# AmnonDrory/PointDSC

Measured on AMD Instinct MI355X. Metric: correspondence-pairs/sec through NSM (N=1k/5k) at 1/2/4/8 GPUs; 3DMatch recall parity, higher is better.
Workload: dtype f32 (3xf16-split contractions); 1 GPU; synthetic random correspondences N=1000 (3dmatch-like, 30% inliers), 128 scan pairs per GPU per step, full PointDSC testing forward (12 layers x 128 ch, trained synthetic weights, classifier rescaled by synthetic.BENCH_CLS for tie-free seed ranking); num_corr=1000, global_batch=128, parallelism=dp1 (independent pairs)

## Files before the change

### include/pdsc.h

```cpp
#ifndef PDSC_H_
#define PDSC_H_

#include <stddef.h>
#include <stdint.h>

#ifdef __cplusplus
extern "C" {
#endif

typedef void *pdsc_stream_t;

enum pdsc_status {
    PDSC_OK = 0,
    PDSC_ERR_ARG = 1,
    PDSC_ERR_HIP = 2,
    PDSC_ERR_UNSUPPORTED = 3,
    PDSC_ERR_RANGE = 4,
};

enum pdsc_precision {
    PDSC_PRECISION_H3 = 0,
    PDSC_PRECISION_F32 = 1,
};

int32_t pdsc_range_status(const void *forward_workspace, int32_t B, int32_t *flags, pdsc_stream_t stream);

int32_t pdsc_range_poll(const void *forward_workspace, int32_t B, pdsc_stream_t stream);

typedef struct pdsc_config {
    int32_t in_dim;
    int32_t num_layers;
    int32_t num_channels;
    int32_t num_iterations;
    int32_t k;
    double ratio;
    float inlier_threshold;
    float nms_radius;
    float refine_threshold;
    int32_t precision;
} pdsc_config;

const char *pdsc_version(void);
const char *pdsc_last_error(void);

int32_t pdsc_param_count(const pdsc_config *cfg);
const char *pdsc_param_name(const pdsc_config *cfg, int32_t i);
size_t pdsc_packed_weights_floats(const pdsc_config *cfg);
int32_t pdsc_pack_weights(const pdsc_config *cfg, const float *const *params_host_array,
                          float *packed, pdsc_stream_t stream);

int32_t pdsc_compat_f32(const float *src, const float *tgt, int32_t B, int32_t N,
                        const float *sigma_d_dev, float *M, pdsc_stream_t stream);
size_t pdsc_compat_packed_floats(int32_t N);
int32_t pdsc_compat_packed_f32(const float *src, const float *tgt, int32_t B, int32_t N,
                               const float *sigma_d_dev, float *Mp, pdsc_stream_t stream);

size_t pdsc_encoder_workspace_bytes(const pdsc_config *cfg, int32_t B, int32_t N);
int32_t pdsc_encoder_f32(const pdsc_config *cfg, const float *packed, const float *corr_pos,
                         const float *M, int32_t B, int32_t N, float *feat, float *normed,
                         float *conf, void *workspace, size_t workspace_bytes,
                         pdsc_stream_t stream);

size_t pdsc_attention_workspace_bytes(int32_t B, int32_t N, int32_t C, int32_t precision);
int32_t pdsc_attention_f32(const float *q, const float *k, const float *v, const float *M,
                           int32_t B, int32_t N, int32_t C, int32_t precision, float *msg, void *workspace,
                           size_t workspace_bytes, pdsc_stream_t stream);

int32_t pdsc_attention_layout(int32_t B, int32_t N, int32_t precision, int32_t *Npad, int32_t *nsplit);

int32_t pdsc_encoder_plan(int32_t B, int32_t N, int32_t precision, int32_t *fused);

int32_t pdsc_attention_timing(void *const *start_events, void *const *stop_events, int32_t capacity,
                              int32_t *count);
#define PDSC_FORWARD_STAGES 7
int32_t pdsc_forward_timing(void *const *events, int32_t capacity, int32_t *count);
int32_t pdsc_diag_qkv_delay(int32_t loops);

int32_t pdsc_pick_seeds(const float *src, const float *conf, int32_t B, int32_t N, float radius,
                        int32_t S, int32_t *seeds, float *is_local_max, pdsc_stream_t stream);

size_t pdsc_seed_knn_workspace_bytes(int32_t B, int32_t N, int32_t S);
int32_t pdsc_seed_knn(const float *normed, const int32_t *seeds, int32_t B, int32_t N, int32_t C,
                      int32_t S, int32_t k, int32_t precision, int32_t *knn, void *workspace,
                      size_t workspace_bytes, pdsc_stream_t stream);

size_t pdsc_nsm_workspace_bytes(int32_t B, int32_t N, int32_t S, int32_t k, int32_t num_iterations);
int32_t pdsc_nsm_weights(const float *normed, const float *src, const float *tgt,
                         const int32_t *knn, int32_t B, int32_t N, int32_t C, int32_t S, int32_t k,
                         int32_t num_iterations, int32_t precision, const float *sigma_dev,
                         const float *sigma_d_dev, float *weights, int32_t *iters_used, void *workspace,
                         size_t workspace_bytes, pdsc_stream_t stream);

int32_t pdsc_rigid_transform_3d(const float *A, const float *Bp, const float *w, int32_t nb,
                                int32_t n, float *trans, pdsc_stream_t stream);

size_t pdsc_seed_hypotheses_workspace_bytes(int32_t B, int32_t S);
int32_t pdsc_seed_hypotheses(const float *src, const float *tgt, const int32_t *knn,
                             const float *weights, int32_t B, int32_t N, int32_t S, int32_t k,
                             float tau, float *seed_trans, float *fitness, int32_t *best,
                             float *trans, float *labels, void *workspace, size_t workspace_bytes,
                             pdsc_stream_t stream);

int32_t pdsc_post_refine(float *trans, const float *src, const float *tgt, int32_t B, int32_t N,
                         float thr, pdsc_stream_t stream);

size_t pdsc_spectral_matching_workspace_bytes(int32_t N);
int32_t pdsc_spectral_matching(const float *corr_pos, const float *src, const float *tgt, int32_t N,
                               double inlier_threshold, double top_ratio, int32_t num_iterations, float *trans,
                               float *labels, float *leading_eig, void *workspace, size_t workspace_bytes,
                               pdsc_stream_t stream);
int32_t pdsc_sm_matvec(const float *M, const float *v, int32_t N, float *y, pdsc_stream_t stream);

size_t pdsc_forward_training_workspace_bytes(const pdsc_config *cfg, int32_t B, int32_t N);
int32_t pdsc_forward_training(const pdsc_config *cfg, const float *packed, const float *corr_pos,
                              const float *src, const float *tgt, int32_t B, int32_t N, float *final_trans,
                              float *confidence, float *M_out, int32_t *seeds_out, void *workspace,
                              size_t workspace_bytes, pdsc_stream_t stream);
size_t pdsc_spectral_matching_loss_workspace_bytes(int32_t B, int32_t N);
int32_t pdsc_spectral_matching_loss(const float *M, const float *gt_labels, int32_t B, int32_t N, int32_t balanced,
                                    float *loss, void *workspace, size_t workspace_bytes, pdsc_stream_t stream);

size_t pdsc_mutual_nn_workspace_bytes(int32_t Ns, int32_t Nt);
int32_t pdsc_mutual_nn(const float *src_desc, const float *tgt_desc, int32_t Ns, int32_t Nt, int32_t D,
                       int32_t *nn_src, int32_t *nn_tgt, void *workspace, size_t workspace_bytes,
                       pdsc_stream_t stream);
int32_t pdsc_build_correspondences(const float *src_desc, const float *tgt_desc, const float *src_xyz,
                                   const float *tgt_xyz, int32_t Ns, int32_t Nt, int32_t D, int32_t mutual,
                                   const double *gt_trans, double inlier_threshold, int32_t *corr,
                                   int32_t *count, float *corr_pos, float *src_keypts, float *tgt_keypts,
                                   float *labels, void *workspace, size_t workspace_bytes, pdsc_stream_t stream);

int32_t pdsc_ply_read_xyz(const char *path, float *xyz, int64_t capacity, int64_t *n_points);
size_t pdsc_radius_knn_workspace_bytes(int32_t n);
int32_t pdsc_radius_knn(const float *pts, int32_t n, float radius, int32_t max_nn, int32_t *nbr, double *dist2,
                        int32_t *count, void *workspace, size_t workspace_bytes, pdsc_stream_t stream);
enum pdsc_normal_orientation {
    PDSC_NORMALS_OPEN3D = 0,
    PDSC_NORMALS_VIEWPOINT = 1,
    PDSC_NORMALS_CENTROID = 2,
};
size_t pdsc_estimate_normals_workspace_bytes(int32_t n, int32_t max_nn);
int32_t pdsc_estimate_normals(const float *pts, int32_t n, float radius, int32_t max_nn, int32_t orient,
                              const float *viewpoint, float *normals, void *workspace, size_t workspace_bytes,
                              pdsc_stream_t stream);
size_t pdsc_voxel_down_sample_workspace_bytes(int32_t n);
int32_t pdsc_voxel_down_sample(const float *pts, const float *normals, int32_t n, float voxel_size, float *out_pts,
                               float *out_normals, int32_t *out_count, void *workspace, size_t workspace_bytes,
                               pdsc_stream_t stream);
size_t pdsc_compute_fpfh_workspace_bytes(int32_t n, int32_t max_nn);
int32_t pdsc_compute_fpfh(const float *pts, const float *normals, int32_t n, float radius, int32_t max_nn,
                          double *fpfh, float *fpfh_normalized, void *workspace, size_t workspace_bytes,
                          pdsc_stream_t stream);

size_t pdsc_forward_workspace_bytes(const pdsc_config *cfg, int32_t B, int32_t N);
int32_t pdsc_forward_testing(const pdsc_config *cfg, const float *packed, const float *corr_pos,
                             const float *src, const float *tgt, int32_t B, int32_t N,
                             float *final_trans, float *final_labels, float *conf_out,
                             int32_t *seeds_out, void *workspace, size_t workspace_bytes,
                             pdsc_stream_t stream);
typedef struct pdsc_forward_debug {
    float *conf;
    int32_t *seeds;
    int32_t *knn;
    float *weights;
    float *trans_pre_refine;
} pdsc_forward_debug;
int32_t pdsc_forward_testing_debug(const pdsc_config *cfg, const float *packed, const float *corr_pos,
                                   const float *src, const float *tgt, int32_t B, int32_t N,
                                   float *final_trans, float *final_labels, const pdsc_forward_debug *debug,
                                   void *workspace, size_t workspace_bytes, pdsc_stream_t stream);

int32_t pdsc_forward_testing_ragged(const pdsc_config *cfg, const float *packed, const float *corr_pos,
                                    const float *src, const float *tgt, int32_t B, int32_t N,
                                    const int32_t *counts, float *final_trans, float *final_labels,
                                    const pdsc_forward_debug *debug, void *workspace, size_t workspace_bytes,
                                    pdsc_stream_t stream);

#ifdef __cplusplus
}
#endif
#endif
```

### pointdsc_amd/_lib.py

```python
from __future__ import annotations

import ctypes
import os
import threading

_HERE = os.path.dirname(os.path.abspath(__file__))
_VARIANT = os.environ.get("PDSC_LIB_VARIANT", "")
LIB_PATH = os.path.join(_HERE, f"libpdsc_{_VARIANT}.so" if _VARIANT else "libpdsc.so")

c_int32, c_size_t, c_float, c_double = ctypes.c_int32, ctypes.c_size_t, ctypes.c_float, ctypes.c_double
vp = ctypes.c_void_p


class PdscConfig(ctypes.Structure):
    _fields_ = [
        ("in_dim", c_int32),
        ("num_layers", c_int32),
        ("num_channels", c_int32),
        ("num_iterations", c_int32),
        ("k", c_int32),
        ("ratio", c_double),
        ("inlier_threshold", c_float),
        ("nms_radius", c_float),
        ("refine_threshold", c_float),
        ("precision", c_int32),
    ]


PRECISIONS = {"h3": 0, "f32": 1}


def precision_code(precision) -> int:
    if precision not in PRECISIONS:
        raise ValueError(f"precision must be one of {sorted(PRECISIONS)}, got {precision!r}")
    return PRECISIONS[precision]


CFG = ctypes.POINTER(PdscConfig)


class PdscForwardDebug(ctypes.Structure):
    _fields_ = [("conf", vp), ("seeds", vp), ("knn", vp), ("weights", vp), ("trans_pre_refine", vp)]


_PROTOS = {
    "pdsc_version": (ctypes.c_char_p, []),
    "pdsc_last_error": (ctypes.c_char_p, []),
    "pdsc_param_count": (c_int32, [CFG]),
    "pdsc_param_name": (ctypes.c_char_p, [CFG, c_int32]),
    "pdsc_packed_weights_floats": (c_size_t, [CFG]),
    "pdsc_pack_weights": (c_int32, [CFG, ctypes.POINTER(vp), vp, vp]),
    "pdsc_compat_f32": (c_int32, [vp, vp, c_int32, c_int32, vp, vp, vp]),
    "pdsc_compat_packed_floats": (c_size_t, [c_int32]),
    "pdsc_compat_packed_f32": (c_int32, [vp, vp, c_int32, c_int32, vp, vp, vp]),
    "pdsc_encoder_workspace_bytes": (c_size_t, [CFG, c_int32, c_int32]),
    "pdsc_encoder_f32": (c_int32, [CFG, vp, vp, vp, c_int32, c_int32, vp, vp, vp, vp, c_size_t, vp]),
    "pdsc_attention_workspace_bytes": (c_size_t, [c_int32, c_int32, c_int32, c_int32]),
    "pdsc_attention_f32": (c_int32, [vp, vp, vp, vp, c_int32, c_int32, c_int32, c_int32, vp, vp, c_size_t, vp]),
    "pdsc_attention_layout": (c_int32, [c_int32, c_int32, c_int32, ctypes.POINTER(c_int32),
                                        ctypes.POINTER(c_int32)]),
    "pdsc_encoder_plan": (c_int32, [c_int32, c_int32, c_int32, ctypes.POINTER(c_int32)]),
    "pdsc_attention_timing": (c_int32, [ctypes.POINTER(vp), ctypes.POINTER(vp), c_int32, ctypes.POINTER(c_int32)]),
    "pdsc_forward_timing": (c_int32, [ctypes.POINTER(vp), c_int32, ctypes.POINTER(c_int32)]),
    "pdsc_diag_qkv_delay": (c_int32, [c_int32]),
    "pdsc_pick_seeds": (c_int32, [vp, vp, c_int32, c_int32, c_float, c_int32, vp, vp, vp]),
    "pdsc_seed_knn_workspace_bytes": (c_size_t, [c_int32, c_int32, c_int32]),
    "pdsc_seed_knn": (c_int32, [vp, vp, c_int32, c_int32, c_int32, c_int32, c_int32, c_int32, vp, vp, c_size_t,
                                vp]),
    "pdsc_nsm_workspace_bytes": (c_size_t, [c_int32, c_int32, c_int32, c_int32, c_int32]),
    "pdsc_nsm_weights": (c_int32, [vp, vp, vp, vp, c_int32, c_int32, c_int32, c_int32, c_int32, c_int32, c_int32,
                                   vp, vp, vp, vp, vp, c_size_t, vp]),
    "pdsc_rigid_transform_3d": (c_int32, [vp, vp, vp, c_int32, c_int32, vp, vp]),
    "pdsc_seed_hypotheses_workspace_bytes": (c_size_t, [c_int32, c_int32]),
    "pdsc_seed_hypotheses": (c_int32, [vp, vp, vp, vp, c_int32, c_int32, c_int32, c_int32, c_float,
                                       vp, vp, vp, vp, vp, vp, c_size_t, vp]),
    "pdsc_post_refine": (c_int32, [vp, vp, vp, c_int32, c_int32, c_float, vp]),
    "pdsc_mutual_nn_workspace_bytes": (c_size_t, [c_int32, c_int32]),
    "pdsc_mutual_nn": (c_int32, [vp, vp, c_int32, c_int32, c_int32, vp, vp, vp, c_size_t, vp]),
    "pdsc_build_correspondences": (c_int32, [vp, vp, vp, vp, c_int32, c_int32, c_int32, c_int32, vp, c_double,
                                             vp, vp, vp, vp, vp, vp, vp, c_size_t, vp]),
    "pdsc_spectral_matching_workspace_bytes": (c_size_t, [c_int32]),
    "pdsc_spectral_matching": (c_int32, [vp, vp, vp, c_int32, c_double, c_double, c_int32, vp, vp, vp, vp,
                                         c_size_t, vp]),
    "pdsc_sm_matvec": (c_int32, [vp, vp, c_int32, vp, vp]),
    "pdsc_forward_workspace_bytes": (c_size_t, [CFG, c_int32, c_int32]),
    "pdsc_forward_testing": (c_int32, [CFG, vp, vp, vp, vp, c_int32, c_int32, vp, vp, vp, vp, vp,
                                       c_size_t, vp]),
    "pdsc_forward_testing_debug": (c_int32, [CFG, vp, vp, vp, vp, c_int32, c_int32, vp, vp,
                                             ctypes.POINTER(PdscForwardDebug), vp, c_size_t, vp]),
    "pdsc_forward_testing_ragged": (c_int32, [CFG, vp, vp, vp, vp, c_int32, c_int32, ctypes.POINTER(c_int32), vp, vp,
                                              ctypes.POINTER(PdscForwardDebug), vp, c_size_t, vp]),
    "pdsc_ply_read_xyz": (c_int32, [ctypes.c_char_p, vp, ctypes.c_int64, ctypes.POINTER(ctypes.c_int64)]),
    "pdsc_radius_knn_workspace_bytes": (c_size_t, [c_int32]),
    "pdsc_radius_knn": (c_int32, [vp, c_int32, c_float, c_int32, vp, vp, vp, vp, c_size_t, vp]),
    "pdsc_estimate_normals_workspace_bytes": (c_size_t, [c_int32, c_int32]),
    "pdsc_estimate_normals": (c_int32, [vp, c_int32, c_float, c_int32, c_int32, vp, vp, vp, c_size_t, vp]),
    "pdsc_voxel_down_sample_workspace_bytes": (c_size_t, [c_int32]),
    "pdsc_voxel_down_sample": (c_int32, [vp, vp, c_int32, c_float, vp, vp, vp, vp, c_size_t, vp]),
    "pdsc_compute_fpfh_workspace_bytes": (c_size_t, [c_int32, c_int32]),
    "pdsc_compute_fpfh": (c_int32, [vp, vp, c_int32, c_float, c_int32, vp, vp, vp, c_size_t, vp]),
    "pdsc_forward_training_workspace_bytes": (c_size_t, [CFG, c_int32, c_int32]),
    "pdsc_range_status": (c_int32, [vp, c_int32, ctypes.POINTER(c_int32), vp]),
    "pdsc_range_poll": (c_int32, [vp, c_int32, vp]),
    "pdsc_forward_training": (c_int32, [CFG, vp, vp, vp, vp, c_int32, c_int32, vp, vp, vp, vp, vp, c_size_t, vp]),
    "pdsc_spectral_matching_loss_workspace_bytes": (c_size_t, [c_int32, c_int32]),
    "pdsc_spectral_matching_loss": (c_int32, [vp, vp, c_int32, c_int32, c_int32, vp, vp, c_size_t, vp]),
}

EXPORTS = tuple(_PROTOS)

_lib = None
_lock = threading.Lock()


def load():
    global _lib
    if _lib is not None:
        return _lib
    with _lock:
        if _lib is None:
            if not os.path.exists(LIB_PATH):
                raise RuntimeError(
                    f"pointdsc_amd: HIP library {LIB_PATH} is missing; build it with "
                    "`make -C pointdsc_amd/csrc` or `python -c 'import __graft_entry__ as g; g.build()'`. "
                    "There is no CPU fallback.")
            try:
                lib = ctypes.CDLL(LIB_PATH)
            except OSError as e:
                raise RuntimeError(f"pointdsc_amd: cannot load {LIB_PATH}: {e}") from e
            for name, (res, args) in _PROTOS.items():
                fn = getattr(lib, name)
                fn.restype, fn.argtypes = res, args
            _lib = lib
    return _lib


def check(status: int, what: str):
    if status != 0:
        msg = load().pdsc_last_error().decode(errors="replace")
        raise RuntimeError(f"{what} failed (status {status}): {msg}")


def make_config(in_dim=6, num_layers=12, num_channels=128, num_iterations=10, k=40, ratio=0.1,
                inlier_threshold=0.10, nms_radius=0.10, precision="h3") -> PdscConfig:
    refine = 0.10 if inlier_threshold == 0.10 else 1.2
    return PdscConfig(int(in_dim), int(num_layers), int(num_channels), int(num_iterations), int(k),
                      float(ratio), float(inlier_threshold), float(nms_radius), float(refine),
                      precision_code(precision))
```

### pointdsc_amd/csrc/api.hip

```cpp
#include <algorithm>
#include <chrono>
#include <cstdarg>
#include <cstdio>
#include <cstdlib>
#include <mutex>
#include <string>
#include <vector>

#include "attention_plan.hpp"
#include "pdsc_internal.hpp"

using namespace pdsc;

namespace pdsc {
thread_local int g_diag_qkv_delay = 0;
}

namespace {

thread_local std::string g_err;
thread_local std::string g_name;

thread_local hipEvent_t *g_tstart = nullptr, *g_tstop = nullptr;
thread_local int g_tcap = 0;
thread_local int32_t *g_tcount = nullptr;
thread_local hipEvent_t *g_fev = nullptr;
thread_local int g_fcap = 0;
thread_local int32_t *g_fcount = nullptr;

int fail(int code, const char *fmt, ...) {
    char buf[512];
    va_list ap;
    va_start(ap, fmt);
    vsnprintf(buf, sizeof(buf), fmt, ap);
    va_end(ap);
    g_err = buf;
    return code;
}

#define HIPCHK(expr)                                                                          \
    do {                                                                                      \
        hipError_t e_ = (expr);                                                               \
        if (e_ != hipSuccess) return fail(PDSC_ERR_HIP, "%s: %s", #expr, hipGetErrorString(e_)); \
    } while (0)

hipStream_t S_(pdsc_stream_t s) { return reinterpret_cast<hipStream_t>(s); }

struct Carve {
    char *base;
    size_t off = 0;
    explicit Carve(void *p) : base(static_cast<char *>(p)) {}
    template <typename T> T *take(size_t n) {
        T *p = base ? reinterpret_cast<T *>(base + off) : nullptr;
        off += align_bytes(n * sizeof(T));
        return p;
    }
};

int check_cfg(const pdsc_config *cfg) {
    if (!cfg) return fail(PDSC_ERR_ARG, "cfg is NULL");
    if (cfg->num_channels != CH)
        return fail(PDSC_ERR_UNSUPPORTED, "num_channels=%d: only %d is implemented", cfg->num_channels, CH);
    if (cfg->num_layers < 1 || cfg->num_layers > 64)
        return fail(PDSC_ERR_UNSUPPORTED, "num_layers=%d not in [1, 64]", cfg->num_layers);
    if (cfg->in_dim < 1 || cfg->in_dim > 128) return fail(PDSC_ERR_UNSUPPORTED, "in_dim=%d not in [1, 128]", cfg->in_dim);
    if (cfg->num_iterations < 0 || cfg->num_iterations > 31)
        return fail(PDSC_ERR_UNSUPPORTED, "num_iterations=%d not in [0, 31]", cfg->num_iterations);
    if (cfg->k < 1) return fail(PDSC_ERR_ARG, "k=%d", cfg->k);
    if (cfg->precision != PDSC_PRECISION_H3 && cfg->precision != PDSC_PRECISION_F32)
        return fail(PDSC_ERR_ARG, "precision=%d (PDSC_PRECISION_H3 or PDSC_PRECISION_F32)", cfg->precision);
    return PDSC_OK;
}

struct Dims {
    int B, N, Npad, S, k, T;
    bool f32;
    EncoderPlan plan;
};

int make_dims(const pdsc_config *cfg, int B, int N, Dims &d, bool dense_m_caller = false) {
    if (B < 1 || N < 2) return fail(PDSC_ERR_ARG, "B=%d N=%d (need B >= 1, N >= 2)", B, N);
    if (N > 32767) return fail(PDSC_ERR_UNSUPPORTED, "N=%d > 32767 (32-bit buffer descriptors over M)", N);
    d.B = B;
    d.N = N;
    d.Npad = round_up(N, QB);
    d.S = (int)((double)N * cfg->ratio);
    d.k = std::min(cfg->k, N - 1);
    d.T = cfg->num_iterations;
    d.f32 = cfg->precision == PDSC_PRECISION_F32;
    d.plan = plan_encoder(B, N, d.f32, dense_m_caller);
    if (d.S < 1) return fail(PDSC_ERR_ARG, "int(N*ratio) = 0 seeds for N=%d", N);
    if (d.k > 63) return fail(PDSC_ERR_UNSUPPORTED, "k=%d > 63", d.k);
    return PDSC_OK;
}

struct EncBufs {
    float *feat, *opart, *ml, *vexp, *vexp2;
    float *feat2;
    _Float16 *q, *k, *v;
    _Float16 *q2, *k2, *v2;
    float *opart1, *ml1;
};

EncBufs carve_encoder(Carve &c, const Dims &d) {
    EncBufs e;
    const size_t rows = (size_t)d.B * d.Npad * CH;
    e.feat = c.take<float>(rows);
    e.q = c.take<_Float16>(2 * rows);
    e.k = c.take<_Float16>(2 * rows);
    e.v = c.take<_Float16>(2 * rows);
    e.opart = c.take<float>(rows * d.plan.nsplit);
    e.ml = c.take<float>((size_t)d.B * d.Npad * d.plan.nsplit * 2);
    e.vexp = c.take<float>((size_t)d.B * (d.Npad / 32));
    e.opart1 = d.plan.precombine ? c.take<float>(rows) : nullptr;
    e.ml1 = d.plan.precombine ? c.take<float>((size_t)d.B * d.Npad * 2) : nullptr;
    e.q2 = e.k2 = e.v2 = nullptr;
    e.vexp2 = nullptr;
    e.feat2 = d.plan.fused() ? nullptr : c.take<float>(rows);
    if (d.plan.fused()) {
        e.q2 = c.take<_Float16>(2 * rows);
        e.k2 = c.take<_Float16>(2 * rows);
        e.v2 = c.take<_Float16>(2 * rows);
        e.vexp2 = c.take<float>((size_t)d.B * (d.Npad / 32));
    }
    return e;
}

int run_encoder(const PackLayout &lay, const float *packed, const float *corr_pos, const float *M, const Dims &d,
                const EncBufs &e, float *feat_out, float *normed, _Float16 *normed_s, float *conf, hipStream_t s,
                Ragged rg = {}) {
    const EncoderPlan plan = d.plan.for_ragged(rg);
    HIPCHK(launch_pw_first(packed, lay, corr_pos, d.f32, d.B, d.N, d.Npad, e.feat, e.q, e.k, e.v, e.vexp, s, rg,
                           plan.fused()));
    if (plan.fused()) {
        _Float16 *q = e.q, *k = e.k, *v = e.v, *q2 = e.q2, *k2 = e.k2, *v2 = e.v2;
        float *vx = e.vexp, *vx2 = e.vexp2;
        for (int l = 0; l + 1 < lay.L; ++l) {
            const bool timed = g_tcap > 0 && g_tcount && *g_tcount < g_tcap;
            if (timed) HIPCHK(hipEventRecord(g_tstart[*g_tcount], s));
            HIPCHK(launch_attn_pw2(plan, packed, lay, l, q, k, v, vx, M, e.feat, q2, k2, v2, vx2, s, rg));
            if (timed) HIPCHK(hipEventRecord(g_tstop[(*g_tcount)++], s));
            std::swap(q, q2);
            std::swap(k, k2);
            std::swap(v, v2);
            std::swap(vx, vx2);
        }
        HIPCHK(launch_attn_pw2_last(plan, packed, lay, q, k, v, vx, M, e.feat, feat_out, normed, normed_s, conf, s, rg));
        return PDSC_OK;
    }
    float *feat = e.feat, *feat_alt = e.feat2;
    for (int l = 0; l < lay.L; ++l) {
        const bool timed = g_tcap > 0 && g_tcount && *g_tcount < g_tcap;
        if (timed) HIPCHK(hipEventRecord(g_tstart[*g_tcount], s));
        HIPCHK(launch_attention(plan, e.q, e.k, e.v, e.vexp, M, e.opart, e.ml, s, rg, l));
        if (timed) HIPCHK(hipEventRecord(g_tstop[(*g_tcount)++], s));
        const float *op = e.opart, *mlp = e.ml;
        int ns = plan.nsplit;
        if (plan.precombine) {
            HIPCHK(launch_combine_rows(e.opart, e.ml, d.B, d.Npad, plan.nsplit, e.opart1, e.ml1, s));
            op = e.opart1;
            mlp = e.ml1;
            ns = 1;
        }
        if (l + 1 < lay.L) {
            HIPCHK(launch_pw_mid(packed, lay, l, d.f32, op, mlp, ns, d.B, d.N, d.Npad, feat, feat_alt, e.q, e.k, e.v,
                                 e.vexp, s));
            std::swap(feat, feat_alt);
        } else {
            HIPCHK(launch_pw_last(packed, lay, d.f32, op, mlp, ns, d.B, d.N, d.Npad, feat, feat_out, normed,
                                  d.f32 ? nullptr : normed_s, conf, s));
        }
    }
    return PDSC_OK;
}

static int enc_halves_mode() {
    static const int v = [] {
        const char *e = getenv("PDSC_ENC_HALVES");
        return e && e[0] == '0' ? 0 : (e && e[0] == '1' ? 2 : 1);
    }();
    return v;
}
constexpr int ENC_MAX_PARTS = 4;
static int enc_parts() {
    static const int v = [] {
        const char *e = getenv("PDSC_ENC_PARTS");
        const int p = e ? atoi(e) : 2;
        return std::min(std::max(p, 2), ENC_MAX_PARTS);
    }();
    return v;
}
static bool enc_work_balanced() {
    static const bool on = [] {
        const char *e = getenv("PDSC_ENC_BAL");
        return e && e[0] == '1';
    }();
    return on;
}
static bool enc_halves(const Dims &d, bool ragged) {
    const int mode = enc_halves_mode();
    return d.plan.fused() && d.B >= 16 * enc_parts() && (mode == 2 || (mode == 1 && ragged));
}
static void enc_bounds(const int32_t *counts, int B, int P, int *bounds) {
    std::vector<double> pre(B + 1, 0.0);
    for (int b = 0; b < B; ++b) pre[b + 1] = pre[b] + (counts ? (double)counts[b] * counts[b] : 1.0);
    bounds[0] = 0;
    bounds[P] = B;
    for (int i = 1; i < P; ++i) {
        const double goal = pre[B] * i / P;
        int h = bounds[i - 1] + 1;
        while (h < B - (P - i) && std::abs(pre[h + 1] - goal) < std::abs(pre[h] - goal)) ++h;
        bounds[i] = h;
    }
}

struct SideStream {
    std::mutex mu;
    hipStream_t s2[ENC_MAX_PARTS - 1] = {};
    hipEvent_t fork = nullptr, join[ENC_MAX_PARTS - 1] = {};
    bool ok = false;
};
static SideStream *side_stream(hipStream_t s) {
    static SideStream ss[64];
    hipDevice_t dev = 0;
    if (!s || hipStreamGetDevice(s, &dev) != hipSuccess)
        if (hipGetDevice(&dev) != hipSuccess) return nullptr;
    if (dev < 0 || dev >= 64) return nullptr;
    SideStream &x = ss[dev];
    static std::mutex create_mu;
    std::lock_guard<std::mutex> lock(create_mu);
    if (!x.ok) {
        int cur = dev;
        if (hipGetDevice(&cur) != hipSuccess || (cur != dev && hipSetDevice(dev) != hipSuccess)) return nullptr;
        bool ok = x.fork || hipEventCreateWithFlags(&x.fork, hipEventDisableTiming) == hipSuccess;
        for (int i = 0; ok && i < ENC_MAX_PARTS - 1; ++i) {
            if (!x.s2[i]) ok = hipStreamCreateWithFlags(&x.s2[i], hipStreamNonBlocking) == hipSuccess;
            if (ok && !x.join[i]) ok = hipEventCreateWithFlags(&x.join[i], hipEventDisableTiming) == hipSuccess;
        }
        if (cur != dev) (void)hipSetDevice(cur);
        x.ok = ok;
    }
    return x.ok ? &x : nullptr;
}

static int run_encoder_part(const PackLayout &lay, const float *packed, const float *corr_pos, const float *M,
                            const Dims &d, const EncBufs &e, float *normed, _Float16 *normed_s, float *conf,
                            hipStream_t s, Ragged rg, int b0, int nb) {
    Dims dh = d;
    dh.B = nb;
    dh.plan = d.plan.for_pairs(nb);
    const size_t rows = (size_t)b0 * d.Npad * CH;
    EncBufs eh = e;
    eh.feat = e.feat + rows;
    eh.q = e.q + 2 * rows;
    eh.k = e.k + 2 * rows;
    eh.v = e.v + 2 * rows;
    eh.q2 = e.q2 + 2 * rows;
    eh.k2 = e.k2 + 2 * rows;
    eh.v2 = e.v2 + 2 * rows;
    eh.vexp = e.vexp + (size_t)b0 * (d.Npad / 32);
    eh.vexp2 = e.vexp2 + (size_t)b0 * (d.Npad / 32);
    const size_t mstr = d.plan.m_layout == M_PACKED ? mpack_floats(d.N) : (size_t)d.N * d.N;
    Ragged rh = rg;
    if (rg.nv) rh.nv = rg.nv + b0;
    if (rg.sv) rh.sv = rg.sv + b0;
    if (rg.po) rh.po = rg.po + b0;
    return run_encoder(lay, packed, corr_pos + (size_t)b0 * d.N * lay.in_dim, M + (size_t)b0 * mstr, dh, eh, nullptr,
                       normed + (size_t)b0 * d.N * CH, normed_s + (size_t)b0 * d.N * 2 * CH, conf + (size_t)b0 * d.N, s,
                       rh);
}

static int run_encoder_fwd(const PackLayout &lay, const float *packed, const float *corr_pos, const float *M,
                           const Dims &d, const EncBufs &e, float *normed, _Float16 *normed_s, float *conf,
                           hipStream_t s, Ragged rg, SideStream *ss, const int *bounds, int P) {
    if (!ss) return run_encoder(lay, packed, corr_pos, M, d, e, nullptr, normed, normed_s, conf, s, rg);
    std::lock_guard<std::mutex> lock(ss->mu);
    {
        hipStreamCaptureStatus cs = hipStreamCaptureStatusNone, c2 = hipStreamCaptureStatusNone;
        unsigned long long id = 0, id2 = 0;
        HIPCHK(hipStreamGetCaptureInfo(s, &cs, &id));
        for (int i = 1; i < P; ++i) {
            HIPCHK(hipStreamGetCaptureInfo(ss->s2[i - 1], &c2, &id2));
            if (c2 != hipStreamCaptureStatusNone && (cs != hipStreamCaptureStatusActive || id2 != id))
                return run_encoder(lay, packed, corr_pos, M, d, e, nullptr, normed, normed_s, conf, s, rg);
        }
    }
    HIPCHK(hipEventRecord(ss->fork, s));
    int forked = 1, r = PDSC_OK;
    for (; forked < P; ++forked)
        if (hipStreamWaitEvent(ss->s2[forked - 1], ss->fork, 0) != hipSuccess) {
            r = fail(PDSC_ERR_HIP, "hipStreamWaitEvent (fork)");
            break;
        }
    for (int i = 0; r == PDSC_OK && i < P; ++i)
        r = run_encoder_part(lay, packed, corr_pos, M, d, e, normed, normed_s, conf, i ? ss->s2[i - 1] : s, rg,
                             bounds[i], bounds[i + 1] - bounds[i]);
    for (int i = 1; i < forked; ++i) {
        const hipError_t a = hipEventRecord(ss->join[i - 1], ss->s2[i - 1]);
        const hipError_t b = a == hipSuccess ? hipStreamWaitEvent(s, ss->join[i - 1], 0) : a;
        if (b != hipSuccess && r == PDSC_OK) r = fail(PDSC_ERR_HIP, "join: %s", hipGetErrorString(b));
    }
    return r;
}

struct NsmBufs {
    float *hist, *weights;
    _Float16 *ns;
    unsigned *mask;
};

NsmBufs carve_nsm(Carve &c, int B, int N, int S, int k, int T, bool own_split) {
    NsmBufs n;
    n.ns = own_split ? c.take<_Float16>((size_t)B * N * 2 * CH) : nullptr;
    n.hist = c.take<float>((size_t)B * S * std::max(T, 1) * k);
    n.mask = c.take<unsigned>((size_t)B * S);
    n.weights = c.take<float>((size_t)B * S * k);
    return n;
}

int run_nsm(const float *normed, const _Float16 *normed_s, bool f32, const float *src, const float *tgt,
            const int *knn, int B, int N, int S, int k, int T, const float *sigma, const float *sigma_d,
            const NsmBufs &nb, float *weights, int *iters, bool batch_global, hipStream_t s, Ragged rg = {}) {
    if (!f32 && !normed_s) {
        HIPCHK(launch_split_rows(normed, (size_t)B * N, nb.ns, s));
        normed_s = nb.ns;
    }
    const void *feats = f32 ? static_cast<const void *>(normed) : static_cast<const void *>(normed_s);
    if (T > 0)
        HIPCHK(launch_nsm_seed(feats, f32, src, tgt, knn, B, N, S, k, T, sigma, sigma_d, nb.hist, nb.mask, s, rg));
    HIPCHK(launch_nsm_finish(nb.hist, nb.mask, B, S, k, T, batch_global, weights, iters, s, rg));
    return PDSC_OK;
}

static bool tail_fused() {
    static const bool off = [] {
        const char *e = getenv("PDSC_TAIL_FUSED");
        return e && e[0] == '0';
    }();
    return !off;
}

static bool ragged_order_on() {
    static const bool off = [] {
        const char *e = getenv("PDSC_RAGGED_ORDER");
        return e && e[0] == '0';
    }();
    return !off;
}

struct FwdBufs {
    int *range;
    float *M, *normed, *conf, *lm, *kdist, *seed_trans, *weights, *hsums;
    _Float16 *normed_s;
    int *seeds, *knn, *counts;
    int *nv, *sv, *po;
    EncBufs enc;
    NsmBufs nsm;
};

FwdBufs carve_forward(Carve &c, const Dims &d) {
    FwdBufs f;
    f.range = c.take<int>((size_t)d.B);
    f.M = c.take<float>((size_t)d.B * std::max(mpack_floats(d.N), (size_t)d.N * d.N));
    f.enc = carve_encoder(c, d);
    f.normed = c.take<float>((size_t)d.B * d.N * CH);
    f.normed_s = c.take<_Float16>((size_t)d.B * d.N * 2 * CH);
    f.conf = c.take<float>((size_t)d.B * d.N);
    f.lm = c.take<float>((size_t)d.B * d.N);
    f.seeds = c.take<int>((size_t)d.B * d.S);
    f.kdist = c.take<float>((size_t)d.B * d.S * d.N);
    f.knn = c.take<int>((size_t)d.B * d.S * d.k);
    f.nsm = carve_nsm(c, d.B, d.N, d.S, d.k, d.T, false);
    f.weights = f.nsm.weights;
    f.seed_trans = c.take<float>((size_t)d.B * d.S * 16);
    f.counts = c.take<int>((size_t)d.B * d.S);
    f.hsums = c.take<float>((size_t)d.B * d.S * 15);
    f.nv = c.take<int>((size_t)d.B);
    f.sv = c.take<int>((size_t)d.B);
    f.po = c.take<int>((size_t)d.B);
    return f;
}

int need_ws(size_t have, size_t need) {
    if (have < need) return fail(PDSC_ERR_ARG, "workspace too small: %zu < %zu bytes", have, need);
    return PDSC_OK;
}

}

#define RET_IF(x)                  \
    do {                           \
        int r_ = (x);              \
        if (r_ != PDSC_OK) return r_; \
    } while (0)

namespace {
int32_t check_nn_args(const float *a, const float *b, int32_t Ns, int32_t Nt, int32_t D, void *ws, size_t ws_bytes) {
    if (!a || !b || !ws) return fail(PDSC_ERR_ARG, "null pointer");
    if (Ns < 1 || Nt < 1 || D < 1 || D > 64) return fail(PDSC_ERR_ARG, "Ns=%d Nt=%d D=%d (1 <= D <= 64)", Ns, Nt, D);
    return need_ws(ws_bytes, pdsc_mutual_nn_workspace_bytes(Ns, Nt));
}

__global__ void unpack_nn_kernel(const unsigned long long *key, int n, int32_t *out) {
    const int i = blockIdx.x * blockDim.x + threadIdx.x;
    if (i < n) out[i] = (int32_t)(uint32_t)key[i];
}
}

extern "C" {

const char *pdsc_version(void) { return "pdsc 0.1.0 gfx950"; }
const char *pdsc_last_error(void) { return g_err.c_str(); }

int32_t pdsc_param_count(const pdsc_config *cfg) { return cfg ? 10 + 26 * cfg->num_layers : -1; }

const char *pdsc_param_name(const pdsc_config *cfg, int32_t i) {
    if (!cfg || i < 0 || i >= pdsc_param_count(cfg)) return nullptr;
    static const char *bn[] = {"weight", "bias", "running_mean", "running_var"};
    static const char *per[] = {"fc_message.0.weight", "fc_message.0.bias", "fc_message.1.weight",
                                "fc_message.1.bias", "fc_message.1.running_mean", "fc_message.1.running_var",
                                "fc_message.3.weight", "fc_message.3.bias", "fc_message.4.weight",
                                "fc_message.4.bias", "fc_message.4.running_mean", "fc_message.4.running_var",
                                "fc_message.6.weight", "fc_message.6.bias", "projection_q.weight",
                                "projection_q.bias", "projection_k.weight", "projection_k.bias",
                                "projection_v.weight", "projection_v.bias"};
    static const char *tail[] = {"encoder.layer0.weight", "encoder.layer0.bias", "classification.0.weight",
                                 "classification.0.bias", "classification.2.weight", "classification.2.bias",
                                 "classification.4.weight", "classification.4.bias"};
    const int L = cfg->num_layers;
    if (i == 0) return "sigma";
    if (i == 1) return "sigma_spat";
    i -= 2;
    if (i < 26 * L) {
        const int l = i / 26, o = i % 26;
        char buf[128];
        if (o < 2)
            snprintf(buf, sizeof(buf), "encoder.blocks.PointCN_layer_%d.0.%s", l, o == 0 ? "weight" : "bias");
        else if (o < 6)
            snprintf(buf, sizeof(buf), "encoder.blocks.PointCN_layer_%d.1.%s", l, bn[o - 2]);
        else
            snprintf(buf, sizeof(buf), "encoder.blocks.NonLocal_layer_%d.%s", l, per[o - 6]);
        g_name = buf;
        return g_name.c_str();
    }
    return tail[i - 26 * L];
}

size_t pdsc_packed_weights_floats(const pdsc_config *cfg) {
    if (check_cfg(cfg) != PDSC_OK) return 0;
    return make_layout(cfg->num_layers, cfg->in_dim).total;
}

int32_t pdsc_pack_weights(const pdsc_config *cfg, const float *const *P, float *packed,
                          pdsc_stream_t stream) {
    RET_IF(check_cfg(cfg));
    if (!P || !packed) return fail(PDSC_ERR_ARG, "null params/packed");
    const int n = pdsc_param_count(cfg);
    for (int i = 0; i < n; ++i)
        if (!P[i]) return fail(PDSC_ERR_ARG, "param %d (%s) is NULL", i, pdsc_param_name(cfg, i));
    hipStream_t s = S_(stream);
    const PackLayout lay = make_layout(cfg->num_layers, cfg->in_dim);
    HIPCHK(hipMemsetAsync(packed, 0, lay.total * sizeof(float), s));
    HIPCHK(launch_copy(P[0], packed + lay.sigma, 1, s));
    HIPCHK(launch_copy(P[1], packed + lay.sigma_d, 1, s));
    const bool f32 = cfg->precision == PDSC_PRECISION_F32;
    auto dense = [&](const DenseOff &o, int wi, int in, int out, bool has_bn) -> hipError_t {
        return launch_pack_dense(P[wi], P[wi + 1], has_bn ? P[wi + 2] : nullptr,
                                 has_bn ? P[wi + 3] : nullptr, has_bn ? P[wi + 4] : nullptr,
                                 has_bn ? P[wi + 5] : nullptr, in, out, f32, packed + o.w, packed + o.bias,
                                 packed + o.alpha, packed + o.beta, packed + o.scale, s);
    };
    for (int l = 0; l < cfg->num_layers; ++l) {
        const int b = 2 + 26 * l;
        const LayerOff &lo = lay.layer[l];
        HIPCHK(dense(lo.pcn, b + 0, CH, CH, true));
        HIPCHK(dense(lo.fc0, b + 6, CH, CH2, true));
        HIPCHK(dense(lo.fc3, b + 12, CH2, CH2, true));
        HIPCHK(dense(lo.fc6, b + 18, CH2, CH, false));
        HIPCHK(dense(lo.q, b + 20, CH, CH, false));
        HIPCHK(dense(lo.k, b + 22, CH, CH, false));
        HIPCHK(dense(lo.v, b + 24, CH, CH, false));
    }
    const int t = 2 + 26 * cfg->num_layers;
    HIPCHK(launch_copy(P[t], packed + lay.l0_w, CH * cfg->in_dim, s));
    HIPCHK(launch_copy(P[t + 1], packed + lay.l0_b, CH, s));
    HIPCHK(dense(lay.c0, t + 2, CH, CLS, false));
    HIPCHK(dense(lay.c2, t + 4, CLS, CLS, false));
    HIPCHK(launch_copy(P[t + 6], packed + lay.c4_w, CLS, s));
    HIPCHK(launch_copy(P[t + 7], packed + lay.c4_b, 1, s));
    return PDSC_OK;
}

int32_t pdsc_compat_f32(const float *src, const float *tgt, int32_t B, int32_t N,
                        const float *sigma_d_dev, float *M, pdsc_stream_t stream) {
    if (!src || !tgt || !sigma_d_dev || !M) return fail(PDSC_ERR_ARG, "null pointer");
    if (B < 1 || N < 1) return fail(PDSC_ERR_ARG, "B=%d N=%d", B, N);
    HIPCHK(launch_compat(src, tgt, B, N, sigma_d_dev, M, S_(stream)));
    return PDSC_OK;
}

size_t pdsc_compat_packed_floats(int32_t N) { return N < 1 ? 0 : mpack_floats(N); }

int32_t pdsc_compat_packed_f32(const float *src, const float *tgt, int32_t B, int32_t N,
                               const float *sigma_d_dev, float *Mp, pdsc_stream_t stream) {
    if (!src || !tgt || !sigma_d_dev || !Mp) return fail(PDSC_ERR_ARG, "null pointer");
    if (B < 1 || N < 1) return fail(PDSC_ERR_ARG, "B=%d N=%d", B, N);
    HIPCHK(launch_compat_packed(src, tgt, B, N, sigma_d_dev, Mp, S_(stream)));
    return PDSC_OK;
}

size_t pdsc_encoder_workspace_bytes(const pdsc_config *cfg, int32_t B, int32_t N) {
    Dims d;
    if (check_cfg(cfg) != PDSC_OK || make_dims(cfg, B, N, d, true) != PDSC_OK) return 0;
    Carve c(nullptr);
    carve_encoder(c, d);
    return c.off;
}

int32_t pdsc_encoder_f32(const pdsc_config *cfg, const float *packed, const float *corr_pos,
                         const float *M, int32_t B, int32_t N, float *feat, float *normed, float *conf,
                         void *ws, size_t ws_bytes, pdsc_stream_t stream) {
    RET_IF(check_cfg(cfg));
    Dims d;
    RET_IF(make_dims(cfg, B, N, d, true));
    if (!packed || !corr_pos || !M || !normed || !conf || !ws) return fail(PDSC_ERR_ARG, "null pointer");
    RET_IF(need_ws(ws_bytes, pdsc_encoder_workspace_bytes(cfg, B, N)));
    Carve c(ws);
    const EncBufs e = carve_encoder(c, d);
    const PackLayout lay = make_layout(cfg->num_layers, cfg->in_dim);
    return run_encoder(lay, packed, corr_pos, M, d, e, feat, normed, nullptr, conf, S_(stream));
}

size_t pdsc_attention_workspace_bytes(int32_t B, int32_t N, int32_t C, int32_t precision) {
    if (C != CH || B < 1 || N < 1 || (precision != PDSC_PRECISION_H3 && precision != PDSC_PRECISION_F32)) return 0;
    const int Npad = round_up(N, QB), ns = plan_encoder(B, N, precision == PDSC_PRECISION_F32, true, false).nsplit;
    Carve c(nullptr);
    for (int i = 0; i < 3; ++i) c.take<_Float16>((size_t)2 * B * Npad * CH);
    c.take<float>((size_t)B * Npad * CH * ns);
    c.take<float>((size_t)B * Npad * ns * 2);
    c.take<float>((size_t)B * (Npad / 32));
    return c.off;
}

int32_t pdsc_attention_f32(const float *q, const float *k, const float *v, const float *M, int32_t B,
                           int32_t N, int32_t C, int32_t precision, float *msg, void *ws, size_t ws_bytes,
                           pdsc_stream_t stream) {
    if (C != CH) return fail(PDSC_ERR_UNSUPPORTED, "C=%d (only %d)", C, CH);
    if (!q || !k || !v || !M || !msg || !ws) return fail(PDSC_ERR_ARG, "null pointer");
    if (B < 1 || N < 1 || N > 32767) return fail(PDSC_ERR_ARG, "B=%d N=%d", B, N);
    if (precision != PDSC_PRECISION_H3 && precision != PDSC_PRECISION_F32)
        return fail(PDSC_ERR_ARG, "precision=%d", precision);
    RET_IF(need_ws(ws_bytes, pdsc_attention_workspace_bytes(B, N, C, precision)));
    hipStream_t s = S_(stream);
    const bool f32 = precision == PDSC_PRECISION_F32;
    const EncoderPlan plan = plan_encoder(B, N, f32, true, false);
    const int Npad = plan.Npad, ns = plan.nsplit;
    Carve c(ws);
    _Float16 *qs = c.take<_Float16>((size_t)2 * B * Npad * CH);
    _Float16 *ks = c.take<_Float16>((size_t)2 * B * Npad * CH);
    _Float16 *vs = c.take<_Float16>((size_t)2 * B * Npad * CH);
    float *op = c.take<float>((size_t)B * Npad * CH * ns);
    float *ml = c.take<float>((size_t)B * Npad * ns * 2);
    float *vexp = c.take<float>((size_t)B * (Npad / 32));
    if (f32) {
        HIPCHK(launch_pad_rows(q, B, N, Npad, reinterpret_cast<float *>(qs), s));
        HIPCHK(launch_pad_rows(k, B, N, Npad, reinterpret_cast<float *>(ks), s));
        HIPCHK(launch_pad_rows(v, B, N, Npad, reinterpret_cast<float *>(vs), s));
    } else {
        HIPCHK(launch_split_qkv(q, k, v, B, N, N, Npad, qs, ks, vs, vexp, s));
    }
    HIPCHK(launch_attention(plan, qs, ks, vs, vexp, M, op, ml, s));
    HIPCHK(launch_attn_combine(op, ml, f32, B, N, Npad, ns, msg, s));
    return PDSC_OK;
}

int32_t pdsc_attention_timing(void *const *start_events, void *const *stop_events, int32_t capacity,
                              int32_t *count) {
    if (capacity > 0 && (!start_events || !stop_events || !count))
        return fail(PDSC_ERR_ARG, "null events/count with capacity %d", capacity);
    g_tstart = reinterpret_cast<hipEvent_t *>(const_cast<void **>(start_events));
    g_tstop = reinterpret_cast<hipEvent_t *>(const_cast<void **>(stop_events));
    g_tcap = capacity;
    g_tcount = count;
    return PDSC_OK;
}

int32_t pdsc_diag_qkv_delay(int32_t loops) {
    if (loops < 0) return fail(PDSC_ERR_ARG, "loops=%d", loops);
    g_diag_qkv_delay = loops;
    return PDSC_OK;
}

int32_t pdsc_forward_timing(void *const *events, int32_t capacity, int32_t *count) {
    if (capacity > 0 && (!events || !count)) return fail(PDSC_ERR_ARG, "null events/count with capacity %d", capacity);
    g_fev = reinterpret_cast<hipEvent_t *>(const_cast<void **>(events));
    g_fcap = capacity;
    g_fcount = count;
    return PDSC_OK;
}

int32_t pdsc_attention_layout(int32_t B, int32_t N, int32_t precision, int32_t *Npad, int32_t *nsplit) {
    if (precision != PDSC_PRECISION_H3 && precision != PDSC_PRECISION_F32)
        return fail(PDSC_ERR_ARG, "precision %d (enum pdsc_precision)", precision);
    if (B < 1 || N < 1 || !Npad || !nsplit) return fail(PDSC_ERR_ARG, "B=%d N=%d", B, N);
    const EncoderPlan plan = plan_encoder(B, N, precision == PDSC_PRECISION_F32, false);
    *Npad = plan.Npad;
    *nsplit = plan.nsplit;
    return PDSC_OK;
}

int32_t pdsc_encoder_plan(int32_t B, int32_t N, int32_t precision, int32_t *fused) {
    if (precision != PDSC_PRECISION_H3 && precision != PDSC_PRECISION_F32)
        return fail(PDSC_ERR_ARG, "precision %d (enum pdsc_precision)", precision);
    if (B < 1 || N < 1 || !fused) return fail(PDSC_ERR_ARG, "B=%d N=%d", B, N);
    const EncoderPlan plan = plan_encoder(B, N, precision == PDSC_PRECISION_F32, false);
    *fused = plan.fused() ? 1 : (plan.w64() ? 2 : 0);
    return PDSC_OK;
}

int32_t pdsc_pick_seeds(const float *src, const float *conf, int32_t B, int32_t N, float radius,
                        int32_t S, int32_t *seeds, float *is_local_max, pdsc_stream_t stream) {
    if (!src || !conf || !seeds || !is_local_max) return fail(PDSC_ERR_ARG, "null pointer (is_local_max is used as scratch)");
    if (B < 1 || N < 1 || S < 1 || S > N) return fail(PDSC_ERR_ARG, "B=%d N=%d S=%d", B, N, S);
    hipStream_t s = S_(stream);
    HIPCHK(launch_local_max(src, conf, B, N, radius, is_local_max, s));
    HIPCHK(launch_seed_rank(conf, is_local_max, B, N, S, seeds, s));
    return PDSC_OK;
}

int run_seed_knn(const float *normed, const _Float16 *normed_s, bool f32, const int *seeds, int B, int N, int S,
                 int k, float *dist, int *knn, hipStream_t s, Ragged rg = {}) {
    if (f32) {
        HIPCHK(launch_knn_dist_f32(normed, seeds, B, N, S, dist, s, rg));
    } else {
        HIPCHK(launch_knn_dist(normed_s, seeds, B, N, S, dist, s, rg));
    }
    HIPCHK(launch_knn_select(dist, B, N, S, k, knn, s, rg));
    return PDSC_OK;
}

size_t pdsc_seed_knn_workspace_bytes(int32_t B, int32_t N, int32_t S) {
    return align_bytes((size_t)B * S * N * sizeof(float)) + align_bytes((size_t)B * N * 2 * CH * sizeof(_Float16));
}

int32_t pdsc_seed_knn(const float *normed, const int32_t *seeds, int32_t B, int32_t N, int32_t C,
                      int32_t S, int32_t k, int32_t precision, int32_t *knn, void *ws, size_t ws_bytes,
                      pdsc_stream_t stream) {
    if (precision != PDSC_PRECISION_H3 && precision != PDSC_PRECISION_F32)
        return fail(PDSC_ERR_ARG, "precision=%d", precision);
    if (C != CH) return fail(PDSC_ERR_UNSUPPORTED, "C=%d (only %d)", C, CH);
    if (!normed || !seeds || !knn || !ws) return fail(PDSC_ERR_ARG, "null pointer");
    if (B < 1 || S < 1 || k < 1 || k + 1 > N || k > 63) return fail(PDSC_ERR_ARG, "B=%d N=%d S=%d k=%d", B, N, S, k);
    RET_IF(need_ws(ws_bytes, pdsc_seed_knn_workspace_bytes(B, N, S)));
    hipStream_t s = S_(stream);
    Carve c(ws);
    float *dist = c.take<float>((size_t)B * S * N);
    _Float16 *ns = c.take<_Float16>((size_t)B * N * 2 * CH);
    const bool f32 = precision == PDSC_PRECISION_F32;
    if (!f32) HIPCHK(launch_split_rows(normed, (size_t)B * N, ns, s));
    return run_seed_knn(normed, ns, f32, seeds, B, N, S, k, dist, knn, s);
}

size_t pdsc_nsm_workspace_bytes(int32_t B, int32_t N, int32_t S, int32_t k, int32_t T) {
    Carve c(nullptr);
    carve_nsm(c, B, N, S, k, T, true);
    return c.off;
}

int32_t pdsc_nsm_weights(const float *normed, const float *src, const float *tgt, const int32_t *knn,
                         int32_t B, int32_t N, int32_t C, int32_t S, int32_t k, int32_t T, int32_t precision,
                         const float *sigma, const float *sigma_d, float *weights, int32_t *iters,
                         void *ws, size_t ws_bytes, pdsc_stream_t stream) {
    if (C != CH) return fail(PDSC_ERR_UNSUPPORTED, "C=%d (only %d)", C, CH);
    if (!normed || !src || !tgt || !knn || !sigma || !sigma_d || !weights || !ws)
        return fail(PDSC_ERR_ARG, "null pointer");
    if (B < 1 || S < 1 || k < 1 || k > 63 || N < k + 1 || T < 0 || T > 31)
        return fail(PDSC_ERR_ARG, "B=%d N=%d S=%d k=%d T=%d (1 <= k <= min(63, N-1), 0 <= T <= 31)", B, N, S, k, T);
    if (precision != PDSC_PRECISION_H3 && precision != PDSC_PRECISION_F32)
        return fail(PDSC_ERR_ARG, "precision=%d", precision);
    RET_IF(need_ws(ws_bytes, pdsc_nsm_workspace_bytes(B, N, S, k, T)));
    Carve c(ws);
    NsmBufs nb = carve_nsm(c, B, N, S, k, T, true);
    return run_nsm(normed, nullptr, precision == PDSC_PRECISION_F32, src, tgt, knn, B, N, S, k, T, sigma, sigma_d,
                   nb, weights, iters, true, S_(stream));
}

int32_t pdsc_rigid_transform_3d(const float *A, const float *Bp, const float *w, int32_t nb, int32_t n,
                                float *trans, pdsc_stream_t stream) {
    if (!A || !Bp || !trans) return fail(PDSC_ERR_ARG, "null pointer");
    if (nb < 1 || n < 0) return fail(PDSC_ERR_ARG, "nb=%d n=%d", nb, n);
    HIPCHK(launch_rigid(A, Bp, w, nb, n, trans, S_(stream)));
    return PDSC_OK;
}

size_t pdsc_seed_hypotheses_workspace_bytes(int32_t B, int32_t S) {
    return align_bytes((size_t)B * S * 15 * sizeof(float));
}

int32_t pdsc_seed_hypotheses(const float *src, const float *tgt, const int32_t *knn, const float *weights,
                             int32_t B, int32_t N, int32_t S, int32_t k, float tau, float *seed_trans,
                             float *fitness, int32_t *best, float *trans, float *labels, void *ws,
                             size_t ws_bytes, pdsc_stream_t stream) {
    if (!src || !tgt || !knn || !weights || !trans || !labels || !seed_trans)
        return fail(PDSC_ERR_ARG, "null pointer (seed_trans is required as scratch)");
    if (B < 1 || S < 1 || k < 1 || k > 63 || N < k + 1)
        return fail(PDSC_ERR_ARG, "B=%d N=%d S=%d k=%d (1 <= k <= min(63, N-1))", B, N, S, k);
    hipStream_t s = S_(stream);
    if (!fitness) return fail(PDSC_ERR_ARG, "fitness [B,S] buffer is required (hosts the inlier counts)");
    int *counts = reinterpret_cast<int *>(fitness);
    if (!ws || ws_bytes < pdsc_seed_hypotheses_workspace_bytes(B, S))
        return fail(PDSC_ERR_ARG, "workspace too small");
    HIPCHK(launch_hypotheses(src, tgt, knn, weights, B, N, S, k, tau, seed_trans, counts,
                             static_cast<float *>(ws), s));
    HIPCHK(launch_select_best(src, tgt, seed_trans, counts, B, N, S, tau, fitness, best, trans, labels, s));
    return PDSC_OK;
}

int32_t pdsc_post_refine(float *trans, const float *src, const float *tgt, int32_t B, int32_t N, float thr,
                         pdsc_stream_t stream) {
    if (!trans || !src || !tgt) return fail(PDSC_ERR_ARG, "null pointer");
    if (B < 1 || N < 1) return fail(PDSC_ERR_ARG, "B=%d N=%d", B, N);
    HIPCHK(launch_post_refine(trans, src, tgt, B, N, thr, S_(stream)));
    return PDSC_OK;
}

size_t pdsc_forward_workspace_bytes(const pdsc_config *cfg, int32_t B, int32_t N) {
    Dims d;
    if (check_cfg(cfg) != PDSC_OK || make_dims(cfg, B, N, d) != PDSC_OK) return 0;
    Carve c(nullptr);
    carve_forward(c, d);
    return c.off;
}

int32_t pdsc_forward_testing(const pdsc_config *cfg, const float *packed, const float *corr_pos,
                             const float *src, const float *tgt, int32_t B, int32_t N, float *final_trans,
                             float *final_labels, float *conf_out, int32_t *seeds_out, void *ws,
                             size_t ws_bytes, pdsc_stream_t stream) {
    pdsc_forward_debug dbg{};
    dbg.conf = conf_out;
    dbg.seeds = seeds_out;
    return pdsc_forward_testing_debug(cfg, packed, corr_pos, src, tgt, B, N, final_trans, final_labels, &dbg, ws,
                                      ws_bytes, stream);
}

static int32_t forward_testing_impl(const pdsc_config *cfg, const float *packed, const float *corr_pos,
                                    const float *src, const float *tgt, int32_t B, int32_t N, const int32_t *counts,
                                    float *final_trans, float *final_labels, const pdsc_forward_debug *dbg, void *ws,
                                    size_t ws_bytes, pdsc_stream_t stream) {
    const pdsc_forward_debug no{};
    if (!dbg) dbg = &no;
    RET_IF(check_cfg(cfg));
    Dims d;
    RET_IF(make_dims(cfg, B, N, d));
    if (!packed || !corr_pos || !src || !tgt || !final_trans || !final_labels || !ws)
        return fail(PDSC_ERR_ARG, "null pointer");
    if (counts)
        for (int b = 0; b < B; ++b) {
            const int n = counts[b];
            if (n < 2 || n > N || std::min(cfg->k, n - 1) != d.k || (int)((double)n * cfg->ratio) < 1)
                return fail(PDSC_ERR_ARG, "counts[%d] = %d: need k + 1 = %d <= count <= N = %d and int(count * ratio) >= 1",
                            b, n, d.k + 1, N);
        }
    RET_IF(need_ws(ws_bytes, pdsc_forward_workspace_bytes(cfg, B, N)));
    hipStream_t s = S_(stream);
    Carve c(ws);
    const FwdBufs f = carve_forward(c, d);
    Ragged rg;
    SideStream *halves = enc_halves(d, counts != nullptr) ? side_stream(s) : nullptr;
    const int parts = halves ? enc_parts() : 1;
// ... 389 lines not shown
```

### pointdsc_amd/csrc/attention_h3.hpp

```cpp
#pragma once
#include "pdsc_internal.hpp"

typedef _Float16 f16x8 __attribute__((ext_vector_type(8)));

namespace pdsc {

constexpr int H3_ROWB = 2 * CH * 2;
constexpr int H3_TILE = 32;
constexpr int H3_KTB = H3_TILE * H3_ROWB;
constexpr int H3_VTB = 2 * CH * H3_TILE * 2;
constexpr int H3_PSHIFT = 7;
constexpr float H3_DEFER = 8.0f;
#ifndef ATT_SOFTMAX_PRIO
#define ATT_SOFTMAX_PRIO 1
#endif
#ifndef ATT_QFMA
#define ATT_QFMA 1
#endif
#ifndef ATT_BUFDMA
#define ATT_BUFDMA 1
#endif
constexpr float H3_QSCALE = 0.12751743082459868f;
constexpr int H3_VEXP_MAX = 8;
constexpr int H3_VEXP_TARGET = 5;
// ... 45 lines not shown
    u32x4 h, l;
#pragma unroll
    for (int e = 0; e < 4; ++e) {
        uint32_t a, b;
        split2(v[2 * e], v[2 * e + 1], a, b);
        h[e] = a;
        l[e] = b;
    }
    hi = __builtin_bit_cast(f16x8, h);
    lo = __builtin_bit_cast(f16x8, l);
}

PDSC_DEV float halves_max(float x) {
    const auto r = __builtin_amdgcn_permlane32_swap(__float_as_uint(x), __float_as_uint(x), false, false);
    return fmaxf(__uint_as_float(r[0]), __uint_as_float(r[1]));
}
PDSC_DEV float halves_sum(float x) {
    const auto r = __builtin_amdgcn_permlane32_swap(__float_as_uint(x), __float_as_uint(x), false, false);
    return __uint_as_float(r[0]) + __uint_as_float(r[1]);
}

PDSC_DEV f32x16 mfma_h(f16x8 a, f16x8 b, f32x16 c) {
    return __builtin_amdgcn_mfma_f32_32x32x16_f16(a, b, c, 0, 0, 0);
}
PDSC_DEV f32x16 mfma_h3(f16x8 ah, f16x8 al, f16x8 bh, f16x8 bl, f32x16 c) {
    c = mfma_h(al, bh, c);
    c = mfma_h(ah, bl, c);
    return mfma_h(ah, bh, c);
}

PDSC_DEV f32x16 mfma_xw3(f16x8 xh, f16x8 xl, f16x8 wh, f16x8 wm, f16x8 wl, f32x16 c) {
    if constexpr (W_PLANES == 3) c = mfma_h(xh, wl, c);
    c = mfma_h(xh, wm, c);
    c = mfma_h(xl, wh, c);
    return mfma_h(xh, wh, c);
}
PDSC_DEV f32x16 mfma_w3x(f16x8 wh, f16x8 wm, f16x8 wl, f16x8 xh, f16x8 xl, f32x16 c) {
    if constexpr (W_PLANES == 3) c = mfma_h(wl, xh, c);
    c = mfma_h(wm, xh, c);
    c = mfma_h(wh, xl, c);
    return mfma_h(wh, xh, c);
}

#ifdef ATT_STAMPS
constexpr int ST_PER_WAVE = 256, ST_WGS = 64;
static __device__ unsigned long long g_att_stamps[ST_WGS * 4 * ST_PER_WAVE];
PDSC_DEV unsigned long long *att_stamp_ptr(int wave) {
    return (blockIdx.x % 16 == 0 && blockIdx.x / 16 < ST_WGS && wave < 4 && blockIdx.z == 0)
               ? g_att_stamps + ((blockIdx.x / 16) * 4 + wave) * ST_PER_WAVE
               : nullptr;
}
#define ATT_STAMP(stp, i)                                                       \
    do {                                                                        \
        __builtin_amdgcn_sched_barrier(0);                                      \
        if (stp) {                                                              \
            const unsigned long long t_ = __builtin_amdgcn_s_memtime();         \
            if (lane == 0) stp[i] = t_;                                         \
        }                                                                       \
        __builtin_amdgcn_sched_barrier(0);                                      \
    } while (0)
#define ATT_RSTAMP(stp, i)                                                      \
    do {                                                                        \
        if (stp) {                                                              \
            const unsigned long long t_ = __builtin_amdgcn_s_memrealtime();     \
            if (lane == 0) stp[i] = t_;                                         \
        }                                                                       \
    } while (0)
#define CH_STAMP(i)                                       \
    do {                                                  \
        unsigned long long *stc_ = att_stamp_ptr(wave);   \
        ATT_STAMP(stc_, i);                               \
    } while (0)
#else
#define CH_STAMP(i) \
    do {            \
    } while (0)
#define ATT_STAMP(stp, i) \
    do {                  \
    } while (0)
#define ATT_RSTAMP(stp, i) \
    do {                   \
    } while (0)
#endif

constexpr int H3_NSLOT = 2;
template <int NW>
constexpr size_t attention_h3_lds_bytes() { return (size_t)H3_NSLOT * (H3_KTB + H3_VTB); }

PDSC_DEV __amdgpu_buffer_rsrc_t h3_rsrc(const void *base, uint32_t bytes) {
    return __builtin_amdgcn_make_buffer_rsrc(const_cast<void *>(base), 0, (int)bytes, 0x00020000);
}

struct AttnGridH3 {
    int B, N, Npad, nqb, nsplit, sps;
    const int *nv;
    const int *po;
    int rev = 0;
    PDSC_DEV int n(int b) const { return nv ? nv[b] : N; }
};

constexpr int H3_SPLIT_C0 = 15;
inline int attention_split_count(long blocks, int nst, int slots) {
    int best = 1;
    long best_cost = -1;
    for (int ns = 1; ns <= std::max(1, nst / 2); ++ns) {
        const int sps = (nst + ns - 1) / ns;
        if ((nst + sps - 1) / sps != ns) continue;
        const long rounds = (blocks * ns + slots - 1) / slots;
        const long cost = rounds * (sps + H3_SPLIT_C0);
        if (best_cost < 0 || cost < best_cost) {
            best = ns;
            best_cost = cost;
        }
    }
    return best;
}

template <int NW>
inline AttnGridH3 attention_h3_grid(int B, int N, int slots) {
    AttnGridH3 g;
    g.nv = nullptr;
    g.po = nullptr;
    g.B = B;
    g.N = N;
    g.Npad = round_up(N, QB);
    g.nqb = (N + NW * 32 - 1) / (NW * 32);
    const int nst = (N + H3_TILE - 1) / H3_TILE;
    const int ns = attention_split_count((long)B * g.nqb, nst, slots);
    g.sps = (nst + ns - 1) / ns;
    g.nsplit = (nst + g.sps - 1) / g.sps;
    return g;
}

struct AttnBlock {
    int b, qb, split;
    int st0 = 0, st1 = -1;
};
PDSC_DEV AttnBlock attention_h3_block(const AttnGridH3 &g, bool xcd) {
    const int G = g.B * g.nqb * g.nsplit;
    int lid = blockIdx.x;
    if (xcd) {
        const int full = G & ~7;
        if (lid < full) {
            const int loc = lid >> 3;
            lid = (lid & 7) * (full >> 3) + (g.rev ? (full >> 3) - 1 - loc : loc);
        }
    } else if (g.rev) {
        lid = G - 1 - lid;
    }
    const int slot = lid / g.nsplit / g.nqb;
    return AttnBlock{g.po ? g.po[slot] : slot, (lid / g.nsplit) % g.nqb, lid % g.nsplit};
}

template <int NW, bool PACKED, bool EARLY = false, int WS = 0>
PDSC_DEV void attention_h3_core(const _Float16 *__restrict__ Qs, const _Float16 *__restrict__ Ks,
                                const _Float16 *__restrict__ Vs, const float *__restrict__ vexp,
                                const float *__restrict__ M, const AttnGridH3 &g, const AttnBlock &blk, char *h3smem,
                                int wave, int lane, f32x16 (&O)[4], float &m_run, float &l_run) {
    static_assert(WS == 0 || (NW == 1 && !EARLY), "wave-split: one 32-query block, the plain loop");
    const int b = blk.b, qb = blk.qb, split = blk.split;
    const int N = g.n(b), Npad = g.Npad;
    const int h = lane >> 5, l32 = lane & 31;
    const int q0 = WS ? qb * 32 : qb * (NW * 32) + wave * 32;
    const int nst = (N + H3_TILE - 1) / H3_TILE;
    int st0 = split * g.sps, st1 = min(nst, st0 + g.sps);
    if constexpr (WS > 0) {
        const int tpw = (st1 - st0 + WS - 1) / WS, a = min(st1, st0 + wave * tpw);
        st1 = min(st1, a + tpw);
        st0 = a;
    }
    const int qq = q0 + l32;
    const bool active = q0 < Npad;

    const char *Kp = reinterpret_cast<const char *>(Ks + (size_t)b * Npad * 2 * CH);
    const char *Vp = reinterpret_cast<const char *>(Vs + (size_t)b * Npad * 2 * CH);
    const int mnt = mpack_ntile(g.N);
    const size_t mper = PACKED ? (size_t)mnt * (mnt + 1) / 2 * MPACK_T * MPACK_T : (size_t)g.N * g.N;
    const __amdgpu_buffer_rsrc_t rM = h3_rsrc(M + (size_t)b * mper, (uint32_t)(mper * 4u));

    f16x8 qh[8], ql[8];
    {
        const _Float16 *qt = Qs + (size_t)b * Npad * 2 * CH + (size_t)(min(q0, Npad - 32) >> 5) * H3_TILE_H;
#pragma unroll
        for (int j = 0; j < 8; ++j) {
            qh[j] = *reinterpret_cast<const f16x8 *>(qt + h3_frag(j, 0, lane));
            ql[j] = *reinterpret_cast<const f16x8 *>(qt + h3_frag(j, 1, lane));
        }
    }

#if ATT_BUFDMA
    const __amdgpu_buffer_rsrc_t rK = h3_rsrc(Kp, (uint32_t)Npad * H3_ROWB), rV = h3_rsrc(Vp, (uint32_t)Npad * H3_ROWB);
#endif
    auto stage = [&](int st, int slot) {
        char *dst = h3smem + (WS ? wave : slot) * (H3_KTB + H3_VTB);
        constexpr int PIECES = (H3_KTB + H3_VTB) / 1024;
#pragma unroll
        for (int i = 0; i < PIECES / NW; ++i) {
            const int piece = WS ? i : wave * (PIECES / NW) + i;
#if ATT_BUFDMA
            if (piece < H3_KTB / 1024)
                __builtin_amdgcn_raw_ptr_buffer_load_lds(rK, (__attribute__((address_space(3))) void *)(dst + piece * 1024),
                                                         16, 16 * lane, st * H3_KTB + piece * 1024, 0, 0);
            else
                __builtin_amdgcn_raw_ptr_buffer_load_lds(rV, (__attribute__((address_space(3))) void *)(dst + piece * 1024),
                                                         16, 16 * lane, st * H3_VTB + (piece - H3_KTB / 1024) * 1024, 0, 0);
#else
            const char *src = piece < H3_KTB / 1024
                                  ? Kp + (size_t)st * H3_KTB + piece * 1024
                                  : Vp + (size_t)st * H3_VTB + (piece - H3_KTB / 1024) * 1024;
            __builtin_amdgcn_global_load_lds(src + 16 * lane, dst + piece * 1024, 16, 0, 0);
#endif
        }
    };

#pragma unroll
    for (int t = 0; t < 4; ++t) O[t] = zero16();
    m_run = -INFINITY;
    l_run = 0.0f;
    const float scale = ATT_QFMA ? 1.0f : H3_QSCALE;
    const uint32_t Nb = (uint32_t)g.N * 4;

#ifdef ATT_STAMPS
    unsigned long long *stp = att_stamp_ptr(wave);
#endif
    int st_si = 0;
    (void)st_si;
    const float *vexp_b = vexp + (size_t)b * (Npad / H3_TILE);
    const __amdgpu_buffer_rsrc_t rE = h3_rsrc(vexp_b, (uint32_t)(Npad / H3_TILE) * 4u);
    auto load_m = [&](int key0, float (&mv)[16], float &ev) {
        if constexpr (PACKED) {
            static_assert(MPACK_T == 32, "one packed tile per wave step");
            const int kt = key0 / MPACK_T, qt = q0 / MPACK_T;
            const int kr = 4 * h, qr = l32;
            if (kt <= qt) {
                const uint32_t vo =
                    ((uint32_t)mpack_tile(kt, qt, mnt) * (MPACK_T * MPACK_T) + (uint32_t)(kr * MPACK_T + qr)) * 4;
#pragma unroll
                for (int r = 0; r < 16; ++r)
                    mv[r] = __builtin_bit_cast(float, __builtin_amdgcn_raw_buffer_load_b32(
                                                          rM, vo + (uint32_t)((r & 3) + 8 * (r >> 2)) * (MPACK_T * 4), 0, 0));
            } else {
                const uint32_t vo =
                    ((uint32_t)mpack_tile(qt, kt, mnt) * (MPACK_T * MPACK_T) + (uint32_t)(qr * MPACK_T + kr)) * 4;
#pragma unroll
                for (int g = 0; g < 4; ++g) {
                    const f32x4 v4 = __builtin_bit_cast(f32x4, __builtin_amdgcn_raw_buffer_load_b128(rM, vo + 32 * g, 0, 0));
#pragma unroll
                    for (int e = 0; e < 4; ++e) mv[4 * g + e] = v4[e];
                }
            }
        } else {
            const uint32_t vo = ((uint32_t)(key0 + 4 * h) * (uint32_t)g.N + (uint32_t)qq) * 4;
#pragma unroll
            for (int r = 0; r < 16; ++r)
                mv[r] = __builtin_bit_cast(
                    float, __builtin_amdgcn_raw_buffer_load_b32(rM, vo + (uint32_t)((r & 3) + 8 * (r >> 2)) * Nb, 0, 0));
        }
        ev = __builtin_bit_cast(float, __builtin_amdgcn_raw_buffer_load_b32(rE, (uint32_t)(key0 / H3_TILE) * 4u, 0, 0));
    };
    auto qk_softmax = [&](const char *Kl, int key0, float (&mv)[16], float ev, f16x8(&ph)[2], f16x8(&pl)[2],
                          bool first, auto after_qk) {
        f32x16 S = zero16();
        f16x8 kf[3][2];
        auto kread = [&](int j, f16x8(&f)[2]) {
            f[0] = *reinterpret_cast<const f16x8 *>(Kl + 2 * h3_frag(j, 0, lane));
            f[1] = *reinterpret_cast<const f16x8 *>(Kl + 2 * h3_frag(j, 1, lane));
        };
        kread(0, kf[0]);
        kread(1, kf[1]);
#pragma unroll
        for (int j = 0; j < 8; ++j) {
            if (j + 2 < 8) kread(j + 2, kf[(j + 2) % 3]);
            S = mfma_h3(kf[j % 3][0], kf[j % 3][1], qh[j], ql[j], S);
            __builtin_amdgcn_sched_barrier(0);
        }
        after_qk();
        if (ATT_SOFTMAX_PRIO > 0) __builtin_amdgcn_s_setprio(ATT_SOFTMAX_PRIO);
        float p[16];
        float mx = -INFINITY;
        float ex[16];
        if (ATT_QFMA && !first) {
            const float mb0 = m_run - (float)H3_PSHIFT + ev;
#pragma unroll
            for (int r = 0; r < 16; ++r) p[r] = __builtin_fmaf(mv[r], S[r], -mb0);
            ATT_STAMP(stp, st_si + 1);
            ATT_STAMP(stp, st_si + 2);
            if (key0 + 32 > N) {
#pragma unroll
                for (int r = 0; r < 16; ++r)
                    if (key0 + acc_row(r, h) >= N) p[r] = -INFINITY;
            }
#pragma unroll
            for (int r = 0; r < 16; ++r) mx = fmaxf(mx, p[r]);
            mx = halves_max(mx);
            if (__any(mx > H3_DEFER + (float)H3_PSHIFT - ev)) {
                const float m_new = fmaxf(m_run, mx + mb0);
                const float alpha = __builtin_amdgcn_exp2f(m_run - m_new);
                const float dm = m_new - m_run;
                m_run = m_new;
                l_run *= alpha;
#pragma unroll
                for (int t = 0; t < 4; ++t)
#pragma unroll
                    for (int r = 0; r < 16; ++r) O[t][r] *= alpha;
#pragma unroll
                for (int r = 0; r < 16; ++r) p[r] -= dm;
            }
        } else {
#pragma unroll
            for (int r = 0; r < 16; ++r) p[r] = S[r] * scale;
            ATT_STAMP(stp, st_si + 1);
#pragma unroll
            for (int r = 0; r < 16; ++r) p[r] = mv[r] * p[r];
            ATT_STAMP(stp, st_si + 2);
            if (key0 + 32 > N) {
#pragma unroll
                for (int r = 0; r < 16; ++r)
                    if (key0 + acc_row(r, h) >= N) p[r] = -INFINITY;
            }
#pragma unroll
            for (int r = 0; r < 16; ++r) mx = fmaxf(mx, p[r]);
            mx = halves_max(mx);
            if (__any(mx > m_run + H3_DEFER)) {
                const float m_new = fmaxf(m_run, mx);
                const float alpha = __builtin_amdgcn_exp2f(m_run - m_new);
                m_run = m_new;
                l_run *= alpha;
#pragma unroll
                for (int t = 0; t < 4; ++t)
#pragma unroll
                    for (int r = 0; r < 16; ++r) O[t][r] *= alpha;
            }
            const float mb = m_run - (float)H3_PSHIFT + ev;
#pragma unroll
            for (int r = 0; r < 16; ++r) p[r] -= mb;
        }
        float psum = 0.0f;
#pragma unroll
        for (int r = 0; r < 16; ++r) {
            ex[r] = __builtin_amdgcn_exp2f(p[r]);
            psum += ex[r];
        }
#pragma unroll
        for (int s = 0; s < 2; ++s) {
            float v[8];
#pragma unroll
            for (int e = 0; e < 8; ++e) v[e] = ex[8 * s + e];
            split8x(v, ph[s], pl[s]);
        }
        l_run += ldexpf(psum, (int)ev);
        if (ATT_SOFTMAX_PRIO > 0) __builtin_amdgcn_s_setprio(0);
    };
    auto pv = [&](const char *Vl, const f16x8(&ph)[2], const f16x8(&pl)[2]) {
        f16x8 vf[3][2];
        auto vread = [&](int i, f16x8(&f)[2]) {
            f[0] = *reinterpret_cast<const f16x8 *>(Vl + 2 * h3_frag(i, 0, lane));
            f[1] = *reinterpret_cast<const f16x8 *>(Vl + 2 * h3_frag(i, 1, lane));
        };
        vread(0, vf[0]);
        vread(1, vf[1]);
#pragma unroll
        for (int i = 0; i < 8; ++i) {
            if (i + 2 < 8) vread(i + 2, vf[(i + 2) % 3]);
            f32x16 o = mfma_h(vf[i % 3][0], pl[i & 1], O[i >> 1]);
            o = mfma_h(vf[i % 3][1], ph[i & 1], o);
            O[i >> 1] = mfma_h(vf[i % 3][0], ph[i & 1], o);
            __builtin_amdgcn_sched_barrier(0);
        }
    };

    auto sync = [&] {
        __builtin_amdgcn_s_waitcnt(0x0070);
#ifndef ATT_DIAG_NOBAR
        if constexpr (WS == 0) __builtin_amdgcn_s_barrier();
#endif
    };

    auto slot_base = [&](int st) {
        return h3smem + (WS ? wave : (st - st0) % H3_NSLOT) * (H3_KTB + H3_VTB);
    };
    if constexpr (WS > 0) {
        char *slot = h3smem + wave * (H3_KTB + H3_VTB);
        auto stage_half = [&](int st, bool v) {
#pragma unroll
            for (int i = 0; i < 16; ++i) {
#if ATT_BUFDMA
                __builtin_amdgcn_raw_ptr_buffer_load_lds(v ? rV : rK,
                                                         (__attribute__((address_space(3))) void *)(slot + (v ? H3_KTB : 0) + i * 1024),
                                                         16, 16 * lane, st * (v ? H3_VTB : H3_KTB) + i * 1024, 0, 0);
#else
                const char *src = (v ? Vp + (size_t)st * H3_VTB : Kp + (size_t)st * H3_KTB) + i * 1024;
                __builtin_amdgcn_global_load_lds(src + 16 * lane, slot + (v ? H3_KTB : 0) + i * 1024, 16, 0, 0);
#endif
            }
        };
        float mvA[16], evA;
        if (st0 < st1) {
            stage_half(st0, false);
            load_m(st0 * H3_TILE, mvA, evA);
            stage_half(st0, true);
        }
        for (int st = st0; st < st1; ++st) {
            float mv[16], ev;
            f16x8 ph[2], pl[2];
            __builtin_amdgcn_s_waitcnt(0x4F70);
#pragma unroll
            for (int r = 0; r < 16; ++r) mv[r] = mvA[r];
            ev = evA;
            const bool more = st + 1 < st1;
            qk_softmax(slot, st * H3_TILE, mv, ev, ph, pl, st == st0, [&] {
                if (more) {
                    __builtin_amdgcn_s_waitcnt(0xC07F);
                    stage_half(st + 1, false);
                }
            });
            if (more)
                __builtin_amdgcn_s_waitcnt(0x4F70);
            else
                __builtin_amdgcn_s_waitcnt(0x0F70);
            pv(slot + H3_KTB, ph, pl);
            if (more) {
                load_m((st + 1) * H3_TILE, mvA, evA);
                __builtin_amdgcn_s_waitcnt(0xC07F);
                stage_half(st + 1, true);
            }
        }
        l_run = halves_sum(l_run);
        return;
    }
    float mvA[16], evA;
    if (st0 < st1) {
        stage(st0, 0);
        if constexpr (EARLY) {
            load_m(st0 * H3_TILE, mvA, evA);
            if (st0 + 1 < st1) stage(st0 + 1, 1);
        }
    }
    sync();
    for (int st = st0; st < st1; ++st) {
        float mv[16], ev;
        f16x8 ph[2], pl[2];
        const int si = 1 + 6 * min(st - st0, 23);
        st_si = si;
        ATT_STAMP(stp, si);
        if constexpr (EARLY) {
#pragma unroll
            for (int r = 0; r < 16; ++r) mv[r] = mvA[r];
            ev = evA;
            if (st + 1 < st1) load_m((st + 1) * H3_TILE, mvA, evA);
            if (st > st0 && st + 1 < st1) stage(st + 1, ((st + 1 - st0) % H3_NSLOT));
        } else {
            load_m(st * H3_TILE, mv, ev);
            if (st + 1 < st1) stage(st + 1, ((st + 1 - st0) % H3_NSLOT));
        }
        qk_softmax(slot_base(st), st * H3_TILE, mv, ev, ph, pl, st == st0, [] {});
        ATT_STAMP(stp, si + 3);
        pv(slot_base(st) + H3_KTB, ph, pl);
        ATT_STAMP(stp, si + 4);
        sync();
        ATT_STAMP(stp, si + 5);
    }
    l_run = halves_sum(l_run);
}

template <int NW, bool XCD, bool PACKED, bool EARLY = false>
__global__ __launch_bounds__(NW * 64, 2) void attention_h3_kernel(
    const _Float16 *__restrict__ Qs, const _Float16 *__restrict__ Ks, const _Float16 *__restrict__ Vs,
    const float *__restrict__ vexp, const float *__restrict__ M, AttnGridH3 g, float *__restrict__ opart,
    float *__restrict__ ml) {
    extern __shared__ __attribute__((aligned(16))) char h3smem[];
    const AttnBlock blk = attention_h3_block(g, XCD);
    if (blk.qb * (NW * 32) >= g.n(blk.b)) return;
    const int b = blk.b, split = blk.split, Npad = g.Npad;
    const int tid = threadIdx.x, wave = __builtin_amdgcn_readfirstlane(tid >> 6), lane = tid & 63, h = lane >> 5;
    const int q0 = blk.qb * (NW * 32) + wave * 32, qq = q0 + (lane & 31);
#ifdef ATT_STAMPS
    unsigned long long *stp = att_stamp_ptr(wave);
    ATT_RSTAMP(stp, 184);
    ATT_STAMP(stp, 160);
#endif
    f32x16 O[4];
    float m_run, l_run;
    attention_h3_core<NW, PACKED, EARLY>(Qs, Ks, Vs, vexp, M, g, blk, h3smem, wave, lane, O, m_run, l_run);
    ATT_STAMP(stp, 161);
    ATT_RSTAMP(stp, 185);
    if (q0 >= Npad) return;
    const size_t obase = (size_t)(b * g.nsplit + split) * Npad;
    float *Ob = opart + obase * CH + (size_t)(q0 >> 5) * (H3_TILE * CH) + 4 * lane;
#pragma unroll
    for (int t = 0; t < 4; ++t)
#pragma unroll
        for (int q = 0; q < 4; ++q)
            *reinterpret_cast<f32x4 *>(Ob + (4 * t + q) * 256) =
                f32x4{O[t][4 * q], O[t][4 * q + 1], O[t][4 * q + 2], O[t][4 * q + 3]};
    if (h == 0) {
        ml[(obase + qq) * 2] = (m_run - (float)H3_PSHIFT) * 0.6931471805599453f;
        ml[(obase + qq) * 2 + 1] = l_run;
    }
}

template <int WS>
constexpr size_t attention_h3_ws_lds_bytes() { return (size_t)WS * (H3_KTB + H3_VTB); }

template <int WS, bool PACKED>
__global__ __launch_bounds__(WS * 64) void attention_h3_ws_kernel(
    const _Float16 *__restrict__ Qs, const _Float16 *__restrict__ Ks, const _Float16 *__restrict__ Vs,
    const float *__restrict__ vexp, const float *__restrict__ M, AttnGridH3 g, float *__restrict__ opart,
    float *__restrict__ ml) {
    extern __shared__ __attribute__((aligned(16))) char h3smem[];
    const AttnBlock blk = attention_h3_block(g, true);
    if (blk.qb * 32 >= g.n(blk.b)) return;
    const int b = blk.b, split = blk.split, Npad = g.Npad;
    const int tid = threadIdx.x, wave = __builtin_amdgcn_readfirstlane(tid >> 6), lane = tid & 63, h = lane >> 5;
    const int q0 = blk.qb * 32, qq = q0 + (lane & 31);
    f32x16 O[4];
    float m_run, l_run;
    attention_h3_core<1, PACKED, false, WS>(Qs, Ks, Vs, vexp, M, g, blk, h3smem, wave, lane, O, m_run, l_run);
    float *rec = reinterpret_cast<float *>(h3smem + wave * (H3_KTB + H3_VTB));
    __builtin_amdgcn_s_waitcnt(0xc07f);
#pragma unroll
    for (int t = 0; t < 4; ++t)
#pragma unroll
        for (int r = 0; r < 16; ++r) rec[(16 * t + r) * 64 + lane] = O[t][r];
    rec[4096 + lane] = m_run;
    rec[4096 + 64 + lane] = l_run;
    __syncthreads();
    if (q0 >= Npad) return;
    float mw[WS], ms = -INFINITY;
#pragma unroll
    for (int w = 0; w < WS; ++w) {
        mw[w] = reinterpret_cast<const float *>(h3smem + w * (H3_KTB + H3_VTB))[4096 + lane];
        ms = fmaxf(ms, mw[w]);
    }
    float a[WS];
#pragma unroll
    for (int w = 0; w < WS; ++w) a[w] = ms == -INFINITY ? 0.0f : __builtin_amdgcn_exp2f(mw[w] - ms);
    const size_t obase = (size_t)(b * g.nsplit + split) * Npad;
    float *Ob = opart + obase * CH + (size_t)(q0 >> 5) * (H3_TILE * CH) + 4 * lane;
    for (int t = wave; t < 4; t += WS) {
        float acc[16];
#pragma unroll
        for (int r = 0; r < 16; ++r) acc[r] = 0.0f;
#pragma unroll
        for (int w = 0; w < WS; ++w) {
            const float *rw = reinterpret_cast<const float *>(h3smem + w * (H3_KTB + H3_VTB));
#pragma unroll
            for (int r = 0; r < 16; ++r) acc[r] = __builtin_fmaf(a[w], rw[(16 * t + r) * 64 + lane], acc[r]);
        }
#pragma unroll
        for (int q = 0; q < 4; ++q)
            *reinterpret_cast<f32x4 *>(Ob + (4 * t + q) * 256) = f32x4{acc[4 * q], acc[4 * q + 1], acc[4 * q + 2], acc[4 * q + 3]};
    }
    if (wave == 0 && h == 0) {
        float l = 0.0f;
#pragma unroll
        for (int w = 0; w < WS; ++w)
            l = __builtin_fmaf(a[w], reinterpret_cast<const float *>(h3smem + w * (H3_KTB + H3_VTB))[4096 + 64 + lane], l);
        ml[(obase + qq) * 2] = (ms - (float)H3_PSHIFT) * 0.6931471805599453f;
        ml[(obase + qq) * 2 + 1] = l;
    }
}

static __global__ __launch_bounds__(256) void vexp_kernel(const float *__restrict__ v, int N, int ld, int Npad,
                                                         float *__restrict__ vexp) {
    __shared__ float part[4];
    const int t = blockIdx.x, b = blockIdx.y, tid = threadIdx.x;
    float m = 0.0f;
    for (int e = tid; e < H3_TILE * CH; e += 256) {
        const int row = t * H3_TILE + e / CH;
        if (row < N) m = fmaxf(m, fabsf(v[((size_t)b * ld + row) * CH + e % CH]));
    }
    m = wave_max(m);
    if ((tid & 63) == 0) part[tid >> 6] = m;
    __syncthreads();
    if (tid == 0) vexp[(size_t)b * (Npad / H3_TILE) + t] = (float)h3_vexp(fmaxf(fmaxf(part[0], part[1]), fmaxf(part[2], part[3])));
}

static __global__ void split_qkv_kernel(const float *__restrict__ q, const float *__restrict__ k,
                                 const float *__restrict__ v, const float *__restrict__ vexp, int B, int N,
                                 int ld, int Npad, _Float16 *__restrict__ Qs, _Float16 *__restrict__ Ks,
                                 _Float16 *__restrict__ Vs) {
    const size_t i = (size_t)blockIdx.x * blockDim.x + threadIdx.x;
    if (i >= (size_t)B * Npad * CH) return;
    const int c = (int)(i % CH);
    const int row = (int)((i / CH) % Npad);
    const int b = (int)(i / CH / Npad);
    const size_t src = ((size_t)b * ld + row) * CH + c, pb = (size_t)b * Npad * 2 * CH;
    const bool in = row < N;
    _Float16 hi, lo;
    split_h(in ? (ATT_QFMA ? q[src] * H3_QSCALE : q[src]) : 0.0f, hi, lo);
    Qs[pb + qs_off(row, 0, c)] = hi;
    Qs[pb + qs_off(row, 1, c)] = lo;
    split_h(in ? k[src] : 0.0f, hi, lo);
    Ks[pb + ks_off(row, 0, c)] = hi;
    Ks[pb + ks_off(row, 1, c)] = lo;
    const float ev = vexp[(size_t)b * (Npad / H3_TILE) + row / H3_TILE];
    split_h(in ? ldexpf(v[src], (int)ev) : 0.0f, hi, lo);
    Vs[pb + vs_off(row, 0, c)] = hi;
    Vs[pb + vs_off(row, 1, c)] = lo;
}

}
```

### pointdsc_amd/csrc/attention_plan.hpp

```cpp
#pragma once
#include <cstdlib>

#include "pdsc_internal.hpp"

namespace pdsc {

inline int env_int(const char *name, int dflt) {
    const char *e = getenv(name);
    return e ? atoi(e) : dflt;
}

struct AttnKnobs {
    int target;
    int nw;
    int tiny;
    int tiny_slots;
    int ws;
    int w64;
    bool w64_sk;
    bool fuse;
    int pw2;
    bool precombine;
    int zigzag;
    bool dense_m;
};
inline const AttnKnobs &attn_knobs() {
    static const AttnKnobs k = [] {
        AttnKnobs v;
        const int t = env_int("PDSC_ATT_TARGET", 0), nw = env_int("PDSC_ATT_NW", 2), ws = env_int("PDSC_ATT_WS", 4),
                  sl = env_int("PDSC_ATT_TINY_SLOTS", 0);
        v.target = t > 0 ? t : 512;
        v.nw = (nw == 1 || nw == 2) ? nw : 4;
        v.tiny = env_int("PDSC_ATT_TINY", 16);
        v.tiny_slots = sl > 0 ? sl : 128;
        v.ws = (ws == 1 || ws == 2) ? ws : 4;
        v.w64 = env_int("PDSC_W64", 2);
        v.w64_sk = env_int("PDSC_W64_SK", 1) != 0;
        v.fuse = env_int("PDSC_FUSE", 1) != 0;
        v.pw2 = env_int("PDSC_PW2", 1);
        v.precombine = env_int("PDSC_PRECOMBINE", 1) != 0;
        v.zigzag = env_int("PDSC_ZIGZAG", 1);
        v.dense_m = env_int("PDSC_DENSE_M", 0) == 1;
        return v;
    }();
    return k;
}

#ifndef PW2_WAVES
#define PW2_WAVES 4
#endif
constexpr int PW2_W = PW2_WAVES;
constexpr int PW2_PTS = PW2_W * 32;

inline bool use_pw2(int B, int Npad, bool f32) {
    const int mode = attn_knobs().pw2;
    if (f32 || mode == 0) return false;
    return mode == 2 || (long)B * ((Npad + PW2_PTS - 1) / PW2_PTS) >= 320;
}

enum AttnKind {
    ATT_FUSED,
    ATT_F32,
    ATT_H3,
    ATT_H3_WS,
    ATT_W64,
    ATT_W64_SK,
};

struct EncoderPlan {
    AttnKind kind;
    int B, N, Npad;
    bool f32;
    int nw;
    int ws;
    bool early;
    int sk_wgs;
    int nqb;
    int sps;
    int nsplit;
    bool precombine;
    int m_layout;

    bool fused() const { return kind == ATT_FUSED; }
    bool w64() const { return kind == ATT_W64 || kind == ATT_W64_SK; }

    EncoderPlan for_ragged(const Ragged &rg) const {
        EncoderPlan p = *this;
        if (kind == ATT_W64_SK && rg.nv && !rg.eq) {
            p.kind = ATT_W64;
            p.sk_wgs = 0;
        }
        return p;
    }
    EncoderPlan for_pairs(int nb) const {
        EncoderPlan p = *this;
        p.B = nb;
        return p;
    }

    int rev(const Ragged &rg, int layer) const {
        const int mode = attn_knobs().zigzag;
        if (rg.po || kind == ATT_W64_SK) return 0;
        return mode == 0 ? 0 : mode == 2 ? !(layer & 1) : (layer & 1);
    }
    int workgroups() const { return kind == ATT_W64_SK ? sk_wgs : B * nqb * (fused() ? 1 : nsplit); }
};

EncoderPlan plan_encoder(int B, int N, bool f32, bool dense_m_caller, bool allow_fused = true);

}
```

### pointdsc_amd/csrc/encoder.hip

```cpp
#include <cstdlib>
#include <type_traits>

#include "attention.hpp"
#include "attention_h3.hpp"
#include "attention_plan.hpp"
#include "attention_w64.hpp"

namespace pdsc {

__global__ __launch_bounds__(256) void wscale_kernel(const float *__restrict__ w, int n, int f32,
                                                     float *__restrict__ sc) {
    __shared__ float part[4];
    if (f32) {
        if (threadIdx.x == 0) sc[0] = sc[1] = 1.0f;
        return;
    }
    float m = 0.0f;
    for (int i = threadIdx.x; i < n; i += 256) m = fmaxf(m, fabsf(w[i]));
    m = wave_max(m);
    if ((threadIdx.x & 63) == 0) part[threadIdx.x >> 6] = m;
    __syncthreads();
    if (threadIdx.x == 0) {
        m = fmaxf(fmaxf(part[0], part[1]), fmaxf(part[2], part[3]));
        int ex = 0;
        if (m > 0.0f && m < INFINITY) frexpf(m, &ex);
        const int sh = max(-100, min(100, 14 - ex));
        sc[0] = ldexpf(1.0f, -sh);
        sc[1] = ldexpf(1.0f, sh);
    }
}

__global__ void pack_dense_kernel(const float *__restrict__ w, const float *__restrict__ b,
                                  const float *__restrict__ bn_w, const float *__restrict__ bn_b,
                                  const float *__restrict__ bn_rm, const float *__restrict__ bn_rv,
                                  int in, int out, int f32, float *__restrict__ dw, float *__restrict__ db,
                                  float *__restrict__ da, float *__restrict__ dbeta,
                                  const float *__restrict__ sc) {
    const int i = blockIdx.x * blockDim.x + threadIdx.x;
    const int total = in * out;
    if (i < total && f32) {
        dw[i] = w[i];
    } else if (i < total) {
        _Float16 *wd = reinterpret_cast<_Float16 *>(dw);
        const int o = i / in, c = i % in;
        float x = w[i] * sc[1];
        asm("" : "+v"(x));
        const _Float16 hi = (_Float16)x;
        const float r1 = x - (float)hi;
        const _Float16 mid = (_Float16)r1;
        const size_t d = w3_index(o, c, in);
        wd[d] = hi;
        wd[d + 512] = mid;
        if (W_PLANES == 3) wd[d + 1024] = (_Float16)(r1 - (float)mid);
    }
    if (i < out) {
        db[i] = b[i];
        if (bn_w) {
            const float invstd = 1.0f / sqrtf(bn_rv[i] + 1e-5f);
            const float alpha = invstd * bn_w[i];
            da[i] = alpha;
            dbeta[i] = bn_b[i] - bn_rm[i] * alpha;
        } else {
            da[i] = 1.0f;
            dbeta[i] = 0.0f;
        }
    }
}

__global__ void copy_kernel(const float *__restrict__ s, float *__restrict__ d, int n) {
    const int i = blockIdx.x * blockDim.x + threadIdx.x;
    if (i < n) d[i] = s[i];
}

hipError_t launch_pack_dense(const float *w, const float *b, const float *bn_w, const float *bn_b,
                             const float *bn_rm, const float *bn_rv, int in, int out, bool f32, float *dst_w,
                             float *dst_b, float *dst_a, float *dst_beta, float *dst_scale, hipStream_t s) {
    const int n = in * out;
    hipLaunchKernelGGL(wscale_kernel, dim3(1), dim3(256), 0, s, w, n, (int)f32, dst_scale);
    hipLaunchKernelGGL(pack_dense_kernel, dim3((n + 255) / 256), dim3(256), 0, s, w, b, bn_w, bn_b,
                       bn_rm, bn_rv, in, out, (int)f32, dst_w, dst_b, dst_a, dst_beta, dst_scale);
    return hipGetLastError();
}

hipError_t launch_copy(const float *src, float *dst, int n, hipStream_t s) {
    hipLaunchKernelGGL(copy_kernel, dim3((n + 255) / 256), dim3(256), 0, s, src, dst, n);
    return hipGetLastError();
}

constexpr int ATT_NW = 4;
constexpr int ATT_F32_KTS = 32;

EncoderPlan plan_encoder(int B, int N, bool f32, bool dense_m_caller, bool allow_fused) {
    const AttnKnobs &k = attn_knobs();
    EncoderPlan p{};
    p.B = B;
    p.N = N;
    p.Npad = round_up(N, QB);
    p.f32 = f32;
    p.nw = ATT_NW;
    p.ws = 1;
    const int nst = (N + H3_TILE - 1) / H3_TILE;
    const long blocks = (long)B * ((N + QB - 1) / QB);
    auto take = [&p](AttnKind kind, const auto &g) {
        p.kind = kind;
        p.nqb = g.nqb;
        p.sps = g.sps;
        p.nsplit = g.nsplit;
    };

    const AttnGridH3 fg = attention_h3_grid<PW2_W>(B, N, k.target * 4 / PW2_W);
    const bool fused = allow_fused && k.fuse && use_pw2(B, p.Npad, f32) && fg.nsplit == 1 && fg.nqb * PW2_PTS == p.Npad;

    const bool w64 = !fused && !f32 && !dense_m_caller && k.w64 != 0 &&
                     (k.w64 == 1 || (long)B * ((N + W64_QPB - 1) / W64_QPB) >= 128);
    if (f32) {
        take(ATT_F32, attention_grid<ATT_NW, ATT_F32_KTS>(B, N, k.target));
    } else if (w64) {
        const int nwg = k.target / 2;
        const AttnGridH3 g = attention_w64_grid(B, N, nwg);
        take(ATT_W64, g);
        const long T = (long)B * g.nqb * nst, rounds = ((long)B * g.nqb * g.nsplit + nwg - 1) / nwg;
        if (k.w64_sk && T >= 4L * nwg && (T + nwg - 1) / nwg + 2 < rounds * g.sps) {
            p.kind = ATT_W64_SK;
            p.sk_wgs = nwg;
            p.nsplit = std::max(g.nsplit, w64_sk_nsplit(B, g.nqb, nst, nwg));
        }
    } else {
        const AttnGridH3 tg = attention_h3_grid<1>(B, N, std::min(k.target, k.tiny_slots));
        if (blocks <= k.tiny && tg.sps <= 24) {
            const bool wave_split = k.ws > 1 && tg.sps >= 4;
            take(wave_split ? ATT_H3_WS : ATT_H3, tg);
            p.nw = 1;
            p.ws = wave_split ? k.ws : 1;
        } else {
            p.nw = blocks <= 16 ? k.nw : ATT_NW;
            take(ATT_H3, p.nw == 1   ? attention_h3_grid<1>(B, N, k.target)
                         : p.nw == 2 ? attention_h3_grid<2>(B, N, k.target)
                                     : attention_h3_grid<ATT_NW>(B, N, k.target));
        }
        p.early = p.kind == ATT_H3 && p.sps >= 3;
    }

    p.precombine = k.precombine && !f32 && !fused && p.nsplit >= 16 && blocks <= 16;
    p.m_layout = w64 || !(f32 || dense_m_caller || k.dense_m) ? M_PACKED : M_DENSE;

    if (fused) {
        p.kind = ATT_FUSED;
        p.nw = PW2_W;
        p.ws = 1;
        p.early = false;
        p.nqb = fg.nqb;
        p.sps = nst;
    }
    return p;
}

static AttnGridH3 plan_grid_h3(const EncoderPlan &plan, const Ragged &rg, int layer) {
    const bool sk = plan.kind == ATT_W64_SK;
    return AttnGridH3{plan.B, plan.N, plan.Npad, plan.nqb, plan.fused() ? 1 : plan.nsplit, plan.sps,
                      sk ? nullptr : rg.nv, sk ? nullptr : rg.po, plan.rev(rg, layer)};
}

template <typename F> static void with_bool(bool b, F &&f) { b ? f(std::true_type{}) : f(std::false_type{}); }
template <int V, int... Vs, typename F> static void with_int(int v, F &&f) {
    if (v == V) f(std::integral_constant<int, V>{});
    else if constexpr (sizeof...(Vs) > 0) with_int<Vs...>(v, f);
}

hipError_t launch_attention(const EncoderPlan &plan, const void *q, const void *k, const void *v, const float *vexp,
                            const float *M, float *opart, float *ml, hipStream_t s, Ragged rg, int layer) {
    const dim3 grid(plan.workgroups());
    const _Float16 *qs = static_cast<const _Float16 *>(q), *ks = static_cast<const _Float16 *>(k),
                   *vs = static_cast<const _Float16 *>(v);
    const AttnGridH3 g = plan_grid_h3(plan, rg, layer);
    const bool packed = plan.m_layout == M_PACKED;
    switch (plan.kind) {
    case ATT_W64_SK:
        hipLaunchKernelGGL((attention_w64_sk_kernel<true>), grid, dim3(W64_NW * 64), W64_LDS, s, qs, ks, vs, vexp, M, g,
                           plan.sk_wgs, opart, ml);
        break;
    case ATT_W64:
        hipLaunchKernelGGL((attention_w64_kernel<true>), grid, dim3(W64_NW * 64), W64_LDS, s, qs, ks, vs, vexp, M, g,
                           opart, ml);
        break;
    case ATT_F32: {
        const AttnGrid gf{plan.B, plan.N, plan.Npad, plan.nqb, plan.nsplit, plan.sps, rg.nv};
        hipLaunchKernelGGL((attention_kernel_t<ATT_NW, ATT_F32_KTS, false, true>), grid, dim3(ATT_NW * 64),
                           (attention_lds_bytes<ATT_NW, ATT_F32_KTS>()), s, static_cast<const float *>(q),
                           static_cast<const float *>(k), static_cast<const float *>(v), M, gf, opart, ml);
        break;
    }
    case ATT_H3_WS:
        with_int<2, 4>(plan.ws, [&](auto ws) {
            with_bool(packed, [&](auto pk) {
                constexpr int WS = decltype(ws)::value;
                hipLaunchKernelGGL((attention_h3_ws_kernel<WS, decltype(pk)::value>), grid, dim3(WS * 64),
                                   attention_h3_ws_lds_bytes<WS>(), s, qs, ks, vs, vexp, M, g, opart, ml);
            });
        });
        break;
    case ATT_H3:
        with_int<1, 2, ATT_NW>(plan.nw, [&](auto nw) {
            with_bool(plan.early, [&](auto early) {
                with_bool(packed, [&](auto pk) {
                    constexpr int NW = decltype(nw)::value;
                    hipLaunchKernelGGL((attention_h3_kernel<NW, true, decltype(pk)::value, decltype(early)::value>), grid,
                                       dim3(NW * 64), attention_h3_lds_bytes<NW>(), s, qs, ks, vs, vexp, M, g, opart,
                                       ml);
                });
            });
        });
        break;
    default: return hipErrorInvalidValue;
    }
    return hipGetLastError();
}

__global__ void pad_rows_kernel(const float *__restrict__ x, int B, int N, int Npad, float *__restrict__ y) {
    const size_t i = (size_t)blockIdx.x * blockDim.x + threadIdx.x;
    if (i >= (size_t)B * Npad * CH) return;
    const int c = (int)(i % CH), row = (int)((i / CH) % Npad), b = (int)(i / CH / Npad);
    y[i] = row < N ? x[((size_t)b * N + row) * CH + c] : 0.0f;
}

hipError_t launch_pad_rows(const float *x, int B, int N, int Npad, float *y, hipStream_t s) {
    const size_t n = (size_t)B * Npad * CH;
    hipLaunchKernelGGL(pad_rows_kernel, dim3((unsigned)((n + 255) / 256)), dim3(256), 0, s, x, B, N, Npad, y);
    return hipGetLastError();
}

hipError_t launch_split_qkv(const float *q, const float *k, const float *v, int B, int N, int ld, int Npad,
                            _Float16 *qs, _Float16 *ks, _Float16 *vs, float *vexp, hipStream_t s) {
    const size_t n = (size_t)B * Npad * CH;
    hipLaunchKernelGGL(vexp_kernel, dim3(Npad / H3_TILE, B), dim3(256), 0, s, v, N, ld, Npad, vexp);
    hipLaunchKernelGGL(split_qkv_kernel, dim3((unsigned)((n + 255) / 256)), dim3(256), 0, s, q, k, v, vexp, B, N, ld,
                       Npad, qs, ks, vs);
    return hipGetLastError();
}

#ifndef PDSC_C16_ONE
#define PDSC_C16_ONE 8
#endif
constexpr int C16_ONE = PDSC_C16_ONE;
template <bool F32>
PDSC_DEV void combine16(const float *__restrict__ opart, const float *__restrict__ ml, int b,
                        int nsplit, int Npad, int row, int d0, float out[16]) {
    const float *mlb = ml + ((size_t)b * nsplit * Npad + row) * 2;
    if (nsplit <= C16_ONE) {
        f32x2 mlv[C16_ONE > 0 ? C16_ONE : 1];
        f32x4 ov[C16_ONE > 0 ? C16_ONE : 1][4];
#pragma unroll
        for (int j = 0; j < C16_ONE; ++j) {
            if (j < nsplit) {
                const size_t base = (size_t)(b * nsplit + j) * Npad + row;
                mlv[j] = *reinterpret_cast<const f32x2 *>(ml + base * 2);
                const float *ob = opart + (base - row) * CH;
#pragma unroll
                for (int i = 0; i < 4; ++i) {
                    const size_t o = F32 ? (size_t)row * CH + d0 + 4 * i : h3_opart_off(row, d0 + 4 * i);
                    ov[j][i] = *reinterpret_cast<const f32x4 *>(ob + o);
                }
            }
        }
        float mstar = -INFINITY;
#pragma unroll
        for (int j = 0; j < C16_ONE; ++j)
            if (j < nsplit) mstar = fmaxf(mstar, mlv[j][0]);
        float L = 0.0f;
        f32x4 acc[4] = {};
#pragma unroll
        for (int j = 0; j < C16_ONE; ++j) {
            if (j < nsplit) {
                const float w = expf(mlv[j][0] - mstar);
                L += w * mlv[j][1];
#pragma unroll
                for (int i = 0; i < 4; ++i) acc[i] += w * ov[j][i];
            }
        }
#pragma unroll
        for (int i = 0; i < 4; ++i)
#pragma unroll
            for (int e = 0; e < 4; ++e) out[4 * i + e] = acc[i][e] / L;
        return;
    }
    float mstar = -INFINITY;
    for (int s0 = 0; s0 < nsplit; s0 += 8) {
        float mv[8];
#pragma unroll
        for (int j = 0; j < 8; ++j) mv[j] = s0 + j < nsplit ? mlb[(size_t)(s0 + j) * Npad * 2] : -INFINITY;
#pragma unroll
        for (int j = 0; j < 8; ++j) mstar = fmaxf(mstar, mv[j]);
    }
    float L = 0.0f;
    f32x4 acc[4] = {};
    constexpr int SB = 4;
    for (int s0 = 0; s0 < nsplit; s0 += SB) {
        f32x2 mlv[SB];
        f32x4 ov[SB][4];
#pragma unroll
        for (int j = 0; j < SB; ++j) {
            if (s0 + j < nsplit) {
                const size_t base = (size_t)(b * nsplit + s0 + j) * Npad + row;
                mlv[j] = *reinterpret_cast<const f32x2 *>(ml + base * 2);
                const float *ob = opart + (base - row) * CH;
#pragma unroll
                for (int i = 0; i < 4; ++i) {
                    const size_t o = F32 ? (size_t)row * CH + d0 + 4 * i : h3_opart_off(row, d0 + 4 * i);
                    ov[j][i] = *reinterpret_cast<const f32x4 *>(ob + o);
                }
            }
        }
#pragma unroll
        for (int j = 0; j < SB; ++j) {
            if (s0 + j < nsplit) {
                const float w = expf(mlv[j][0] - mstar);
                L += w * mlv[j][1];
#pragma unroll
                for (int i = 0; i < 4; ++i) acc[i] += w * ov[j][i];
            }
        }
    }
#pragma unroll
    for (int i = 0; i < 4; ++i)
#pragma unroll
        for (int e = 0; e < 4; ++e) out[4 * i + e] = acc[i][e] / L;
}

template <bool F32>
__global__ __launch_bounds__(256) void attn_combine_kernel(const float *__restrict__ opart,
                                                           const float *__restrict__ ml, int N,
                                                           int Npad, int nsplit,
                                                           float *__restrict__ msg) {
    const int b = blockIdx.y;
    const int row = blockIdx.x * 32 + (threadIdx.x >> 3), d0 = (threadIdx.x & 7) * 16;
    if (row >= N) return;
    float out[16];
    combine16<F32>(opart, ml, b, nsplit, Npad, row, d0, out);
    f32x4 *dst = reinterpret_cast<f32x4 *>(msg + ((size_t)b * N + row) * CH + d0);
#pragma unroll
    for (int i = 0; i < 4; ++i) dst[i] = f32x4{out[4 * i], out[4 * i + 1], out[4 * i + 2], out[4 * i + 3]};
}

hipError_t launch_attn_combine(const float *opart, const float *ml, bool f32, int B, int N, int Npad,
                               int nsplit, float *msg, hipStream_t s) {
    if (f32)
        hipLaunchKernelGGL(attn_combine_kernel<true>, dim3((N + 31) / 32, B), dim3(256), 0, s, opart, ml, N, Npad,
                           nsplit, msg);
    else
        hipLaunchKernelGGL(attn_combine_kernel<false>, dim3((N + 31) / 32, B), dim3(256), 0, s, opart, ml, N, Npad,
                           nsplit, msg);
    return hipGetLastError();
}

constexpr int CMB_SB = 16;
// ... 699 lines not shown
static void w2_sched_add(W2Sched &S, const DenseOff &o, int in, int out) {
    const int nks = in / 16, nt = w2_nt(in, out);
    for (int c = 0; c < out / 32 / nt; ++c) {
        S.off[S.n] = (uint32_t)(2 * o.w + (size_t)c * nt * nks * W3_BLOCK);
        S.np[S.n] = W_PLANES * nt * nks;
        ++S.n;
    }
}

PDSC_DEV void w2_stage(const float *pk, const W2Sched &S, int c, char *slot, int wave, int lane) {
    if (c >= S.n) return;
#if ATT_BUFDMA
    const __amdgpu_buffer_rsrc_t r = h3_rsrc(pk, 0xFFFFFFFFu);
    for (int i = wave; i < S.np[c]; i += PW2_W)
        __builtin_amdgcn_raw_ptr_buffer_load_lds(r, (__attribute__((address_space(3))) void *)(slot + 1024 * i), 16,
                                                 16 * lane, (int)(2 * S.off[c]) + 1024 * i, 0, 0);
#else
    const _Float16 *src = reinterpret_cast<const _Float16 *>(pk) + S.off[c] + 8 * lane;
    for (int i = wave; i < S.np[c]; i += PW2_W)
        __builtin_amdgcn_global_load_lds(src + 512 * i, slot + 1024 * i, 16, 0, 0);
#endif
}

struct W2Pipe {
    char *base;
    int c;
    PDSC_DEV char *slot(int k) const { return base + (k % PW2_NSLOT) * PW2_SLOT; }
};

template <int NST>
PDSC_DEV void w2_sync(bool active) {
    if (NST > 0 && active)
        asm volatile("s_waitcnt vmcnt(%0) lgkmcnt(0)\n\ts_barrier" ::"n"(NST) : "memory");
    else
        asm volatile("s_waitcnt vmcnt(0) lgkmcnt(0)\n\ts_barrier" ::: "memory");
}

PDSC_DEV void w2_frag(const char *bp, f16x8 (&w)[3]) {
    w[0] = *reinterpret_cast<const f16x8 *>(bp);
    w[1] = *reinterpret_cast<const f16x8 *>(bp + 1024);
    if constexpr (W_PLANES == 3) w[2] = *reinterpret_cast<const f16x8 *>(bp + 2048);
}

template <int NKS, int NT, bool TRANS, int NACC>
PDSC_DEV void w2_mma(const char *slot, const f16x8 *xh, const f16x8 *xl, f32x16 (&acc)[NACC], int t0, int lane) {
    constexpr int NB = NT * NKS;
    const char *bp = slot + 16 * lane;
    f16x8 w[3][3];
    w2_frag(bp, w[0]);
    if (NB > 1) w2_frag(bp + PW2_BLKB, w[1]);
#pragma unroll
    for (int j = 0; j < NB; ++j) {
        if (j + 2 < NB) w2_frag(bp + (j + 2) * PW2_BLKB, w[(j + 2) % 3]);
        const int t = j / NKS, ks = j % NKS;
        const f16x8(&f)[3] = w[j % 3];
        const f32x16 c = ks == 0 ? zero16() : acc[t0 + t];
        acc[t0 + t] = TRANS ? mfma_w3x(f[0], f[1], f[2], xh[ks], xl[ks], c) : mfma_xw3(xh[ks], xl[ks], f[0], f[1], f[2], c);
        __builtin_amdgcn_sched_barrier(0);
    }
}

template <int IN, int OUT, bool TRANS, int NST = 0>
PDSC_DEV void w2_layer(W2Pipe &P, const float *pk, const W2Sched &S, const f16x8 *xh, const f16x8 *xl,
                       f32x16 (&acc)[OUT / 32], bool active, int wave, int lane) {
    constexpr int NKS = IN / 16, NT = w2_nt(IN, OUT), NCH = OUT / 32 / NT;
    static_assert(NCH * NT == OUT / 32, "chunk tiling");
#pragma unroll
    for (int c = 0; c < NCH; ++c) {
        CH_STAMP(192 + 3 * min(P.c, 20));
        if (active) w2_mma<NKS, NT, TRANS>(P.slot(P.c), xh, xl, acc, c * NT, lane);
        CH_STAMP(193 + 3 * min(P.c, 20));
        if (c == 0)
            w2_sync<NST>(active);
        else
            w2_sync<0>(active);
        CH_STAMP(194 + 3 * min(P.c, 20));
        w2_stage(pk, S, P.c + PW2_NSLOT, P.slot(P.c), wave, lane);
        asm volatile("" ::: "memory");
        ++P.c;
    }
}

PDSC_DEV void w2_coef(float *dst, const float *__restrict__ pk, const DenseOff &o, int out, int tid) {
    for (int i = tid; i < 3 * out; i += PW2_W * 64) dst[i] = pk[o.bias + i];
}

PDSC_DEV void split8v(const float (&v)[8], f16x8 &hi, f16x8 &lo) { split8x(v, hi, lo); }

PDSC_DEV int w2_chan(int t, int u, int e, int h) { return 32 * t + 16 * u + 8 * (e >> 2) + 4 * h + (e & 3); }

template <int OUT, int EPI, bool SPLIT = true>
PDSC_DEV void w2_epilogue(f32x16 (&acc)[OUT / 32], float inv, const float *cf, const f32x16 *resid, f16x8 *xh,
                          f16x8 *xl, int lane) {
    const int h = lane >> 5;
#pragma unroll
    for (int t = 0; t < OUT / 32; ++t)
#pragma unroll
        for (int u = 0; u < 2; ++u) {
            const int c0 = 32 * t + 16 * u + 4 * h;
            const f32x4 b0 = *reinterpret_cast<const f32x4 *>(cf + c0), b1 = *reinterpret_cast<const f32x4 *>(cf + c0 + 8);
            f32x4 a0, a1, e0, e1;
            if (EPI == EPI_BN_RELU) {
                a0 = *reinterpret_cast<const f32x4 *>(cf + OUT + c0);
                a1 = *reinterpret_cast<const f32x4 *>(cf + OUT + c0 + 8);
                e0 = *reinterpret_cast<const f32x4 *>(cf + 2 * OUT + c0);
                e1 = *reinterpret_cast<const f32x4 *>(cf + 2 * OUT + c0 + 8);
            }
            float v[8];
#pragma unroll
            for (int e = 0; e < 8; ++e) {
                const int r = 8 * u + e;
                float y = __builtin_fmaf(acc[t][r], inv, e < 4 ? b0[e] : b1[e - 4]);
                if (EPI == EPI_BN_RELU) y = relu_nan(y * (e < 4 ? a0[e] : a1[e - 4]) + (e < 4 ? e0[e] : e1[e - 4]));
                if (EPI == EPI_RELU) y = relu_nan(y);
                if (EPI == EPI_RESID) y = resid[t][r] + y;
                acc[t][r] = y;
                v[e] = y;
            }
            if constexpr (SPLIT) split8v(v, xh[2 * t + u], xl[2 * t + u]);
        }
}

PDSC_DEV void w2_combine(const float *__restrict__ opart, const float *__restrict__ ml, int b, int nsplit, int Npad,
                         int row, f16x8 *xh, f16x8 *xl, int lane) {
    float mstar = -INFINITY;
    for (int s = 0; s < nsplit; ++s) mstar = fmaxf(mstar, ml[((size_t)(b * nsplit + s) * Npad + row) * 2]);
    float L = 0.0f;
    f32x4 acc[16];
#pragma unroll
    for (int i = 0; i < 16; ++i) acc[i] = f32x4{0.0f, 0.0f, 0.0f, 0.0f};
    for (int s = 0; s < nsplit; ++s) {
        const size_t base = (size_t)(b * nsplit + s) * Npad + row;
        const float ms = ml[base * 2];
        if (ms == -INFINITY) continue;
        const float w = expf(ms - mstar);
        L += w * ml[base * 2 + 1];
        const float *src = opart + (base - (row & 31)) * CH + 4 * lane;
#pragma unroll
        for (int i = 0; i < 16; ++i) acc[i] += w * *reinterpret_cast<const f32x4 *>(src + 256 * i);
    }
    const float rl = 1.0f / L;
#pragma unroll
    for (int ks = 0; ks < 8; ++ks) {
        float v[8];
#pragma unroll
        for (int e = 0; e < 4; ++e) {
            v[e] = acc[2 * ks][e] * rl;
            v[4 + e] = acc[2 * ks + 1][e] * rl;
        }
        split8v(v, xh[ks], xl[ks]);
    }
}

PDSC_DEV void w2_msg_frags(const f32x16 (&O)[4], float l_run, f16x8 *xh, f16x8 *xl) {
    const float rl = 1.0f / l_run;
#pragma unroll
    for (int ks = 0; ks < 8; ++ks) {
        float v[8];
#pragma unroll
        for (int e = 0; e < 8; ++e) v[e] = O[ks >> 1][8 * (ks & 1) + e] * rl;
        split8v(v, xh[ks], xl[ks]);
    }
}

PDSC_DEV void w2_load_row(const float *__restrict__ featL, int row, int lane, f32x16 (&y)[4]) {
    const f32x4 *src = reinterpret_cast<const f32x4 *>(featL + (size_t)(row >> 5) * (32 * CH)) + lane;
#pragma unroll
    for (int t = 0; t < 4; ++t)
#pragma unroll
        for (int q = 0; q < 4; ++q) {
            const f32x4 v = src[64 * (4 * t + q)];
#pragma unroll
            for (int e = 0; e < 4; ++e) y[t][4 * q + e] = v[e];
        }
}
PDSC_DEV void w2_store_row(float *__restrict__ featL, int row, int lane, const f32x16 (&y)[4]) {
    f32x4 *dst = reinterpret_cast<f32x4 *>(featL + (size_t)(row >> 5) * (32 * CH)) + lane;
#pragma unroll
    for (int t = 0; t < 4; ++t)
#pragma unroll
        for (int q = 0; q < 4; ++q) dst[64 * (4 * t + q)] = f32x4{y[t][4 * q], y[t][4 * q + 1], y[t][4 * q + 2], y[t][4 * q + 3]};
}

template <bool QSCALE>
PDSC_DEV void w2_store_qk(const f32x16 (&acc)[4], float inv, const float *bias, _Float16 *__restrict__ dst, int row,
                          int lane) {
    const int h = lane >> 5;
    _Float16 *dtile = dst + (size_t)(row >> 5) * H3_TILE_H;
#pragma unroll
    for (int t = 0; t < 4; ++t)
#pragma unroll
        for (int u = 0; u < 2; ++u) {
            const int c0 = 32 * t + 16 * u + 4 * h;
            const f32x4 b0 = *reinterpret_cast<const f32x4 *>(bias + c0), b1 = *reinterpret_cast<const f32x4 *>(bias + c0 + 8);
            float v[8];
#pragma unroll
            for (int e = 0; e < 8; ++e) {
                v[e] = __builtin_fmaf(acc[t][8 * u + e], inv, e < 4 ? b0[e] : b1[e - 4]);
                if (QSCALE && ATT_QFMA) v[e] *= H3_QSCALE;
            }
            f16x8 hi, lo;
            split8v(v, hi, lo);
            *reinterpret_cast<f16x8 *>(dtile + h3_frag(2 * t + u, 0, lane)) = hi;
            *reinterpret_cast<f16x8 *>(dtile + h3_frag(2 * t + u, 1, lane)) = lo;
        }
}

PDSC_DEV void w2_store_v(f32x16 (&acc)[4], float inv, const float *bias, _Float16 *__restrict__ Vt,
                         float *__restrict__ vexp_t, int lane) {
    const int h = lane >> 5, l32 = lane & 31;
    float m = 0.0f;
#pragma unroll
    for (int t = 0; t < 4; ++t) {
        const float bs = bias[32 * t + l32];
#pragma unroll
        for (int r = 0; r < 16; ++r) {
            acc[t][r] = __builtin_fmaf(acc[t][r], inv, bs);
            m = fmaxf(m, fabsf(acc[t][r]));
        }
    }
    const int ev = h3_vexp(wave_max(m));
    if (lane == 0) *vexp_t = (float)ev;
#pragma unroll
    for (int t = 0; t < 4; ++t) {
#pragma unroll
        for (int s = 0; s < 2; ++s) {
            float v[8];
#pragma unroll
            for (int e = 0; e < 8; ++e) v[e] = ldexpf(acc[t][8 * s + e], ev);
            f16x8 hi, lo;
            split8v(v, hi, lo);
            *reinterpret_cast<f16x8 *>(Vt + h3_frag(2 * t + s, 0, lane)) = hi;
            *reinterpret_cast<f16x8 *>(Vt + h3_frag(2 * t + s, 1, lane)) = lo;
        }
    }
}

struct W2CoefQKV {
    static constexpr int pcn = 0, q = 3 * CH, k = 4 * CH, v = 5 * CH, end = 6 * CH;
};
PDSC_DEV void w2_coef_qkv(float *cf, const float *pk, const PwDense4 &d, int tid) {
    w2_coef(cf + W2CoefQKV::pcn, pk, d.pcn, CH, tid);
    for (int i = tid; i < CH; i += PW2_W * 64) {
        cf[W2CoefQKV::q + i] = pk[d.q.bias + i];
        cf[W2CoefQKV::k + i] = pk[d.k.bias + i];
        cf[W2CoefQKV::v + i] = pk[d.v.bias + i];
    }
}

PDSC_DEV void w2_pcn_qkv(W2Pipe &P, const float *__restrict__ pk, const W2Sched &S, const float *cf, const PwDense4 &d,
                         const f16x8 *xh, const f16x8 *xl, float *__restrict__ featL, _Float16 *__restrict__ Q,
                         _Float16 *__restrict__ K, _Float16 *__restrict__ V, float *__restrict__ vexp, int row,
                         bool active, int wave, int lane) {
    const int h = lane >> 5;
    f32x16 acc[4];
    f16x8 yh[8], yl[8];
    const float sp = pk[d.pcn.scale], sq = pk[d.q.scale], sk = pk[d.k.scale], sv = pk[d.v.scale];
    w2_layer<CH, CH, true>(P, pk, S, xh, xl, acc, active, wave, lane);
    if (active) {
        w2_epilogue<CH, EPI_BN_RELU>(acc, sp, cf + W2CoefQKV::pcn, nullptr, yh, yl, lane);
        w2_store_row(featL, row, lane, acc);
    }
    CH_STAMP(175);
    w2_layer<CH, CH, true, 16>(P, pk, S, yh, yl, acc, active, wave, lane);
    if (active) w2_store_qk<true>(acc, sq, cf + W2CoefQKV::q, Q, row, lane);
    CH_STAMP(176);
    w2_layer<CH, CH, true, 16>(P, pk, S, yh, yl, acc, active, wave, lane);
    if (active) w2_store_qk<false>(acc, sk, cf + W2CoefQKV::k, K, row, lane);
    CH_STAMP(177);
    w2_layer<CH, CH, false, 16>(P, pk, S, yh, yl, acc, active, wave, lane);
    if (active) w2_store_v(acc, sv, cf + W2CoefQKV::v, V + (size_t)(row >> 5) * H3_TILE_H, vexp + (row >> 5), lane);
    CH_STAMP(178);
}

struct W2CoefMid {
    static constexpr int f0 = W2CoefQKV::end, f3 = f0 + 3 * CH2, f6 = f3 + 3 * CH2, end = f6 + 3 * CH;
};
static_assert(W2CoefMid::end <= PW2_COEF, "coefficient table");
PDSC_DEV void w2_coef_mid(float *cf, const float *__restrict__ pk, const PwMsg &m, const PwDense4 &d, int tid) {
    w2_coef_qkv(cf, pk, d, tid);
    w2_coef(cf + W2CoefMid::f0, pk, m.fc0, CH2, tid);
    w2_coef(cf + W2CoefMid::f3, pk, m.fc3, CH2, tid);
    w2_coef(cf + W2CoefMid::f6, pk, m.fc6, CH, tid);
}

PDSC_DEV void w2_mid_chain(W2Pipe &P, const float *__restrict__ pk, const W2Sched &S, const float *cf, const PwMsg &m,
                           const PwDense4 &d, f16x8 *xh, f16x8 *xl, const float *featL_in, float *featL,
                           _Float16 *__restrict__ Q, _Float16 *__restrict__ K, _Float16 *__restrict__ V,
                           float *__restrict__ vexp, int row, bool active, int wave, int lane) {
    f32x16 a2[2], a4[4], res[4];
    f16x8 yh[8], yl[8];
    w2_layer<CH, CH2, true>(P, pk, S, xh, xl, a2, active, wave, lane);
    if (active) w2_epilogue<CH2, EPI_BN_RELU>(a2, pk[m.fc0.scale], cf + W2CoefMid::f0, nullptr, yh, yl, lane);
    CH_STAMP(172);
    w2_layer<CH2, CH2, true>(P, pk, S, yh, yl, a2, active, wave, lane);
    if (active) {
        w2_epilogue<CH2, EPI_BN_RELU>(a2, pk[m.fc3.scale], cf + W2CoefMid::f3, nullptr, xh, xl, lane);
        w2_load_row(featL_in, row, lane, res);
    }
    CH_STAMP(173);
    w2_layer<CH2, CH, true, 16>(P, pk, S, xh, xl, a4, active, wave, lane);
    if (active) w2_epilogue<CH, EPI_RESID>(a4, pk[m.fc6.scale], cf + W2CoefMid::f6, res, yh, yl, lane);
    CH_STAMP(174);
    w2_pcn_qkv(P, pk, S, cf, d, yh, yl, featL, Q, K, V, vexp, row, active, wave, lane);
}

#define PW2_PROLOGUE                                                                              \
    extern __shared__ __attribute__((aligned(16))) char w2smem[];                                 \
    const int b = blockIdx.y, tid = threadIdx.x, wave = tid >> 6, lane = tid & 63, h = lane >> 5; \
    const int row = blockIdx.x * PW2_PTS + wave * 32 + (lane & 31);                               \
    const bool active = blockIdx.x * PW2_PTS + wave * 32 < Npad;                \
    const size_t boff = (size_t)b * Npad * CH;                                                    \
    W2Pipe P{w2smem, 0};                                                                          \
    float *cf = reinterpret_cast<float *>(w2smem + PW2_NSLOT * PW2_SLOT);                         \
    for (int c_ = 0; c_ < PW2_NSLOT; ++c_) w2_stage(pk, S, c_, P.slot(c_), wave, lane);

__global__ __launch_bounds__(PW2_W * 64, PW2_OCC) void pw2_first_kernel(const float *__restrict__ pk, W2Sched S, size_t l0w,
                                                                 size_t l0b, PwDense4 d, const float *__restrict__ corr,
                                                                 int in_dim, int N, int Npad, float *__restrict__ featL,
                                                                 _Float16 *__restrict__ Q, _Float16 *__restrict__ K,
                                                                 _Float16 *__restrict__ V, float *__restrict__ vexp,
                                                                 const int *__restrict__ nv) {
    if (nv && (int)blockIdx.x * PW2_PTS >= nv[blockIdx.y]) return;
    PW2_PROLOGUE
    const int l32 = lane & 31;
    const int n = nv ? nv[b] : N;
    w2_coef_qkv(cf, pk, d, tid);
    f16x8 xh[8], xl[8];
    if (active) {
        const float *cp = corr + ((size_t)b * N + min(row, n - 1)) * in_dim;
        const bool in = row < n;
        f32x16 acc[4] = {zero16(), zero16(), zero16(), zero16()};
        for (int j = 0; j < (in_dim + 1) / 2; ++j) {
            const int i = 2 * j + h;
            const float x = (in && i < in_dim) ? cp[i] : 0.0f;
#pragma unroll
            for (int t = 0; t < 4; ++t) {
                const float w = i < in_dim ? pk[l0w + (32 * t + l32) * in_dim + i] : 0.0f;
                acc[t] = mfma32(w, x, acc[t]);
            }
        }
#pragma unroll
        for (int t = 0; t < 4; ++t)
#pragma unroll
            for (int u = 0; u < 2; ++u) {
                float v[8];
#pragma unroll
                for (int e = 0; e < 8; ++e) v[e] = acc[t][8 * u + e] + pk[l0b + w2_chan(t, u, e, h)];
                split8v(v, xh[2 * t + u], xl[2 * t + u]);
            }
    }
    __syncthreads();
    w2_pcn_qkv(P, pk, S, cf, d, xh, xl, featL + boff, Q + 2 * boff, K + 2 * boff, V + 2 * boff,
               vexp + (size_t)b * (Npad / 32), row, active, wave, lane);
}

__global__ __launch_bounds__(PW2_W * 64, PW2_OCC) void pw2_mid_kernel(const float *__restrict__ pk, W2Sched S, PwMsg m,
                                                               PwDense4 d, const float *__restrict__ opart,
                                                               const float *__restrict__ ml, int nsplit, int N,
                                                               int Npad, const float *__restrict__ featL_in,
                                                               float *__restrict__ featL,
                                                               _Float16 *__restrict__ Q, _Float16 *__restrict__ K,
                                                               _Float16 *__restrict__ V, float *__restrict__ vexp) {
    PW2_PROLOGUE
    w2_coef_mid(cf, pk, m, d, tid);
    f16x8 xh[8], xl[8];
    if (active) w2_combine(opart, ml, b, nsplit, Npad, row, xh, xl, lane);
    __syncthreads();
    w2_mid_chain(P, pk, S, cf, m, d, xh, xl, featL_in + boff, featL + boff, Q + 2 * boff, K + 2 * boff,
                 V + 2 * boff, vexp + (size_t)b * (Npad / 32), row, active, wave, lane);
}

template <bool PACKED>
__global__ __launch_bounds__(PW2_W * 64, PW2_OCC) void attn_pw2_kernel(
    const _Float16 *__restrict__ Qs, const _Float16 *__restrict__ Ks, const _Float16 *__restrict__ Vs,
    const float *__restrict__ vexp_in, const float *__restrict__ M, AttnGridH3 g, const float *__restrict__ pk,
    W2Sched S, PwMsg m, PwDense4 d, float *__restrict__ featL, _Float16 *__restrict__ Q, _Float16 *__restrict__ K,
    _Float16 *__restrict__ V, float *__restrict__ vexp) {
    extern __shared__ __attribute__((aligned(16))) char w2smem[];
    const AttnBlock blk = attention_h3_block(g, true);
    if (blk.qb * PW2_PTS >= g.n(blk.b)) return;
    const int b = blk.b, Npad = g.Npad, tid = threadIdx.x, wave = __builtin_amdgcn_readfirstlane(tid >> 6),
              lane = tid & 63;
    const int row = blk.qb * PW2_PTS + wave * 32 + (lane & 31);
    const bool active = blk.qb * PW2_PTS + wave * 32 < Npad;
    const size_t boff = (size_t)b * Npad * CH;
#ifdef ATT_STAMPS
    unsigned long long *stp = att_stamp_ptr(wave);
    ATT_RSTAMP(stp, 188);
    ATT_STAMP(stp, 0);
#endif
    f32x16 O[4];
    float m_run, l_run;
    attention_h3_core<PW2_W, PACKED, PW2_EARLY>(Qs, Ks, Vs, vexp_in, M, g, blk, w2smem, wave, lane, O, m_run, l_run);
    ATT_STAMP(stp, 170);
    W2Pipe P{w2smem, 0};
    float *cf = reinterpret_cast<float *>(w2smem + PW2_NSLOT * PW2_SLOT);
    for (int c = 0; c < PW2_NSLOT; ++c) w2_stage(pk, S, c, P.slot(c), wave, lane);
    w2_coef_mid(cf, pk, m, d, tid);
    f16x8 xh[8], xl[8];
    if (active) w2_msg_frags(O, l_run, xh, xl);
    __syncthreads();
    ATT_STAMP(stp, 171);
    w2_mid_chain(P, pk, S, cf, m, d, xh, xl, featL + boff, featL + boff, Q + 2 * boff, K + 2 * boff,
                 V + 2 * boff, vexp + (size_t)b * (Npad / 32), row, active, wave, lane);
    ATT_STAMP(stp, 180);
    ATT_RSTAMP(stp, 189);
}

#ifdef ATT_STAMPS
extern "C" int pdsc_diag_att_stamps(void *host, size_t bytes) {
    const size_t n = std::min(bytes, sizeof(g_att_stamps));
    return hipMemcpyFromSymbol(host, HIP_SYMBOL(g_att_stamps), n, 0, hipMemcpyDeviceToHost) == hipSuccess ? 0 : -1;
}
extern "C" int pdsc_diag_att_stamps_clear() {
    static unsigned long long zero[ST_WGS * 4 * ST_PER_WAVE];
    return hipMemcpyToSymbol(HIP_SYMBOL(g_att_stamps), zero, sizeof(zero), 0, hipMemcpyHostToDevice) == hipSuccess ? 0
                                                                                                             : -1;
}
#endif

struct W2CoefLast {
    static constexpr int f0 = 0, f3 = f0 + 3 * CH2, f6 = f3 + 3 * CH2, c0 = f6 + 3 * CH, c2 = c0 + 3 * CLS,
                         c4 = c2 + 3 * CLS, end = c4 + CLS;
};
static_assert(W2CoefLast::end <= PW2_COEF, "coefficient table");
PDSC_DEV void w2_coef_last(float *cf, const float *__restrict__ pk, const PwMsg &m, const DenseOff &c0,
                           const DenseOff &c2, size_t c4w, int tid) {
    w2_coef(cf + W2CoefLast::f0, pk, m.fc0, CH2, tid);
    w2_coef(cf + W2CoefLast::f3, pk, m.fc3, CH2, tid);
    w2_coef(cf + W2CoefLast::f6, pk, m.fc6, CH, tid);
    w2_coef(cf + W2CoefLast::c0, pk, c0, CLS, tid);
    w2_coef(cf + W2CoefLast::c2, pk, c2, CLS, tid);
    for (int i = tid; i < CLS; i += PW2_W * 64) cf[W2CoefLast::c4 + i] = pk[c4w + i];
}

PDSC_DEV void w2_last_chain(W2Pipe &P, const float *__restrict__ pk, const W2Sched &S, const float *cf, const PwMsg &m,
                            const DenseOff &c0, const DenseOff &c2, size_t c4b, f16x8 *xh, f16x8 *xl,
                            const float *__restrict__ featL, float *__restrict__ feat_out, float *__restrict__ normed,
                            _Float16 *__restrict__ normed_s, float *__restrict__ conf, int b, int N, int row,
                            bool active, int wave, int lane) {
    constexpr int CF0 = W2CoefLast::f0, CF3 = W2CoefLast::f3, CF6 = W2CoefLast::f6, CC0 = W2CoefLast::c0,
                  CC2 = W2CoefLast::c2, CC4 = W2CoefLast::c4;
    const int h = lane >> 5;
    f32x16 a1[1], a2[2], a4[4], res[4];
    f16x8 yh[8], yl[8];
    w2_layer<CH, CH2, true>(P, pk, S, xh, xl, a2, active, wave, lane);
    if (active) w2_epilogue<CH2, EPI_BN_RELU>(a2, pk[m.fc0.scale], cf + CF0, nullptr, yh, yl, lane);
    w2_layer<CH2, CH2, true>(P, pk, S, yh, yl, a2, active, wave, lane);
    if (active) {
        w2_epilogue<CH2, EPI_BN_RELU>(a2, pk[m.fc3.scale], cf + CF3, nullptr, xh, xl, lane);
        w2_load_row(featL, row, lane, res);
    }
    w2_layer<CH2, CH, true, 16>(P, pk, S, xh, xl, a4, active, wave, lane);
    const bool in = row < N;
    if (active) {
        w2_epilogue<CH, EPI_RESID>(a4, pk[m.fc6.scale], cf + CF6, res, yh, yl, lane);
        float ss = 0.0f;
#pragma unroll
        for (int t = 0; t < 4; ++t)
#pragma unroll
            for (int r = 0; r < 16; ++r) ss = __builtin_fmaf(a4[t][r], a4[t][r], ss);
        ss = halves_sum(ss);
        const float den = fmaxf(sqrtf(ss), 1e-12f);
        if (in) {
            float *dst = normed + ((size_t)b * N + row) * CH;
            _Float16 *ds = normed_s ? normed_s + ((size_t)b * N + row) * 2 * CH : nullptr;
#pragma unroll
            for (int t = 0; t < 4; ++t)
#pragma unroll
                for (int u = 0; u < 2; ++u) {
                    float v[8];
#pragma unroll
                    for (int e = 0; e < 8; ++e) v[e] = a4[t][8 * u + e] / den;
                    *reinterpret_cast<f32x4 *>(dst + 32 * t + 16 * u + 4 * h) = f32x4{v[0], v[1], v[2], v[3]};
                    *reinterpret_cast<f32x4 *>(dst + 32 * t + 16 * u + 8 + 4 * h) = f32x4{v[4], v[5], v[6], v[7]};
                    if (ds) {
                        f16x8 hi, lo;
                        split8v(v, hi, lo);
                        const int chk = 4 * t + 2 * u + h;
                        *reinterpret_cast<f16x8 *>(ds + 8 * chk) = hi;
                        *reinterpret_cast<f16x8 *>(ds + CH + 8 * chk) = lo;
                    }
                }
            if (feat_out) {
                float *fo = feat_out + ((size_t)b * N + row) * CH;
#pragma unroll
                for (int t = 0; t < 4; ++t)
#pragma unroll
                    for (int g = 0; g < 4; ++g)
                        *reinterpret_cast<f32x4 *>(fo + 32 * t + 8 * g + 4 * h) =
                            f32x4{a4[t][4 * g], a4[t][4 * g + 1], a4[t][4 * g + 2], a4[t][4 * g + 3]};
            }
        }
    }
    w2_layer<CH, CLS, true>(P, pk, S, yh, yl, a1, active, wave, lane);
    if (active) w2_epilogue<CLS, EPI_RELU>(a1, pk[c0.scale], cf + CC0, nullptr, xh, xl, lane);
    w2_layer<CLS, CLS, true>(P, pk, S, xh, xl, a1, active, wave, lane);
    if (active) {
        w2_epilogue<CLS, EPI_RELU, false>(a1, pk[c2.scale], cf + CC2, nullptr, nullptr, nullptr, lane);
        float s = 0.0f;
#pragma unroll
        for (int u = 0; u < 2; ++u)
#pragma unroll
            for (int e = 0; e < 8; ++e) s = __builtin_fmaf(cf[CC4 + w2_chan(0, u, e, h)], a1[0][8 * u + e], s);
        s = halves_sum(s);
        if (in && h == 0) conf[(size_t)b * N + row] = s + pk[c4b];
    }
}

__global__ __launch_bounds__(PW2_W * 64, PW2_OCC) void pw2_last_kernel(
    const float *__restrict__ pk, W2Sched S, PwMsg m, DenseOff c0, DenseOff c2, size_t c4w, size_t c4b,
    const float *__restrict__ opart, const float *__restrict__ ml, int nsplit, int N, int Npad,
    const float *__restrict__ featL, float *__restrict__ feat_out, float *__restrict__ normed,
    _Float16 *__restrict__ normed_s, float *__restrict__ conf) {
    PW2_PROLOGUE
    w2_coef_last(cf, pk, m, c0, c2, c4w, tid);
    f16x8 xh[8], xl[8];
    if (active) w2_combine(opart, ml, b, nsplit, Npad, row, xh, xl, lane);
    __syncthreads();
    w2_last_chain(P, pk, S, cf, m, c0, c2, c4b, xh, xl, featL + boff, feat_out, normed, normed_s, conf, b, N, row,
                  active, wave, lane);
}

template <bool PACKED>
__global__ __launch_bounds__(PW2_W * 64, PW2_OCC) void attn_pw2_last_kernel(
    const _Float16 *__restrict__ Qs, const _Float16 *__restrict__ Ks, const _Float16 *__restrict__ Vs,
    const float *__restrict__ vexp_in, const float *__restrict__ M, AttnGridH3 g, const float *__restrict__ pk,
    W2Sched S, PwMsg m, DenseOff c0, DenseOff c2, size_t c4w, size_t c4b, const float *__restrict__ featL,
    float *__restrict__ feat_out, float *__restrict__ normed, _Float16 *__restrict__ normed_s,
    float *__restrict__ conf) {
    extern __shared__ __attribute__((aligned(16))) char w2smem[];
    const AttnBlock blk = attention_h3_block(g, true);
    if (blk.qb * PW2_PTS >= g.n(blk.b)) return;
    const int b = blk.b, N = g.N, Npad = g.Npad, tid = threadIdx.x, wave = __builtin_amdgcn_readfirstlane(tid >> 6),
              lane = tid & 63;
    const int row = blk.qb * PW2_PTS + wave * 32 + (lane & 31);
    const bool active = blk.qb * PW2_PTS + wave * 32 < Npad;
    f32x16 O[4];
    float m_run, l_run;
    attention_h3_core<PW2_W, PACKED, PW2_EARLY>(Qs, Ks, Vs, vexp_in, M, g, blk, w2smem, wave, lane, O, m_run, l_run);
    W2Pipe P{w2smem, 0};
    float *cf = reinterpret_cast<float *>(w2smem + PW2_NSLOT * PW2_SLOT);
    for (int c = 0; c < PW2_NSLOT; ++c) w2_stage(pk, S, c, P.slot(c), wave, lane);
    w2_coef_last(cf, pk, m, c0, c2, c4w, tid);
    f16x8 xh[8], xl[8];
    if (active) w2_msg_frags(O, l_run, xh, xl);
    __syncthreads();
    w2_last_chain(P, pk, S, cf, m, c0, c2, c4b, xh, xl, featL + (size_t)b * Npad * CH, feat_out, normed, normed_s,
                  conf, b, N, row, active, wave, lane);
}
#undef PW2_PROLOGUE

static W2Sched sched_qkv(W2Sched S, const PwDense4 &d) {
    w2_sched_add(S, d.pcn, CH, CH);
    w2_sched_add(S, d.q, CH, CH);
    w2_sched_add(S, d.k, CH, CH);
    w2_sched_add(S, d.v, CH, CH);
    return S;
}
static W2Sched sched_msg(const PwMsg &m) {
    W2Sched S{};
    w2_sched_add(S, m.fc0, CH, CH2);
    w2_sched_add(S, m.fc3, CH2, CH2);
    w2_sched_add(S, m.fc6, CH2, CH);
    return S;
}

static PwDense4 dense4(const LayerOff &l) { return PwDense4{l.pcn, l.q, l.k, l.v}; }
static PwMsg msg3(const LayerOff &l) { return PwMsg{l.fc0, l.fc3, l.fc6}; }

hipError_t launch_attn_pw2(const EncoderPlan &plan, const float *packed, const PackLayout &lay, int layer,
                           const void *q, const void *k, const void *v, const float *vexp_in, const float *M,
                           float *feat, void *qo, void *ko, void *vo, float *vexp_out, hipStream_t s, Ragged rg) {
    if (!plan.fused() || layer + 1 >= lay.L) return hipErrorInvalidValue;
    const AttnGridH3 g = plan_grid_h3(plan, rg, layer);
    const W2Sched S = sched_qkv(sched_msg(msg3(lay.layer[layer])), dense4(lay.layer[layer + 1]));
    const size_t lds = std::max(attention_h3_lds_bytes<PW2_W>(), PW2_LDS);
    const _Float16 *qs = static_cast<const _Float16 *>(q), *ks = static_cast<const _Float16 *>(k),
                   *vs = static_cast<const _Float16 *>(v);
    _Float16 *Q = static_cast<_Float16 *>(qo), *K = static_cast<_Float16 *>(ko), *V = static_cast<_Float16 *>(vo);
    with_bool(plan.m_layout == M_PACKED, [&](auto pk) {
        hipLaunchKernelGGL(attn_pw2_kernel<decltype(pk)::value>, dim3(plan.workgroups()), dim3(PW2_W * 64), lds, s, qs,
                           ks, vs, vexp_in, M, g, packed, S, msg3(lay.layer[layer]), dense4(lay.layer[layer + 1]), feat,
                           Q, K, V, vexp_out);
    });
    return hipGetLastError();
}

hipError_t launch_attn_pw2_last(const EncoderPlan &plan, const float *packed, const PackLayout &lay, const void *q,
                                const void *k, const void *v, const float *vexp_in, const float *M, const float *feat,
                                float *feat_out, float *normed, _Float16 *normed_s, float *conf, hipStream_t s,
                                Ragged rg) {
    if (!plan.fused()) return hipErrorInvalidValue;
    const AttnGridH3 g = plan_grid_h3(plan, rg, lay.L - 1);
    W2Sched S = sched_msg(msg3(lay.layer[lay.L - 1]));
    w2_sched_add(S, lay.c0, CH, CLS);
    w2_sched_add(S, lay.c2, CLS, CLS);
    const size_t lds = std::max(attention_h3_lds_bytes<PW2_W>(), PW2_LDS);
    const _Float16 *qs = static_cast<const _Float16 *>(q), *ks = static_cast<const _Float16 *>(k),
                   *vs = static_cast<const _Float16 *>(v);
    const PwMsg m = msg3(lay.layer[lay.L - 1]);
    with_bool(plan.m_layout == M_PACKED, [&](auto pk) {
        hipLaunchKernelGGL(attn_pw2_last_kernel<decltype(pk)::value>, dim3(plan.workgroups()), dim3(PW2_W * 64), lds, s,
                           qs, ks, vs, vexp_in, M, g, packed, S, m, lay.c0, lay.c2, lay.c4_w, lay.c4_b, feat, feat_out,
                           normed, normed_s, conf);
    });
    return hipGetLastError();
}

static bool small_tiles(int B, int Npad) {
    static const long lim = [] {
        const char *e = getenv("PDSC_PW_SMALL_LIMIT");
        return e ? atol(e) : 512L;
    }();
    return (long)B * (Npad / 64) < lim;
}

static bool pw_waves8(int B, int Npad) {
    static const bool off = [] {
        const char *e = getenv("PDSC_PW_WAVES");
        return e && atoi(e) == 4;
    }();
    return !off && (long)B * (Npad / 32) <= 256;
}

static bool pw_qkv_split(int B, int Npad) {
    static const bool off = [] {
        const char *e = getenv("PDSC_PW_QKV_SPLIT");
        return e && e[0] == '0';
    }();
    return !off && 3L * B * (Npad / 32) <= 256;
}

#define PW_LAUNCH(K, rows, ...)                                                                         \
    do {                                                                                                \
        const bool st_ = small_tiles(B, Npad);                                                          \
        const int pt_ = st_ ? 32 : 64;                                                                  \
        const dim3 g_(((rows) + pt_ - 1) / pt_, B);                                                     \
        if (st_ && f32)                                                                                 \
            hipLaunchKernelGGL((K<32, true>), g_, dim3(256), pw_lds<32>(), s, __VA_ARGS__);             \
        else if (st_)                                                                                   \
            hipLaunchKernelGGL((K<32, false>), g_, dim3(256), pw_lds<32>(), s, __VA_ARGS__);            \
        else if (f32)                                                                                   \
            hipLaunchKernelGGL((K<64, true>), g_, dim3(256), pw_lds<64>(), s, __VA_ARGS__);             \
        else                                                                                            \
            hipLaunchKernelGGL((K<64, false>), g_, dim3(256), pw_lds<64>(), s, __VA_ARGS__);            \
    } while (0)

hipError_t launch_pw_first(const float *packed, const PackLayout &lay, const float *corr_pos, bool f32, int B,
                           int N, int Npad, float *feat, void *q, void *k, void *v, float *vexp, hipStream_t s,
                           Ragged rg, bool fused) {
    if (lay.in_dim > IN_LIMIT) return hipErrorInvalidValue;
    _Float16 *Q = static_cast<_Float16 *>(q), *K = static_cast<_Float16 *>(k), *V = static_cast<_Float16 *>(v);
    if (fused || use_pw2(B, Npad, f32)) {
        const W2Sched S = sched_qkv(W2Sched{}, dense4(lay.layer[0]));
        hipLaunchKernelGGL(pw2_first_kernel, dim3((Npad + PW2_PTS - 1) / PW2_PTS, B), dim3(PW2_W * 64), PW2_LDS, s,
                           packed, S, lay.l0_w, lay.l0_b, dense4(lay.layer[0]), corr_pos, lay.in_dim, N, Npad, feat, Q, K,
                           V, vexp, rg.nv);
        return hipGetLastError();
    }
    if (!f32 && small_tiles(B, Npad) && pw_qkv_split(B, Npad)) {
        hipLaunchKernelGGL((pw_first_kernel<32, false>), dim3(Npad / 32, B, 3), dim3(256), pw_lds<32>(), s, packed,
                           lay.l0_w, lay.l0_b, dense4(lay.layer[0]), corr_pos, lay.in_dim, N, Npad, feat, Q, K, V, vexp,
                           rg.nv);
        return hipGetLastError();
    }
    PW_LAUNCH(pw_first_kernel, Npad, packed, lay.l0_w, lay.l0_b, dense4(lay.layer[0]), corr_pos, lay.in_dim, N, Npad,
              feat, Q, K, V, vexp, rg.nv);
    return hipGetLastError();
}

hipError_t launch_pw_mid(const float *packed, const PackLayout &lay, int layer, bool f32, const float *opart,
                         const float *ml, int nsplit, int B, int N, int Npad, const float *feat_in, float *feat,
                         void *q, void *k, void *v, float *vexp, hipStream_t s) {
    const int delay = g_diag_qkv_delay;
    _Float16 *Q = static_cast<_Float16 *>(q), *K = static_cast<_Float16 *>(k), *V = static_cast<_Float16 *>(v);
    if (use_pw2(B, Npad, f32)) {
        const W2Sched S = sched_qkv(sched_msg(msg3(lay.layer[layer])), dense4(lay.layer[layer + 1]));
        hipLaunchKernelGGL(pw2_mid_kernel, dim3((Npad + PW2_PTS - 1) / PW2_PTS, B), dim3(PW2_W * 64), PW2_LDS, s,
                           packed, S, msg3(lay.layer[layer]), dense4(lay.layer[layer + 1]), opart, ml, nsplit, N, Npad,
                           feat_in, feat, Q, K, V, vexp);
        return hipGetLastError();
    }
    if (!f32 && pw_waves8(B, Npad)) {
        hipLaunchKernelGGL((pw_mid_kernel<32, false, 8>), dim3(Npad / 32, B, pw_qkv_split(B, Npad) ? 3 : 1), dim3(512),
                           pw_lds<32>(), s, packed,
                           msg3(lay.layer[layer]), dense4(lay.layer[layer + 1]), opart, ml, nsplit, N, Npad, feat_in,
                           feat, Q, K, V, vexp, delay, (int)pw_prefetch_on());
        return hipGetLastError();
    }
    PW_LAUNCH(pw_mid_kernel, Npad, packed, msg3(lay.layer[layer]), dense4(lay.layer[layer + 1]), opart, ml, nsplit,
              N, Npad, feat_in, feat, Q, K, V, vexp, 0, 0);
    return hipGetLastError();
}

hipError_t launch_pw_last(const float *packed, const PackLayout &lay, bool f32, const float *opart,
                          const float *ml, int nsplit, int B, int N, int Npad, const float *feat,
                          float *feat_out, float *normed, _Float16 *normed_s, float *conf, hipStream_t s) {
    if (use_pw2(B, Npad, f32)) {
        W2Sched S = sched_msg(msg3(lay.layer[lay.L - 1]));
        w2_sched_add(S, lay.c0, CH, CLS);
        w2_sched_add(S, lay.c2, CLS, CLS);
        hipLaunchKernelGGL(pw2_last_kernel, dim3((Npad + PW2_PTS - 1) / PW2_PTS, B), dim3(PW2_W * 64), PW2_LDS, s,
                           packed, S, msg3(lay.layer[lay.L - 1]), lay.c0, lay.c2, lay.c4_w, lay.c4_b, opart, ml, nsplit, N,
                           Npad, feat, feat_out, normed, normed_s, conf);
        return hipGetLastError();
    }
    PW_LAUNCH(pw_last_kernel, N, packed, msg3(lay.layer[lay.L - 1]), lay.c0, lay.c2, lay.c4_w, lay.c4_b, opart, ml,
              nsplit, N, Npad, feat, feat_out, normed, normed_s, conf);
    return hipGetLastError();
}
#undef PW_LAUNCH
}
```

### pointdsc_amd/csrc/pdsc_internal.hpp

```cpp
#pragma once
#include <string>
#include "pdsc_common.hpp"
#include "../../include/pdsc.h"

namespace pdsc {

constexpr int CH = 128;
constexpr int CH2 = CH / 2;
constexpr int CLS = 32;
constexpr int QB = 128;
constexpr int KT = 32;
constexpr int PT = 64;

inline int round_up(int x, int m) { return (x + m - 1) / m * m; }

constexpr int MPACK_T = 32;
__host__ __device__ inline int mpack_ntile(int N) { return (N + MPACK_T - 1) / MPACK_T; }
__host__ __device__ inline size_t mpack_floats(int N) {
    const size_t nt = mpack_ntile(N);
    return nt * (nt + 1) / 2 * MPACK_T * MPACK_T;
}
__host__ __device__ inline int mpack_tile(int ti, int tj, int nt) { return ti * nt - ti * (ti - 1) / 2 + (tj - ti); }
inline size_t align_bytes(size_t x) { return (x + 255) & ~size_t(255); }

#ifndef PDSC_W_PLANES
#define PDSC_W_PLANES 2
#endif
constexpr int W_PLANES = PDSC_W_PLANES;
static_assert(W_PLANES == 2 || W_PLANES == 3, "weight planes");

constexpr int W3_BLOCK = W_PLANES * 512;
__host__ __device__ inline size_t w3_index(int o, int c, int in) {
    const int t = o >> 5, n = o & 31, ks = c >> 4, q = c & 15;
    const int pos = (q & ~12) | ((q & 4) << 1) | ((q & 8) >> 1);
    return ((size_t)t * (in / 16) + ks) * W3_BLOCK + (size_t)(32 * (pos >> 3) + n) * 8 + (pos & 7);
}

struct DenseOff {
    size_t w, bias, alpha, beta, scale;
};

struct LayerOff {
    DenseOff pcn, fc0, fc3, fc6, q, k, v;
};

struct PackLayout {
    int L, in_dim;
    size_t sigma, sigma_d;
    size_t l0_w, l0_b;
    size_t cls0, cls2;
    DenseOff c0, c2;
    size_t c4_w, c4_b;
    size_t total;
    LayerOff layer[64];
};

inline DenseOff dense_at(size_t &o, int in, int out) {
    DenseOff d;
    d.w = o;
    o += (size_t)out * in * (W_PLANES > 2 ? W_PLANES : 2) / 2;
    d.bias = o;
    o += out;
    d.alpha = o;
    o += out;
    d.beta = o;
    o += out;
    o = (o + 3) & ~size_t(3);
    d.scale = o;
    o += 4;
    return d;
}

inline PackLayout make_layout(int L, int in_dim) {
    PackLayout p{};
    p.L = L;
    p.in_dim = in_dim;
    size_t o = 0;
    p.sigma = 0;
    p.sigma_d = 1;
    o = 16;
    p.l0_w = o;
    o += (size_t)CH * in_dim;
    p.l0_b = o;
    o += CH;
    o = (o + 3) & ~size_t(3);
    for (int l = 0; l < L; ++l) {
        LayerOff &lo = p.layer[l];
        lo.pcn = dense_at(o, CH, CH);
        lo.fc0 = dense_at(o, CH, CH2);
        lo.fc3 = dense_at(o, CH2, CH2);
        lo.fc6 = dense_at(o, CH2, CH);
        lo.q = dense_at(o, CH, CH);
        lo.k = dense_at(o, CH, CH);
        lo.v = dense_at(o, CH, CH);
    }
    p.c0 = dense_at(o, CH, CLS);
    p.c2 = dense_at(o, CLS, CLS);
    p.c4_w = o;
    o += CLS;
    p.c4_b = o;
    o += 4;
    p.total = o;
    return p;
}

extern thread_local int g_diag_qkv_delay;
struct Ragged {
    const int *nv = nullptr, *sv = nullptr;
    const int *po = nullptr;
    bool eq = false;
    PDSC_DEV int n(int b, int N) const { return nv ? nv[b] : N; }
    PDSC_DEV int s(int b, int S) const { return sv ? sv[b] : S; }
};
constexpr int RAGGED_CHUNK = 512;
hipError_t launch_ragged_setup(const int32_t *counts_host, int B, double ratio, int *nv, int *sv, hipStream_t s);
hipError_t launch_ragged_order(const int32_t *counts_host, int B, int *po, hipStream_t s);

hipError_t launch_compat(const float *src, const float *tgt, int B, int N, const float *sigma_d,
                         float *M, hipStream_t s, Ragged rg = {});
hipError_t launch_compat_packed(const float *src, const float *tgt, int B, int N, const float *sigma_d,
                                float *Mp, hipStream_t s, Ragged rg = {});

hipError_t launch_pack_dense(const float *w, const float *b, const float *bn_w, const float *bn_b,
                             const float *bn_rm, const float *bn_rv, int in, int out, bool f32, float *dst_w,
                             float *dst_b, float *dst_a, float *dst_beta, float *dst_scale, hipStream_t s);
hipError_t launch_copy(const float *src, float *dst, int n, hipStream_t s);

enum MLayout { M_DENSE = 0, M_PACKED = 1 };
struct EncoderPlan;
hipError_t launch_attention(const EncoderPlan &plan, const void *q, const void *k, const void *v, const float *vexp,
                            const float *M, float *opart, float *ml, hipStream_t s, Ragged rg = {}, int layer = 0);
hipError_t launch_attn_pw2(const EncoderPlan &plan, const float *packed, const PackLayout &lay, int layer,
                           const void *q, const void *k, const void *v, const float *vexp_in, const float *M,
                           float *feat, void *qo, void *ko, void *vo, float *vexp_out, hipStream_t s, Ragged rg = {});
hipError_t launch_attn_pw2_last(const EncoderPlan &plan, const float *packed, const PackLayout &lay, const void *q,
                                const void *k, const void *v, const float *vexp_in, const float *M, const float *feat,
                                float *feat_out, float *normed, _Float16 *normed_s, float *conf, hipStream_t s,
                                Ragged rg = {});
hipError_t launch_pad_rows(const float *x, int B, int N, int Npad, float *y, hipStream_t s);
hipError_t launch_split_qkv(const float *q, const float *k, const float *v, int B, int N, int ld, int Npad,
                            _Float16 *qs, _Float16 *ks, _Float16 *vs, float *vexp, hipStream_t s);
hipError_t launch_attn_combine(const float *opart, const float *ml, bool f32, int B, int N, int Npad,
                               int nsplit, float *msg, hipStream_t s);

hipError_t launch_pw_first(const float *packed, const PackLayout &lay, const float *corr_pos, bool f32, int B,
                           int N, int Npad, float *feat, void *q, void *k, void *v, float *vexp, hipStream_t s,
                           Ragged rg = {}, bool fused = false);
hipError_t launch_combine_rows(const float *opart, const float *ml, int B, int Npad, int nsplit, float *opart1,
                               float *ml1, hipStream_t s);
hipError_t launch_pw_mid(const float *packed, const PackLayout &lay, int layer, bool f32, const float *opart,
                         const float *ml, int nsplit, int B, int N, int Npad, const float *feat_in, float *feat,
                         void *q, void *k, void *v, float *vexp, hipStream_t s);
hipError_t launch_pw_last(const float *packed, const PackLayout &lay, bool f32, const float *opart,
                          const float *ml, int nsplit, int B, int N, int Npad, const float *feat,
                          float *feat_out, float *normed, _Float16 *normed_s, float *conf, hipStream_t s);

hipError_t launch_local_max(const float *src, const float *conf, int B, int N, float radius,
                            float *lm, hipStream_t s, Ragged rg = {});
hipError_t launch_seed_rank(const float *conf, const float *lm, int B, int N, int S, int *seeds,
                            hipStream_t s, Ragged rg = {}, uint32_t *scratch = nullptr);

hipError_t launch_knn_dist(const _Float16 *ns, const int *seeds, int B, int N, int S, float *dist,
                           hipStream_t s, Ragged rg = {});
hipError_t launch_split_rows(const float *x, size_t rows, _Float16 *out, hipStream_t s);
hipError_t launch_knn_dist_f32(const float *normed, const int *seeds, int B, int N, int S, float *dist,
                               hipStream_t s, Ragged rg = {});
hipError_t launch_knn_select(const float *dist, int B, int N, int S, int k, int *knn, hipStream_t s,
                             Ragged rg = {});
hipError_t launch_nsm_seed(const void *feats, bool f32, const float *src, const float *tgt, const int *knn, int B,
                           int N, int S, int k, int T, const float *sigma, const float *sigma_d, float *hist,
                           unsigned *seed_flags, hipStream_t s, Ragged rg = {});
hipError_t launch_nsm_finish(const float *hist, const unsigned *seed_flags, int B, int S, int k, int T, bool batch_global,
                             float *weights, int *iters_used, hipStream_t s, Ragged rg = {});
hipError_t launch_hypotheses(const float *src, const float *tgt, const int *knn, const float *weights,
                             int B, int N, int S, int k, float tau, float *seed_trans, int *counts,
                             float *sums, hipStream_t s, Ragged rg = {}, const float *hist = nullptr,
                             const unsigned *seed_flags = nullptr, int T = 0, float *wout = nullptr);
hipError_t launch_select_best(const float *src, const float *tgt, const float *seed_trans,
                              const int *counts, int B, int N, int S, float tau, float *fitness,
                              int *best, float *trans, float *labels, hipStream_t s, Ragged rg = {},
                              const float *conf = nullptr, int *range = nullptr);
hipError_t launch_post_refine(float *trans, const float *src, const float *tgt, int B, int N, float thr,
                              hipStream_t s, Ragged rg = {}, const int *range = nullptr);
hipError_t launch_best_refine(const float *src, const float *tgt, const float *seed_trans, const int *counts, int B,
                              int N, int S, float tau, float thr, float *trans, float *labels, hipStream_t s,
                              Ragged rg = {}, const float *conf = nullptr, int *range = nullptr);
hipError_t launch_rigid(const float *A, const float *Bp, const float *w, int nb, int n, float *trans,
                        hipStream_t s);

hipError_t launch_feat_sim(const void *feats, bool f32, int B, int N, const float *sigma, float *M, hipStream_t s);
size_t sm_loss_partial_doubles(int B, int N);
hipError_t launch_sm_loss(const float *M, const float *labels, int B, int N, int balanced, double *part, float *loss,
                          hipStream_t s);

struct CloudStats {
    float mn[3], mx[3];
    double centroid[3];
};
struct GridView {
    unsigned long long *skey, *ukey;
    int *sidx, *ustart, *ucount, *nruns;
};
struct GridBufs {
    CloudStats *st;
    GridView view;
    int *err;
};
size_t grid_workspace_bytes(int n);
hipError_t build_grid(const float *pts, int n, double cell, double half, void *ws, GridBufs &G, hipStream_t s);
hipError_t launch_radius_knn(const float *pts, int n, const GridBufs &G, double radius, int K, int *nbr, double *d2,
                             int *cnt, hipStream_t s);
hipError_t launch_normals(const float *pts, int n, const int *nbr, const int *cnt, int K, const GridBufs &G,
                          int orient, const float *viewpoint, float *nrm, hipStream_t s);
hipError_t launch_voxel_reduce(const float *pts, const float *nrm, int n, const GridBufs &G, float *opts, float *onrm,
                               int *count, hipStream_t s);
hipError_t launch_fpfh(const float *pts, const float *nrm, int n, const int *nbr, const int *cnt, const double *d2,
                       int K, double *spfh, double *out, float *outn, hipStream_t s);
int ply_read_xyz(const char *path, float *xyz, int64_t capacity, int64_t *n_out, std::string &err);

#define HIP_RET(expr)                         \
    do {                                      \
        hipError_t e_ = (expr);               \
        if (e_ != hipSuccess) return e_;      \
    } while (0)
hipError_t launch_sm(const float *corr, const float *src, const float *tgt, int N, float sig2, int S, int iters,
                     float *M, float *v, float *y, float *w, float *labels, float *trans, hipStream_t s);
hipError_t launch_sm_matvec(const float *M, const float *v, int N, float *y, hipStream_t s);
hipError_t launch_nn_argmin(const float *A, const float *B, int Na, int Nb, int D, unsigned long long *rowkey,
                            unsigned long long *colkey, hipStream_t s);
hipError_t launch_corr_build(const unsigned long long *rowkey, const unsigned long long *colkey,
                             const float *src_xyz, const float *tgt_xyz, int Na, int mutual, const double *gt,
                             double thr, int *corr, int *count, float *corr_pos, float *src_out, float *tgt_out,
                             float *labels, hipStream_t s);

}
```

Before: 35.00 million correspondences/s.

## Fold value projection into message first dense layer to halve attention V width

Precomputes, at weight-pack time, the product of the message MLP's first layer with the value projection, producing a folded 64-wide value matrix. Attention then carries 64-channel values instead of 128, which cuts V staging, MFMA work and accumulator registers in the softmax-times-V phase. The pointwise kernels skip the separate first message dense. This adds a packed-weight block and a new template path, and it changes the rounding order of the f16-split values.

```diff
diff --git a/include/pdsc.h b/include/pdsc.h
--- a/include/pdsc.h
+++ b/include/pdsc.h
@@ -69,6 +69,8 @@
 int32_t pdsc_attention_layout(int32_t B, int32_t N, int32_t precision, int32_t *Npad, int32_t *nsplit);
 
 int32_t pdsc_encoder_plan(int32_t B, int32_t N, int32_t precision, int32_t *fused);
+int32_t pdsc_encoder_plan_vfold(int32_t B, int32_t N, int32_t precision, int32_t *vfold);
+int32_t pdsc_packed_block(const pdsc_config *cfg, int32_t layer, int32_t block, size_t offsets[5]);
 
 int32_t pdsc_attention_timing(void *const *start_events, void *const *stop_events, int32_t capacity,
                               int32_t *count);
diff --git a/pointdsc_amd/_lib.py b/pointdsc_amd/_lib.py
--- a/pointdsc_amd/_lib.py
+++ b/pointdsc_amd/_lib.py
@@ -60,6 +60,8 @@
     "pdsc_attention_layout": (c_int32, [c_int32, c_int32, c_int32, ctypes.POINTER(c_int32),
                                         ctypes.POINTER(c_int32)]),
     "pdsc_encoder_plan": (c_int32, [c_int32, c_int32, c_int32, ctypes.POINTER(c_int32)]),
+    "pdsc_encoder_plan_vfold": (c_int32, [c_int32, c_int32, c_int32, ctypes.POINTER(c_int32)]),
+    "pdsc_packed_block": (c_int32, [CFG, c_int32, c_int32, ctypes.POINTER(c_size_t)]),
     "pdsc_attention_timing": (c_int32, [ctypes.POINTER(vp), ctypes.POINTER(vp), c_int32, ctypes.POINTER(c_int32)]),
     "pdsc_forward_timing": (c_int32, [ctypes.POINTER(vp), c_int32, ctypes.POINTER(c_int32)]),
     "pdsc_diag_qkv_delay": (c_int32, [c_int32]),
diff --git a/pointdsc_amd/csrc/api.hip b/pointdsc_amd/csrc/api.hip
--- a/pointdsc_amd/csrc/api.hip
+++ b/pointdsc_amd/csrc/api.hip
@@ -131,7 +131,7 @@
                 Ragged rg = {}) {
     const EncoderPlan plan = d.plan.for_ragged(rg);
     HIPCHK(launch_pw_first(packed, lay, corr_pos, d.f32, d.B, d.N, d.Npad, e.feat, e.q, e.k, e.v, e.vexp, s, rg,
-                           plan.fused()));
+                           plan.fused(), plan.vfold));
     if (plan.fused()) {
         _Float16 *q = e.q, *k = e.k, *v = e.v, *q2 = e.q2, *k2 = e.k2, *v2 = e.v2;
         float *vx = e.vexp, *vx2 = e.vexp2;
@@ -164,11 +164,11 @@
         }
         if (l + 1 < lay.L) {
             HIPCHK(launch_pw_mid(packed, lay, l, d.f32, op, mlp, ns, d.B, d.N, d.Npad, feat, feat_alt, e.q, e.k, e.v,
-                                 e.vexp, s));
+                                 e.vexp, s, plan.vfold));
             std::swap(feat, feat_alt);
         } else {
             HIPCHK(launch_pw_last(packed, lay, d.f32, op, mlp, ns, d.B, d.N, d.Npad, feat, feat_out, normed,
-                                  d.f32 ? nullptr : normed_s, conf, s));
+                                  d.f32 ? nullptr : normed_s, conf, s, plan.vfold));
         }
     }
     return PDSC_OK;
@@ -470,6 +470,8 @@
                                  has_bn ? P[wi + 5] : nullptr, in, out, f32, packed + o.w, packed + o.bias,
                                  packed + o.alpha, packed + o.beta, packed + o.scale, s);
     };
+    float *fold_tmp = nullptr;
+    HIPCHK(hipMallocAsync(reinterpret_cast<void **>(&fold_tmp), ((size_t)CH2 * CH + CH2) * sizeof(float), s));
     for (int l = 0; l < cfg->num_layers; ++l) {
         const int b = 2 + 26 * l;
         const LayerOff &lo = lay.layer[l];
@@ -480,7 +482,12 @@
         HIPCHK(dense(lo.q, b + 20, CH, CH, false));
         HIPCHK(dense(lo.k, b + 22, CH, CH, false));
         HIPCHK(dense(lo.v, b + 24, CH, CH, false));
-    }
+        float *wm = fold_tmp, *bm = wm + (size_t)CH2 * CH;
+        HIPCHK(launch_fold_vm(P[b + 6], P[b + 7], P[b + 24], P[b + 25], wm, bm, s));
+        HIPCHK(launch_pack_dense(wm, bm, P[b + 8], P[b + 9], P[b + 10], P[b + 11], CH, CH2, f32, packed + lo.vm.w,
+                                 packed + lo.vm.bias, packed + lo.vm.alpha, packed + lo.vm.beta, packed + lo.vm.scale, s));
+    }
+    HIPCHK(hipFreeAsync(fold_tmp, s));
     const int t = 2 + 26 * cfg->num_layers;
     HIPCHK(launch_copy(P[t], packed + lay.l0_w, CH * cfg->in_dim, s));
     HIPCHK(launch_copy(P[t + 1], packed + lay.l0_b, CH, s));
@@ -615,6 +622,25 @@
     if (B < 1 || N < 1 || !fused) return fail(PDSC_ERR_ARG, "B=%d N=%d", B, N);
     const EncoderPlan plan = plan_encoder(B, N, precision == PDSC_PRECISION_F32, false);
     *fused = plan.fused() ? 1 : (plan.w64() ? 2 : 0);
+    return PDSC_OK;
+}
+
+int32_t pdsc_encoder_plan_vfold(int32_t B, int32_t N, int32_t precision, int32_t *vfold) {
+    if (precision != PDSC_PRECISION_H3 && precision != PDSC_PRECISION_F32)
+        return fail(PDSC_ERR_ARG, "precision %d (enum pdsc_precision)", precision);
+    if (B < 1 || N < 1 || !vfold) return fail(PDSC_ERR_ARG, "B=%d N=%d", B, N);
+    *vfold = plan_encoder(B, N, precision == PDSC_PRECISION_F32, false).vfold ? 1 : 0;
+    return PDSC_OK;
+}
+
+int32_t pdsc_packed_block(const pdsc_config *cfg, int32_t layer, int32_t block, size_t offsets[5]) {
+    RET_IF(check_cfg(cfg));
+    if (layer < 0 || layer >= cfg->num_layers || block < 0 || block > 7 || !offsets)
+        return fail(PDSC_ERR_ARG, "layer=%d block=%d", layer, block);
+    const LayerOff lo = make_layout(cfg->num_layers, cfg->in_dim).layer[layer];
+    const DenseOff d[8] = {lo.pcn, lo.fc0, lo.fc3, lo.fc6, lo.q, lo.k, lo.v, lo.vm};
+    const DenseOff &o = d[block];
+    offsets[0] = o.w, offsets[1] = o.bias, offsets[2] = o.alpha, offsets[3] = o.beta, offsets[4] = o.scale;
     return PDSC_OK;
 }
 
diff --git a/pointdsc_amd/csrc/attention_h3.hpp b/pointdsc_amd/csrc/attention_h3.hpp
--- a/pointdsc_amd/csrc/attention_h3.hpp
+++ b/pointdsc_amd/csrc/attention_h3.hpp
@@ -221,12 +221,14 @@
     return AttnBlock{g.po ? g.po[slot] : slot, (lid / g.nsplit) % g.nqb, lid % g.nsplit};
 }
 
-template <int NW, bool PACKED, bool EARLY = false, int WS = 0>
+template <int NW, bool PACKED, bool EARLY = false, int WS = 0, int CV = CH>
 PDSC_DEV void attention_h3_core(const _Float16 *__restrict__ Qs, const _Float16 *__restrict__ Ks,
                                 const _Float16 *__restrict__ Vs, const float *__restrict__ vexp,
                                 const float *__restrict__ M, const AttnGridH3 &g, const AttnBlock &blk, char *h3smem,
-                                int wave, int lane, f32x16 (&O)[4], float &m_run, float &l_run) {
+                                int wave, int lane, f32x16 (&O)[CV / 32], float &m_run, float &l_run) {
     static_assert(WS == 0 || (NW == 1 && !EARLY), "wave-split: one 32-query block, the plain loop");
+    static_assert(CV == CH || (CV == CH2 && WS == 0), "value width");
+    constexpr int VTB = H3_VTB * CV / CH;
     const int b = blk.b, qb = blk.qb, split = blk.split;
     const int N = g.n(b), Npad = g.Npad;
     const int h = lane >> 5, l32 = lane & 31;
@@ -262,7 +264,8 @@
 #endif
     auto stage = [&](int st, int slot) {
         char *dst = h3smem + (WS ? wave : slot) * (H3_KTB + H3_VTB);
-        constexpr int PIECES = (H3_KTB + H3_VTB) / 1024;
+        constexpr int PIECES = (H3_KTB + VTB) / 1024;
+        static_assert(PIECES % NW == 0, "pieces per wave");
 #pragma unroll
         for (int i = 0; i < PIECES / NW; ++i) {
             const int piece = WS ? i : wave * (PIECES / NW) + i;
@@ -283,7 +286,7 @@
     };
 
 #pragma unroll
-    for (int t = 0; t < 4; ++t) O[t] = zero16();
+    for (int t = 0; t < CV / 32; ++t) O[t] = zero16();
     m_run = -INFINITY;
     l_run = 0.0f;
     const float scale = ATT_QFMA ? 1.0f : H3_QSCALE;
@@ -369,7 +372,7 @@
                 m_run = m_new;
                 l_run *= alpha;
 #pragma unroll
-                for (int t = 0; t < 4; ++t)
+                for (int t = 0; t < CV / 32; ++t)
 #pragma unroll
                     for (int r = 0; r < 16; ++r) O[t][r] *= alpha;
 #pragma unroll
@@ -396,7 +399,7 @@
                 m_run = m_new;
                 l_run *= alpha;
 #pragma unroll
-                for (int t = 0; t < 4; ++t)
+                for (int t = 0; t < CV / 32; ++t)
 #pragma unroll
                     for (int r = 0; r < 16; ++r) O[t][r] *= alpha;
             }
@@ -429,8 +432,8 @@
         vread(0, vf[0]);
         vread(1, vf[1]);
 #pragma unroll
-        for (int i = 0; i < 8; ++i) {
-            if (i + 2 < 8) vread(i + 2, vf[(i + 2) % 3]);
+        for (int i = 0; i < CV / 16; ++i) {
+            if (i + 2 < CV / 16) vread(i + 2, vf[(i + 2) % 3]);
             f32x16 o = mfma_h(vf[i % 3][0], pl[i & 1], O[i >> 1]);
             o = mfma_h(vf[i % 3][1], ph[i & 1], o);
             O[i >> 1] = mfma_h(vf[i % 3][0], ph[i & 1], o);
@@ -532,7 +535,7 @@
     l_run = halves_sum(l_run);
 }
 
-template <int NW, bool XCD, bool PACKED, bool EARLY = false>
+template <int NW, bool XCD, bool PACKED, bool EARLY = false, int CV = CH>
 __global__ __launch_bounds__(NW * 64, 2) void attention_h3_kernel(
     const _Float16 *__restrict__ Qs, const _Float16 *__restrict__ Ks, const _Float16 *__restrict__ Vs,
     const float *__restrict__ vexp, const float *__restrict__ M, AttnGridH3 g, float *__restrict__ opart,
@@ -548,16 +551,16 @@
     ATT_RSTAMP(stp, 184);
     ATT_STAMP(stp, 160);
 #endif
-    f32x16 O[4];
+    f32x16 O[CV / 32];
     float m_run, l_run;
-    attention_h3_core<NW, PACKED, EARLY>(Qs, Ks, Vs, vexp, M, g, blk, h3smem, wave, lane, O, m_run, l_run);
+    attention_h3_core<NW, PACKED, EARLY, 0, CV>(Qs, Ks, Vs, vexp, M, g, blk, h3smem, wave, lane, O, m_run, l_run);
     ATT_STAMP(stp, 161);
     ATT_RSTAMP(stp, 185);
     if (q0 >= Npad) return;
     const size_t obase = (size_t)(b * g.nsplit + split) * Npad;
     float *Ob = opart + obase * CH + (size_t)(q0 >> 5) * (H3_TILE * CH) + 4 * lane;
 #pragma unroll
-    for (int t = 0; t < 4; ++t)
+    for (int t = 0; t < CV / 32; ++t)
 #pragma unroll
         for (int q = 0; q < 4; ++q)
             *reinterpret_cast<f32x4 *>(Ob + (4 * t + q) * 256) =
diff --git a/pointdsc_amd/csrc/attention_plan.hpp b/pointdsc_amd/csrc/attention_plan.hpp
--- a/pointdsc_amd/csrc/attention_plan.hpp
+++ b/pointdsc_amd/csrc/attention_plan.hpp
@@ -23,6 +23,7 @@
     bool precombine;
     int zigzag;
     bool dense_m;
+    bool vfold;
 };
 inline const AttnKnobs &attn_knobs() {
     static const AttnKnobs k = [] {
@@ -41,6 +42,7 @@
         v.precombine = env_int("PDSC_PRECOMBINE", 1) != 0;
         v.zigzag = env_int("PDSC_ZIGZAG", 1);
         v.dense_m = env_int("PDSC_DENSE_M", 0) == 1;
+        v.vfold = env_int("PDSC_VFOLD", 1) != 0;
         return v;
     }();
     return k;
@@ -80,6 +82,7 @@
     int nsplit;
     bool precombine;
     int m_layout;
+    bool vfold;
 
     bool fused() const { return kind == ATT_FUSED; }
     bool w64() const { return kind == ATT_W64 || kind == ATT_W64_SK; }
diff --git a/pointdsc_amd/csrc/encoder.hip b/pointdsc_amd/csrc/encoder.hip
--- a/pointdsc_amd/csrc/encoder.hip
+++ b/pointdsc_amd/csrc/encoder.hip
@@ -82,6 +82,29 @@
     return hipGetLastError();
 }
 
+__global__ void fold_vm_kernel(const float *__restrict__ w0, const float *__restrict__ b0,
+                               const float *__restrict__ wv, const float *__restrict__ bv,
+                               float *__restrict__ wm, float *__restrict__ bm) {
+    const int i = blockIdx.x * blockDim.x + threadIdx.x;
+    if (i < CH2 * CH) {
+        const int o = i / CH, c = i % CH;
+        double acc = 0.0;
+        for (int j = 0; j < CH; ++j) acc += (double)w0[o * CH + j] * (double)wv[j * CH + c];
+        wm[i] = (float)acc;
+    }
+    if (i < CH2) {
+        double acc = (double)b0[i];
+        for (int j = 0; j < CH; ++j) acc += (double)w0[i * CH + j] * (double)bv[j];
+        bm[i] = (float)acc;
+    }
+}
+
+hipError_t launch_fold_vm(const float *w0, const float *b0, const float *wv, const float *bv, float *wm, float *bm,
+                          hipStream_t s) {
+    hipLaunchKernelGGL(fold_vm_kernel, dim3(CH2 * CH / 256), dim3(256), 0, s, w0, b0, wv, bv, wm, bm);
+    return hipGetLastError();
+}
+
 hipError_t launch_copy(const float *src, float *dst, int n, hipStream_t s) {
     hipLaunchKernelGGL(copy_kernel, dim3((n + 255) / 256), dim3(256), 0, s, src, dst, n);
     return hipGetLastError();
@@ -144,6 +167,9 @@
     p.precombine = k.precombine && !f32 && !fused && p.nsplit >= 16 && blocks <= 16;
     p.m_layout = w64 || !(f32 || dense_m_caller || k.dense_m) ? M_PACKED : M_DENSE;
 
+    p.vfold = k.vfold && allow_fused && !f32 &&
+              (fused || (use_pw2(B, p.Npad, f32) && !p.precombine &&
+                         (p.w64() || (p.kind == ATT_H3 && p.nw == ATT_NW))));
     if (fused) {
         p.kind = ATT_FUSED;
         p.nw = PW2_W;
@@ -191,6 +217,7 @@
         break;
     }
     case ATT_H3_WS:
+        if (plan.vfold) return hipErrorInvalidValue;
         with_int<2, 4>(plan.ws, [&](auto ws) {
             with_bool(packed, [&](auto pk) {
                 constexpr int WS = decltype(ws)::value;
@@ -200,6 +227,17 @@
         });
         break;
     case ATT_H3:
+        if (plan.vfold) {
+            if (plan.nw != ATT_NW) return hipErrorInvalidValue;
+            with_bool(plan.early, [&](auto early) {
+                with_bool(packed, [&](auto pk) {
+                    hipLaunchKernelGGL((attention_h3_kernel<ATT_NW, true, decltype(pk)::value, decltype(early)::value, CH2>),
+                                       grid, dim3(ATT_NW * 64), attention_h3_lds_bytes<ATT_NW>(), s, qs, ks, vs, vexp, M,
+                                       g, opart, ml);
+                });
+            });
+            break;
+        }
         with_int<1, 2, ATT_NW>(plan.nw, [&](auto nw) {
             with_bool(plan.early, [&](auto early) {
                 with_bool(packed, [&](auto pk) {
@@ -1205,6 +1243,39 @@
     }
 }
 
+PDSC_DEV void w2_combine_acc(const float *__restrict__ opart, const float *__restrict__ ml, int b, int nsplit, int Npad,
+                             int row, f32x16 (&a)[2], int lane) {
+    float mstar = -INFINITY;
+    for (int s = 0; s < nsplit; ++s) mstar = fmaxf(mstar, ml[((size_t)(b * nsplit + s) * Npad + row) * 2]);
+    float L = 0.0f;
+    f32x4 acc[8];
+#pragma unroll
+    for (int i = 0; i < 8; ++i) acc[i] = f32x4{0.0f, 0.0f, 0.0f, 0.0f};
+    for (int s = 0; s < nsplit; ++s) {
+        const size_t base = (size_t)(b * nsplit + s) * Npad + row;
+        const float ms = ml[base * 2];
+        if (ms == -INFINITY) continue;
+        const float w = expf(ms - mstar);
+        L += w * ml[base * 2 + 1];
+        const float *src = opart + (base - (row & 31)) * CH + 4 * lane;
+#pragma unroll
+        for (int i = 0; i < 8; ++i) acc[i] += w * *reinterpret_cast<const f32x4 *>(src + 256 * i);
+    }
+    const float rl = 1.0f / L;
+#pragma unroll
+    for (int i = 0; i < 8; ++i)
+#pragma unroll
+        for (int e = 0; e < 4; ++e) a[i >> 2][4 * (i & 3) + e] = acc[i][e] * rl;
+}
+
+PDSC_DEV void w2_msg_acc(const f32x16 (&O)[2], float l_run, f32x16 (&a)[2]) {
+    const float rl = 1.0f / l_run;
+#pragma unroll
+    for (int t = 0; t < 2; ++t)
+#pragma unroll
+        for (int r = 0; r < 16; ++r) a[t][r] = O[t][r] * rl;
+}
+
 PDSC_DEV void w2_msg_frags(const f32x16 (&O)[4], float l_run, f16x8 *xh, f16x8 *xl) {
     const float rl = 1.0f / l_run;
 #pragma unroll
@@ -1259,13 +1330,14 @@
         }
 }
 
-PDSC_DEV void w2_store_v(f32x16 (&acc)[4], float inv, const float *bias, _Float16 *__restrict__ Vt,
-                         float *__restrict__ vexp_t, int lane) {
+template <int NT>
+PDSC_DEV void w2_store_v(f32x16 (&acc)[NT], float inv, const float *bias, _Float16 *__restrict__ Vt,
+                         float *__restrict__ vexp_t, int lane, bool pad = false) {
     const int h = lane >> 5, l32 = lane & 31;
     float m = 0.0f;
 #pragma unroll
-    for (int t = 0; t < 4; ++t) {
-        const float bs = bias[32 * t + l32];
+    for (int t = 0; t < NT; ++t) {
+        const float bs = NT == 4 ? bias[32 * t + l32] : 0.0f;
 #pragma unroll
         for (int r = 0; r < 16; ++r) {
             acc[t][r] = __builtin_fmaf(acc[t][r], inv, bs);
@@ -1274,8 +1346,16 @@
     }
     const int ev = h3_vexp(wave_max(m));
     if (lane == 0) *vexp_t = (float)ev;
-#pragma unroll
-    for (int t = 0; t < 4; ++t) {
+    if (NT == 2 && pad) {
+        const f16x8 z = {0, 0, 0, 0, 0, 0, 0, 0};
+#pragma unroll
+        for (int i = 4; i < 8; ++i) {
+            *reinterpret_cast<f16x8 *>(Vt + h3_frag(i, 0, lane)) = z;
+            *reinterpret_cast<f16x8 *>(Vt + h3_frag(i, 1, lane)) = z;
+        }
+    }
+#pragma unroll
+    for (int t = 0; t < NT; ++t) {
 #pragma unroll
         for (int s = 0; s < 2; ++s) {
             float v[8];
@@ -1292,19 +1372,20 @@
 struct W2CoefQKV {
     static constexpr int pcn = 0, q = 3 * CH, k = 4 * CH, v = 5 * CH, end = 6 * CH;
 };
-PDSC_DEV void w2_coef_qkv(float *cf, const float *pk, const PwDense4 &d, int tid) {
+PDSC_DEV void w2_coef_qkv(float *cf, const float *pk, const PwDense4 &d, int tid, bool vfold) {
     w2_coef(cf + W2CoefQKV::pcn, pk, d.pcn, CH, tid);
     for (int i = tid; i < CH; i += PW2_W * 64) {
         cf[W2CoefQKV::q + i] = pk[d.q.bias + i];
         cf[W2CoefQKV::k + i] = pk[d.k.bias + i];
-        cf[W2CoefQKV::v + i] = pk[d.v.bias + i];
-    }
-}
-
+        if (!vfold) cf[W2CoefQKV::v + i] = pk[d.v.bias + i];
+    }
+}
+
+template <bool VFOLD>
 PDSC_DEV void w2_pcn_qkv(W2Pipe &P, const float *__restrict__ pk, const W2Sched &S, const float *cf, const PwDense4 &d,
                          const f16x8 *xh, const f16x8 *xl, float *__restrict__ featL, _Float16 *__restrict__ Q,
                          _Float16 *__restrict__ K, _Float16 *__restrict__ V, float *__restrict__ vexp, int row,
-                         bool active, int wave, int lane) {
+                         bool active, int wave, int lane, bool vpad = false) {
     const int h = lane >> 5;
     f32x16 acc[4];
     f16x8 yh[8], yl[8];
@@ -1321,8 +1402,16 @@
     w2_layer<CH, CH, true, 16>(P, pk, S, yh, yl, acc, active, wave, lane);
     if (active) w2_store_qk<false>(acc, sk, cf + W2CoefQKV::k, K, row, lane);
     CH_STAMP(177);
-    w2_layer<CH, CH, false, 16>(P, pk, S, yh, yl, acc, active, wave, lane);
-    if (active) w2_store_v(acc, sv, cf + W2CoefQKV::v, V + (size_t)(row >> 5) * H3_TILE_H, vexp + (row >> 5), lane);
+    if constexpr (VFOLD) {
+        f32x16 av[2];
+        w2_layer<CH, CH2, false, 16>(P, pk, S, yh, yl, av, active, wave, lane);
+        if (active)
+            w2_store_v<2>(av, sv, nullptr, V + (size_t)(row >> 5) * H3_TILE_H, vexp + (row >> 5), lane, vpad);
+    } else {
+        w2_layer<CH, CH, false, 16>(P, pk, S, yh, yl, acc, active, wave, lane);
+        if (active)
+            w2_store_v<4>(acc, sv, cf + W2CoefQKV::v, V + (size_t)(row >> 5) * H3_TILE_H, vexp + (row >> 5), lane);
+    }
     CH_STAMP(178);
 }
 
@@ -1330,21 +1419,27 @@
     static constexpr int f0 = W2CoefQKV::end, f3 = f0 + 3 * CH2, f6 = f3 + 3 * CH2, end = f6 + 3 * CH;
 };
 static_assert(W2CoefMid::end <= PW2_COEF, "coefficient table");
-PDSC_DEV void w2_coef_mid(float *cf, const float *__restrict__ pk, const PwMsg &m, const PwDense4 &d, int tid) {
-    w2_coef_qkv(cf, pk, d, tid);
+PDSC_DEV void w2_coef_mid(float *cf, const float *__restrict__ pk, const PwMsg &m, const PwDense4 &d, int tid,
+                          bool vfold) {
+    w2_coef_qkv(cf, pk, d, tid, vfold);
     w2_coef(cf + W2CoefMid::f0, pk, m.fc0, CH2, tid);
     w2_coef(cf + W2CoefMid::f3, pk, m.fc3, CH2, tid);
     w2_coef(cf + W2CoefMid::f6, pk, m.fc6, CH, tid);
 }
 
+template <bool VFOLD>
 PDSC_DEV void w2_mid_chain(W2Pipe &P, const float *__restrict__ pk, const W2Sched &S, const float *cf, const PwMsg &m,
-                           const PwDense4 &d, f16x8 *xh, f16x8 *xl, const float *featL_in, float *featL,
+                           const PwDense4 &d, f16x8 *xh, f16x8 *xl, f32x16 (&a2)[2], const float *featL_in, float *featL,
                            _Float16 *__restrict__ Q, _Float16 *__restrict__ K, _Float16 *__restrict__ V,
-                           float *__restrict__ vexp, int row, bool active, int wave, int lane) {
-    f32x16 a2[2], a4[4], res[4];
+                           float *__restrict__ vexp, int row, bool active, int wave, int lane, bool vpad = false) {
+    f32x16 a4[4], res[4];
     f16x8 yh[8], yl[8];
-    w2_layer<CH, CH2, true>(P, pk, S, xh, xl, a2, active, wave, lane);
-    if (active) w2_epilogue<CH2, EPI_BN_RELU>(a2, pk[m.fc0.scale], cf + W2CoefMid::f0, nullptr, yh, yl, lane);
+    if constexpr (VFOLD) {
+        if (active) w2_epilogue<CH2, EPI_BN_RELU>(a2, 1.0f, cf + W2CoefMid::f0, nullptr, yh, yl, lane);
+    } else {
+        w2_layer<CH, CH2, true>(P, pk, S, xh, xl, a2, active, wave, lane);
+        if (active) w2_epilogue<CH2, EPI_BN_RELU>(a2, pk[m.fc0.scale], cf + W2CoefMid::f0, nullptr, yh, yl, lane);
+    }
     CH_STAMP(172);
     w2_layer<CH2, CH2, true>(P, pk, S, yh, yl, a2, active, wave, lane);
     if (active) {
@@ -1355,7 +1450,7 @@
     w2_layer<CH2, CH, true, 16>(P, pk, S, xh, xl, a4, active, wave, lane);
     if (active) w2_epilogue<CH, EPI_RESID>(a4, pk[m.fc6.scale], cf + W2CoefMid::f6, res, yh, yl, lane);
     CH_STAMP(174);
-    w2_pcn_qkv(P, pk, S, cf, d, yh, yl, featL, Q, K, V, vexp, row, active, wave, lane);
+    w2_pcn_qkv<VFOLD>(P, pk, S, cf, d, yh, yl, featL, Q, K, V, vexp, row, active, wave, lane, vpad);
 }
 
 #define PW2_PROLOGUE                                                                              \
@@ -1368,17 +1463,18 @@
     float *cf = reinterpret_cast<float *>(w2smem + PW2_NSLOT * PW2_SLOT);                         \
     for (int c_ = 0; c_ < PW2_NSLOT; ++c_) w2_stage(pk, S, c_, P.slot(c_), wave, lane);
 
+template <bool VFOLD>
 __global__ __launch_bounds__(PW2_W * 64, PW2_OCC) void pw2_first_kernel(const float *__restrict__ pk, W2Sched S, size_t l0w,
                                                                  size_t l0b, PwDense4 d, const float *__restrict__ corr,
                                                                  int in_dim, int N, int Npad, float *__restrict__ featL,
                                                                  _Float16 *__restrict__ Q, _Float16 *__restrict__ K,
                                                                  _Float16 *__restrict__ V, float *__restrict__ vexp,
-                                                                 const int *__restrict__ nv) {
+                                                                 const int *__restrict__ nv, int vpad) {
     if (nv && (int)blockIdx.x * PW2_PTS >= nv[blockIdx.y]) return;
     PW2_PROLOGUE
     const int l32 = lane & 31;
     const int n = nv ? nv[b] : N;
-    w2_coef_qkv(cf, pk, d, tid);
+    w2_coef_qkv(cf, pk, d, tid, VFOLD);
     f16x8 xh[8], xl[8];
     if (active) {
         const float *cp = corr + ((size_t)b * N + min(row, n - 1)) * in_dim;
@@ -1404,10 +1500,11 @@
             }
     }
     __syncthreads();
-    w2_pcn_qkv(P, pk, S, cf, d, xh, xl, featL + boff, Q + 2 * boff, K + 2 * boff, V + 2 * boff,
-               vexp + (size_t)b * (Npad / 32), row, active, wave, lane);
-}
-
+    w2_pcn_qkv<VFOLD>(P, pk, S, cf, d, xh, xl, featL + boff, Q + 2 * boff, K + 2 * boff, V + 2 * boff,
+                      vexp + (size_t)b * (Npad / 32), row, active, wave, lane, vpad != 0);
+}
+
+template <bool VFOLD>
 __global__ __launch_bounds__(PW2_W * 64, PW2_OCC) void pw2_mid_kernel(const float *__restrict__ pk, W2Sched S, PwMsg m,
                                                                PwDense4 d, const float *__restrict__ opart,
                                                                const float *__restrict__ ml, int nsplit, int N,
@@ -1416,15 +1513,21 @@
                                                                _Float16 *__restrict__ Q, _Float16 *__restrict__ K,
                                                                _Float16 *__restrict__ V, float *__restrict__ vexp) {
     PW2_PROLOGUE
-    w2_coef_mid(cf, pk, m, d, tid);
+    w2_coef_mid(cf, pk, m, d, tid, VFOLD);
     f16x8 xh[8], xl[8];
-    if (active) w2_combine(opart, ml, b, nsplit, Npad, row, xh, xl, lane);
-    __syncthreads();
-    w2_mid_chain(P, pk, S, cf, m, d, xh, xl, featL_in + boff, featL + boff, Q + 2 * boff, K + 2 * boff,
-                 V + 2 * boff, vexp + (size_t)b * (Npad / 32), row, active, wave, lane);
-}
-
-template <bool PACKED>
+    f32x16 a2[2];
+    if (active) {
+        if constexpr (VFOLD)
+            w2_combine_acc(opart, ml, b, nsplit, Npad, row, a2, lane);
+        else
+            w2_combine(opart, ml, b, nsplit, Npad, row, xh, xl, lane);
+    }
+    __syncthreads();
+    w2_mid_chain<VFOLD>(P, pk, S, cf, m, d, xh, xl, a2, featL_in + boff, featL + boff, Q + 2 * boff, K + 2 * boff,
+                        V + 2 * boff, vexp + (size_t)b * (Npad / 32), row, active, wave, lane, true);
+}
+
+template <bool PACKED, bool VFOLD>
 __global__ __launch_bounds__(PW2_W * 64, PW2_OCC) void attn_pw2_kernel(
     const _Float16 *__restrict__ Qs, const _Float16 *__restrict__ Ks, const _Float16 *__restrict__ Vs,
     const float *__restrict__ vexp_in, const float *__restrict__ M, AttnGridH3 g, const float *__restrict__ pk,
@@ -1443,20 +1546,28 @@
     ATT_RSTAMP(stp, 188);
     ATT_STAMP(stp, 0);
 #endif
-    f32x16 O[4];
+    constexpr int CV = VFOLD ? CH2 : CH;
+    f32x16 O[CV / 32];
     float m_run, l_run;
-    attention_h3_core<PW2_W, PACKED, PW2_EARLY>(Qs, Ks, Vs, vexp_in, M, g, blk, w2smem, wave, lane, O, m_run, l_run);
+    attention_h3_core<PW2_W, PACKED, PW2_EARLY, 0, CV>(Qs, Ks, Vs, vexp_in, M, g, blk, w2smem, wave, lane, O, m_run,
+                                                       l_run);
     ATT_STAMP(stp, 170);
     W2Pipe P{w2smem, 0};
     float *cf = reinterpret_cast<float *>(w2smem + PW2_NSLOT * PW2_SLOT);
     for (int c = 0; c < PW2_NSLOT; ++c) w2_stage(pk, S, c, P.slot(c), wave, lane);
-    w2_coef_mid(cf, pk, m, d, tid);
+    w2_coef_mid(cf, pk, m, d, tid, VFOLD);
     f16x8 xh[8], xl[8];
-    if (active) w2_msg_frags(O, l_run, xh, xl);
+    f32x16 a2[2];
+    if (active) {
+        if constexpr (VFOLD)
+            w2_msg_acc(O, l_run, a2);
+        else
+            w2_msg_frags(O, l_run, xh, xl);
+    }
     __syncthreads();
     ATT_STAMP(stp, 171);
-    w2_mid_chain(P, pk, S, cf, m, d, xh, xl, featL + boff, featL + boff, Q + 2 * boff, K + 2 * boff,
-                 V + 2 * boff, vexp + (size_t)b * (Npad / 32), row, active, wave, lane);
+    w2_mid_chain<VFOLD>(P, pk, S, cf, m, d, xh, xl, a2, featL + boff, featL + boff, Q + 2 * boff, K + 2 * boff,
+                        V + 2 * boff, vexp + (size_t)b * (Npad / 32), row, active, wave, lane);
     ATT_STAMP(stp, 180);
     ATT_RSTAMP(stp, 189);
 }
@@ -1488,18 +1599,23 @@
     for (int i = tid; i < CLS; i += PW2_W * 64) cf[W2CoefLast::c4 + i] = pk[c4w + i];
 }
 
+template <bool VFOLD>
 PDSC_DEV void w2_last_chain(W2Pipe &P, const float *__restrict__ pk, const W2Sched &S, const float *cf, const PwMsg &m,
-                            const DenseOff &c0, const DenseOff &c2, size_t c4b, f16x8 *xh, f16x8 *xl,
+                            const DenseOff &c0, const DenseOff &c2, size_t c4b, f16x8 *xh, f16x8 *xl, f32x16 (&a2)[2],
                             const float *__restrict__ featL, float *__restrict__ feat_out, float *__restrict__ normed,
                             _Float16 *__restrict__ normed_s, float *__restrict__ conf, int b, int N, int row,
                             bool active, int wave, int lane) {
     constexpr int CF0 = W2CoefLast::f0, CF3 = W2CoefLast::f3, CF6 = W2CoefLast::f6, CC0 = W2CoefLast::c0,
                   CC2 = W2CoefLast::c2, CC4 = W2CoefLast::c4;
     const int h = lane >> 5;
-    f32x16 a1[1], a2[2], a4[4], res[4];
+    f32x16 a1[1], a4[4], res[4];
     f16x8 yh[8], yl[8];
-    w2_layer<CH, CH2, true>(P, pk, S, xh, xl, a2, active, wave, lane);
-    if (active) w2_epilogue<CH2, EPI_BN_RELU>(a2, pk[m.fc0.scale], cf + CF0, nullptr, yh, yl, lane);
+    if constexpr (VFOLD) {
+        if (active) w2_epilogue<CH2, EPI_BN_RELU>(a2, 1.0f, cf + CF0, nullptr, yh, yl, lane);
+    } else {
+        w2_layer<CH, CH2, true>(P, pk, S, xh, xl, a2, active, wave, lane);
+        if (active) w2_epilogue<CH2, EPI_BN_RELU>(a2, pk[m.fc0.scale], cf + CF0, nullptr, yh, yl, lane);
+    }
     w2_layer<CH2, CH2, true>(P, pk, S, yh, yl, a2, active, wave, lane);
     if (active) {
         w2_epilogue<CH2, EPI_BN_RELU>(a2, pk[m.fc3.scale], cf + CF3, nullptr, xh, xl, lane);
@@ -1562,6 +1678,7 @@
     }
 }
 
+template <bool VFOLD>
 __global__ __launch_bounds__(PW2_W * 64, PW2_OCC) void pw2_last_kernel(
     const float *__restrict__ pk, W2Sched S, PwMsg m, DenseOff c0, DenseOff c2, size_t c4w, size_t c4b,
     const float *__restrict__ opart, const float *__restrict__ ml, int nsplit, int N, int Npad,
@@ -1570,13 +1687,19 @@
     PW2_PROLOGUE
     w2_coef_last(cf, pk, m, c0, c2, c4w, tid);
     f16x8 xh[8], xl[8];
-    if (active) w2_combine(opart, ml, b, nsplit, Npad, row, xh, xl, lane);
-    __syncthreads();
-    w2_last_chain(P, pk, S, cf, m, c0, c2, c4b, xh, xl, featL + boff, feat_out, normed, normed_s, conf, b, N, row,
-                  active, wave, lane);
-}
-
-template <bool PACKED>
+    f32x16 a2[2];
+    if (active) {
+        if constexpr (VFOLD)
+            w2_combine_acc(opart, ml, b, nsplit, Npad, row, a2, lane);
+        else
+            w2_combine(opart, ml, b, nsplit, Npad, row, xh, xl, lane);
+    }
+    __syncthreads();
+    w2_last_chain<VFOLD>(P, pk, S, cf, m, c0, c2, c4b, xh, xl, a2, featL + boff, feat_out, normed, normed_s, conf, b, N,
+                         row, active, wave, lane);
+}
+
+template <bool PACKED, bool VFOLD>
 __global__ __launch_bounds__(PW2_W * 64, PW2_OCC) void attn_pw2_last_kernel(
     const _Float16 *__restrict__ Qs, const _Float16 *__restrict__ Ks, const _Float16 *__restrict__ Vs,
     const float *__restrict__ vexp_in, const float *__restrict__ M, AttnGridH3 g, const float *__restrict__ pk,
@@ -1590,53 +1713,66 @@
               lane = tid & 63;
     const int row = blk.qb * PW2_PTS + wave * 32 + (lane & 31);
     const bool active = blk.qb * PW2_PTS + wave * 32 < Npad;
-    f32x16 O[4];
+    constexpr int CV = VFOLD ? CH2 : CH;
+    f32x16 O[CV / 32];
     float m_run, l_run;
-    attention_h3_core<PW2_W, PACKED, PW2_EARLY>(Qs, Ks, Vs, vexp_in, M, g, blk, w2smem, wave, lane, O, m_run, l_run);
+    attention_h3_core<PW2_W, PACKED, PW2_EARLY, 0, CV>(Qs, Ks, Vs, vexp_in, M, g, blk, w2smem, wave, lane, O, m_run,
+                                                       l_run);
     W2Pipe P{w2smem, 0};
     float *cf = reinterpret_cast<float *>(w2smem + PW2_NSLOT * PW2_SLOT);
     for (int c = 0; c < PW2_NSLOT; ++c) w2_stage(pk, S, c, P.slot(c), wave, lane);
     w2_coef_last(cf, pk, m, c0, c2, c4w, tid);
     f16x8 xh[8], xl[8];
-    if (active) w2_msg_frags(O, l_run, xh, xl);
-    __syncthreads();
-    w2_last_chain(P, pk, S, cf, m, c0, c2, c4b, xh, xl, featL + (size_t)b * Npad * CH, feat_out, normed, normed_s,
-                  conf, b, N, row, active, wave, lane);
+    f32x16 a2[2];
+    if (active) {
+        if constexpr (VFOLD)
+            w2_msg_acc(O, l_run, a2);
+        else
+            w2_msg_frags(O, l_run, xh, xl);
+    }
+    __syncthreads();
+    w2_last_chain<VFOLD>(P, pk, S, cf, m, c0, c2, c4b, xh, xl, a2, featL + (size_t)b * Npad * CH, feat_out, normed,
+                         normed_s, conf, b, N, row, active, wave, lane);
 }
 #undef PW2_PROLOGUE
 
-static W2Sched sched_qkv(W2Sched S, const PwDense4 &d) {
+static W2Sched sched_qkv(W2Sched S, const PwDense4 &d, bool vfold) {
     w2_sched_add(S, d.pcn, CH, CH);
     w2_sched_add(S, d.q, CH, CH);
     w2_sched_add(S, d.k, CH, CH);
-    w2_sched_add(S, d.v, CH, CH);
+    w2_sched_add(S, d.v, CH, vfold ? CH2 : CH);
     return S;
 }
-static W2Sched sched_msg(const PwMsg &m) {
+static W2Sched sched_msg(const PwMsg &m, bool vfold) {
     W2Sched S{};
-    w2_sched_add(S, m.fc0, CH, CH2);
+    if (!vfold) w2_sched_add(S, m.fc0, CH, CH2);
     w2_sched_add(S, m.fc3, CH2, CH2);
     w2_sched_add(S, m.fc6, CH2, CH);
     return S;
 }
 
-static PwDense4 dense4(const LayerOff &l) { return PwDense4{l.pcn, l.q, l.k, l.v}; }
-static PwMsg msg3(const LayerOff &l) { return PwMsg{l.fc0, l.fc3, l.fc6}; }
+static PwDense4 dense4(const LayerOff &l, bool vfold = false) { return PwDense4{l.pcn, l.q, l.k, vfold ? l.vm : l.v}; }
+static PwMsg msg3(const LayerOff &l, bool vfold = false) { return PwMsg{vfold ? l.vm : l.fc0, l.fc3, l.fc6}; }
 
 hipError_t launch_attn_pw2(const EncoderPlan &plan, const float *packed, const PackLayout &lay, int layer,
                            const void *q, const void *k, const void *v, const float *vexp_in, const float *M,
                            float *feat, void *qo, void *ko, void *vo, float *vexp_out, hipStream_t s, Ragged rg) {
     if (!plan.fused() || layer + 1 >= lay.L) return hipErrorInvalidValue;
     const AttnGridH3 g = plan_grid_h3(plan, rg, layer);
-    const W2Sched S = sched_qkv(sched_msg(msg3(lay.layer[layer])), dense4(lay.layer[layer + 1]));
+    const bool vf = plan.vfold;
+    const PwMsg m = msg3(lay.layer[layer], vf);
+    const PwDense4 d = dense4(lay.layer[layer + 1], vf);
+    const W2Sched S = sched_qkv(sched_msg(m, vf), d, vf);
     const size_t lds = std::max(attention_h3_lds_bytes<PW2_W>(), PW2_LDS);
     const _Float16 *qs = static_cast<const _Float16 *>(q), *ks = static_cast<const _Float16 *>(k),
                    *vs = static_cast<const _Float16 *>(v);
     _Float16 *Q = static_cast<_Float16 *>(qo), *K = static_cast<_Float16 *>(ko), *V = static_cast<_Float16 *>(vo);
     with_bool(plan.m_layout == M_PACKED, [&](auto pk) {
-        hipLaunchKernelGGL(attn_pw2_kernel<decltype(pk)::value>, dim3(plan.workgroups()), dim3(PW2_W * 64), lds, s, qs,
-                           ks, vs, vexp_in, M, g, packed, S, msg3(lay.layer[layer]), dense4(lay.layer[layer + 1]), feat,
-                           Q, K, V, vexp_out);
+        with_bool(vf, [&](auto vfold) {
+            hipLaunchKernelGGL((attn_pw2_kernel<decltype(pk)::value, decltype(vfold)::value>), dim3(plan.workgroups()),
+                               dim3(PW2_W * 64), lds, s, qs, ks, vs, vexp_in, M, g, packed, S, m, d, feat, Q, K, V,
+                               vexp_out);
+        });
     });
     return hipGetLastError();
 }
@@ -1647,17 +1783,20 @@
                                 Ragged rg) {
     if (!plan.fused()) return hipErrorInvalidValue;
     const AttnGridH3 g = plan_grid_h3(plan, rg, lay.L - 1);
-    W2Sched S = sched_msg(msg3(lay.layer[lay.L - 1]));
+    const bool vf = plan.vfold;
+    const PwMsg m = msg3(lay.layer[lay.L - 1], vf);
+    W2Sched S = sched_msg(m, vf);
     w2_sched_add(S, lay.c0, CH, CLS);
     w2_sched_add(S, lay.c2, CLS, CLS);
     const size_t lds = std::max(attention_h3_lds_bytes<PW2_W>(), PW2_LDS);
     const _Float16 *qs = static_cast<const _Float16 *>(q), *ks = static_cast<const _Float16 *>(k),
                    *vs = static_cast<const _Float16 *>(v);
-    const PwMsg m = msg3(lay.layer[lay.L - 1]);
     with_bool(plan.m_layout == M_PACKED, [&](auto pk) {
-        hipLaunchKernelGGL(attn_pw2_last_kernel<decltype(pk)::value>, dim3(plan.workgroups()), dim3(PW2_W * 64), lds, s,
-                           qs, ks, vs, vexp_in, M, g, packed, S, m, lay.c0, lay.c2, lay.c4_w, lay.c4_b, feat, feat_out,
-                           normed, normed_s, conf);
+        with_bool(vf, [&](auto vfold) {
+            hipLaunchKernelGGL((attn_pw2_last_kernel<decltype(pk)::value, decltype(vfold)::value>),
+                               dim3(plan.workgroups()), dim3(PW2_W * 64), lds, s, qs, ks, vs, vexp_in, M, g, packed, S, m,
+                               lay.c0, lay.c2, lay.c4_w, lay.c4_b, feat, feat_out, normed, normed_s, conf);
+        });
     });
     return hipGetLastError();
 }
@@ -1703,16 +1842,20 @@
 
 hipError_t launch_pw_first(const float *packed, const PackLayout &lay, const float *corr_pos, bool f32, int B,
                            int N, int Npad, float *feat, void *q, void *k, void *v, float *vexp, hipStream_t s,
-                           Ragged rg, bool fused) {
+                           Ragged rg, bool fused, bool vfold) {
     if (lay.in_dim > IN_LIMIT) return hipErrorInvalidValue;
     _Float16 *Q = static_cast<_Float16 *>(q), *K = static_cast<_Float16 *>(k), *V = static_cast<_Float16 *>(v);
     if (fused || use_pw2(B, Npad, f32)) {
-        const W2Sched S = sched_qkv(W2Sched{}, dense4(lay.layer[0]));
-        hipLaunchKernelGGL(pw2_first_kernel, dim3((Npad + PW2_PTS - 1) / PW2_PTS, B), dim3(PW2_W * 64), PW2_LDS, s,
-                           packed, S, lay.l0_w, lay.l0_b, dense4(lay.layer[0]), corr_pos, lay.in_dim, N, Npad, feat, Q, K,
-                           V, vexp, rg.nv);
+        const PwDense4 d = dense4(lay.layer[0], vfold);
+        const W2Sched S = sched_qkv(W2Sched{}, d, vfold);
+        with_bool(vfold, [&](auto vf) {
+            hipLaunchKernelGGL(pw2_first_kernel<decltype(vf)::value>, dim3((Npad + PW2_PTS - 1) / PW2_PTS, B),
+                               dim3(PW2_W * 64), PW2_LDS, s, packed, S, lay.l0_w, lay.l0_b, d, corr_pos, lay.in_dim, N,
+                               Npad, feat, Q, K, V, vexp, rg.nv, (int)!fused);
+        });
         return hipGetLastError();
     }
+    if (vfold) return hipErrorInvalidValue;
     if (!f32 && small_tiles(B, Npad) && pw_qkv_split(B, Npad)) {
         hipLaunchKernelGGL((pw_first_kernel<32, false>), dim3(Npad / 32, B, 3), dim3(256), pw_lds<32>(), s, packed,
                            lay.l0_w, lay.l0_b, dense4(lay.layer[0]), corr_pos, lay.in_dim, N, Npad, feat, Q, K, V, vexp,
@@ -1726,16 +1869,21 @@
 
 hipError_t launch_pw_mid(const float *packed, const PackLayout &lay, int layer, bool f32, const float *opart,
                          const float *ml, int nsplit, int B, int N, int Npad, const float *feat_in, float *feat,
-                         void *q, void *k, void *v, float *vexp, hipStream_t s) {
+                         void *q, void *k, void *v, float *vexp, hipStream_t s, bool vfold) {
     const int delay = g_diag_qkv_delay;
     _Float16 *Q = static_cast<_Float16 *>(q), *K = static_cast<_Float16 *>(k), *V = static_cast<_Float16 *>(v);
     if (use_pw2(B, Npad, f32)) {
-        const W2Sched S = sched_qkv(sched_msg(msg3(lay.layer[layer])), dense4(lay.layer[layer + 1]));
-        hipLaunchKernelGGL(pw2_mid_kernel, dim3((Npad + PW2_PTS - 1) / PW2_PTS, B), dim3(PW2_W * 64), PW2_LDS, s,
-                           packed, S, msg3(lay.layer[layer]), dense4(lay.layer[layer + 1]), opart, ml, nsplit, N, Npad,
-                           feat_in, feat, Q, K, V, vexp);
+        const PwMsg m = msg3(lay.layer[layer], vfold);
+        const PwDense4 d = dense4(lay.layer[layer + 1], vfold);
+        const W2Sched S = sched_qkv(sched_msg(m, vfold), d, vfold);
+        with_bool(vfold, [&](auto vf) {
+            hipLaunchKernelGGL(pw2_mid_kernel<decltype(vf)::value>, dim3((Npad + PW2_PTS - 1) / PW2_PTS, B),
+                               dim3(PW2_W * 64), PW2_LDS, s, packed, S, m, d, opart, ml, nsplit, N, Npad, feat_in, feat, Q,
+                               K, V, vexp);
+        });
         return hipGetLastError();
     }
+    if (vfold) return hipErrorInvalidValue;
     if (!f32 && pw_waves8(B, Npad)) {
         hipLaunchKernelGGL((pw_mid_kernel<32, false, 8>), dim3(Npad / 32, B, pw_qkv_split(B, Npad) ? 3 : 1), dim3(512),
                            pw_lds<32>(), s, packed,
@@ -1750,16 +1898,21 @@
 
 hipError_t launch_pw_last(const float *packed, const PackLayout &lay, bool f32, const float *opart,
                           const float *ml, int nsplit, int B, int N, int Npad, const float *feat,
-                          float *feat_out, float *normed, _Float16 *normed_s, float *conf, hipStream_t s) {
+                          float *feat_out, float *normed, _Float16 *normed_s, float *conf, hipStream_t s,
+                          bool vfold) {
     if (use_pw2(B, Npad, f32)) {
-        W2Sched S = sched_msg(msg3(lay.layer[lay.L - 1]));
+        const PwMsg m = msg3(lay.layer[lay.L - 1], vfold);
+        W2Sched S = sched_msg(m, vfold);
         w2_sched_add(S, lay.c0, CH, CLS);
         w2_sched_add(S, lay.c2, CLS, CLS);
-        hipLaunchKernelGGL(pw2_last_kernel, dim3((Npad + PW2_PTS - 1) / PW2_PTS, B), dim3(PW2_W * 64), PW2_LDS, s,
-                           packed, S, msg3(lay.layer[lay.L - 1]), lay.c0, lay.c2, lay.c4_w, lay.c4_b, opart, ml, nsplit, N,
-                           Npad, feat, feat_out, normed, normed_s, conf);
+        with_bool(vfold, [&](auto vf) {
+            hipLaunchKernelGGL(pw2_last_kernel<decltype(vf)::value>, dim3((Npad + PW2_PTS - 1) / PW2_PTS, B),
+                               dim3(PW2_W * 64), PW2_LDS, s, packed, S, m, lay.c0, lay.c2, lay.c4_w, lay.c4_b, opart, ml,
+                               nsplit, N, Npad, feat, feat_out, normed, normed_s, conf);
+        });
         return hipGetLastError();
     }
+    if (vfold) return hipErrorInvalidValue;
     PW_LAUNCH(pw_last_kernel, N, packed, msg3(lay.layer[lay.L - 1]), lay.c0, lay.c2, lay.c4_w, lay.c4_b, opart, ml,
               nsplit, N, Npad, feat, feat_out, normed, normed_s, conf);
     return hipGetLastError();
diff --git a/pointdsc_amd/csrc/pdsc_internal.hpp b/pointdsc_amd/csrc/pdsc_internal.hpp
--- a/pointdsc_amd/csrc/pdsc_internal.hpp
+++ b/pointdsc_amd/csrc/pdsc_internal.hpp
@@ -41,7 +41,7 @@
 };
 
 struct LayerOff {
-    DenseOff pcn, fc0, fc3, fc6, q, k, v;
+    DenseOff pcn, fc0, fc3, fc6, q, k, v, vm;
 };
 
 struct PackLayout {
@@ -100,6 +100,7 @@
     o += CLS;
     p.c4_b = o;
     o += 4;
+    for (int l = 0; l < L; ++l) p.layer[l].vm = dense_at(o, CH, CH2);
     p.total = o;
     return p;
 }
@@ -125,6 +126,8 @@
                              const float *bn_rm, const float *bn_rv, int in, int out, bool f32, float *dst_w,
                              float *dst_b, float *dst_a, float *dst_beta, float *dst_scale, hipStream_t s);
 hipError_t launch_copy(const float *src, float *dst, int n, hipStream_t s);
+hipError_t launch_fold_vm(const float *w0, const float *b0, const float *wv, const float *bv, float *wm, float *bm,
+                          hipStream_t s);
 
 enum MLayout { M_DENSE = 0, M_PACKED = 1 };
 struct EncoderPlan;
@@ -145,15 +148,16 @@
 
 hipError_t launch_pw_first(const float *packed, const PackLayout &lay, const float *corr_pos, bool f32, int B,
                            int N, int Npad, float *feat, void *q, void *k, void *v, float *vexp, hipStream_t s,
-                           Ragged rg = {}, bool fused = false);
+                           Ragged rg = {}, bool fused = false, bool vfold = false);
 hipError_t launch_combine_rows(const float *opart, const float *ml, int B, int Npad, int nsplit, float *opart1,
                                float *ml1, hipStream_t s);
 hipError_t launch_pw_mid(const float *packed, const PackLayout &lay, int layer, bool f32, const float *opart,
                          const float *ml, int nsplit, int B, int N, int Npad, const float *feat_in, float *feat,
-                         void *q, void *k, void *v, float *vexp, hipStream_t s);
+                         void *q, void *k, void *v, float *vexp, hipStream_t s, bool vfold = false);
 hipError_t launch_pw_last(const float *packed, const PackLayout &lay, bool f32, const float *opart,
                           const float *ml, int nsplit, int B, int N, int Npad, const float *feat,
-                          float *feat_out, float *normed, _Float16 *normed_s, float *conf, hipStream_t s);
+                          float *feat_out, float *normed, _Float16 *normed_s, float *conf, hipStream_t s,
+                          bool vfold = false);
 
 hipError_t launch_local_max(const float *src, const float *conf, int B, int N, float radius,
                             float *lm, hipStream_t s, Ragged rg = {});
```

New measurement: 41.39 million correspondences/s (median of 6 runs). 18.3% higher.
